# jianfch/stable-ts

Hardware: AMD Instinct MI355X
Metric: real-time factor (audio-sec/wall-sec) large-v3 word_timestamps=True (higher is better)
Workload: dtype f16; 1 GPU; large-v3 (random-init, weight recipe BENCH_WEIGHTS = the parity-pinned recipe of tests/test_gpu_f16_depth.py), 10 min synthetic 16 kHz audio per GPU, word_timestamps=True, beam_size=5, 112 decode steps/window, window-parallel batch 20, default regrouping inside the timed pass; mode=transcribe, windows_per_gpu=20, segments=125, words=1670, parallelism=dp1 (windows sharded, no data-path collective)

## Files before the change

include/swx.h:

```cpp
#ifndef SWX_H
#define SWX_H
#include <stdint.h>
#include <stddef.h>

#ifdef __cplusplus
extern "C" {
#endif

#define SWX_F32 0
#define SWX_F16 1

#define SWX_N_SAMPLES 480000
#define SWX_N_FRAMES 3000
#define SWX_N_FFT 400
#define SWX_HOP 160

typedef struct swx_dims {
    int32_t n_mels, n_audio_ctx, n_audio_state, n_audio_head, n_audio_layer;
    int32_t n_vocab, n_text_ctx, n_text_state, n_text_head, n_text_layer;
} swx_dims;

typedef struct swx_model swx_model;

const char *swx_strerror(int code);
int swx_version(void);

int swx_model_create(const swx_dims *dims, int dtype, swx_model **out);
void swx_model_destroy(swx_model *m);
size_t swx_weights_bytes(const swx_model *m);
int swx_bind_weights(swx_model *m, void *d_arena, size_t bytes);
int swx_share_weights(swx_model *m, const swx_model *owner);
int swx_load_tensor(swx_model *m, const char *name, const float *d_src, int64_t numel, void *stream);
int swx_weights_complete(const swx_model *m);
int swx_missing_tensor(const swx_model *m, int index, char *buf, int buflen);
int swx_weights_mark_loaded(swx_model *m);
int swx_weights_finalize(swx_model *m, void *stream);
int swx_set_alignment_heads(swx_model *m, const int32_t *h_layer_head_pairs, int n_pairs);
int swx_num_alignment_heads(const swx_model *m);

size_t swx_workspace_bytes(const swx_model *m, int max_windows, int max_rows);
int swx_bind_workspace(swx_model *m, void *d_ws, size_t bytes, int max_windows, int max_rows);

int swx_log_mel(swx_model *m, const float *d_pcm, int B, float *d_mel, int per_item_max, void *stream);

int swx_log_mel_ragged(swx_model *m, const float *d_pcm, const int32_t *n_valid, const int32_t *n_total, int B,
                       float *d_mel, int per_item_max, void *stream);
int swx_log_mel_ragged_grouped(swx_model *m, const float *d_pcm, const int32_t *n_valid, const int32_t *n_total, int B,
                               float *d_mel, int group, void *stream);

int swx_encode(swx_model *m, const float *d_mel, int B, void *d_xa, void *stream);

size_t swx_cross_kv_bytes(const swx_model *m, int B);
int swx_cross_kv(swx_model *m, const void *d_xa, int B, void *d_xkv, void *stream);

typedef struct swx_decode_cfg {
    int32_t n_windows;
    int32_t n_group;
    int32_t beam;
    float temperature;
    float patience;
    int32_t sample_len;
    int32_t sample_begin;
    int32_t sot_index;
    int32_t suppress_blank;
    int32_t apply_timestamp_rules;
    int32_t max_initial_timestamp_index;
    int32_t eot, sot, no_timestamps, timestamp_begin, no_speech, blank_token;
    int32_t n_suppress;
    int32_t min_tokens;
    uint64_t seed;
    const int32_t *window_uid;
    const float *noise;
    const int32_t *sample_begins;
    const int32_t *sot_indices;
} swx_decode_cfg;

int swx_decode(swx_model *m, const swx_decode_cfg *cfg, const int32_t *d_init_tokens, const int32_t *d_suppress,
               const uint8_t *d_ts_mask, const void *d_xkv, int32_t *d_tokens_out, int32_t *d_lens_out,
               float *d_sumlp_out, float *d_nospeech, void *stream);
int swx_decode_gout(const swx_decode_cfg *cfg);

int swx_score(swx_model *m, const int32_t *d_tokens, const int32_t *h_n_tok, int W, int max_n, int n_sot, int eot,
              const int32_t *h_n_frames, float qk_scale, int medfilt_width, const void *d_xkv,
              float *d_token_probs, float *d_neg_matrix, void *stream);

int swx_score_qk(swx_model *m, const int32_t *d_tokens, const int32_t *h_n_tok, int W, int max_n, int n_sot, int eot,
                 int row0, int n_rows, const void *d_xkv, float *d_token_probs, float *d_qk, void *stream);

size_t swx_qcap_bytes(const swx_model *m, int max_n);
int swx_score_q(swx_model *m, const int32_t *d_tokens, const int32_t *h_n_tok, int max_n, int n_sot, int eot,
                const void *d_xkv, float *d_token_probs, void *d_q, void *stream);
size_t swx_heads_scratch_bytes(const swx_model *m, int max_n);
int swx_heads_dynamic(swx_model *m, const void *d_q, int max_n, int row0, int n_rows, const void *d_xkv, int n_frames,
                      float qk_scale, int count, const double *d_peaks, float *d_qk_sel, int ld_f, void *d_scratch,
                      size_t scratch_bytes, void *stream);
int swx_heads_new(swx_model *m, const void *d_q, int max_n, int n_tok, int row0, int n_out, const void *d_xkv, int n_frames,
                  float qk_scale, int medfilt_width, int topk, float w_colnorm, float w_rownorm, float w_coverage,
                  float *d_neg_matrix, int ld_f, void *d_scratch, size_t scratch_bytes, void *stream);
int swx_weighted_sum(const float *const *h_xs, const float *h_coef, int n_in, float *d_out, int64_t n, void *stream);

int swx_forward_logits(swx_model *m, const int32_t *d_tokens, const int32_t *h_n_tok, int W, int max_n,
                       const void *d_xkv, float *d_logits, void *stream);

int swx_forward_token_ranks(swx_model *m, const int32_t *d_tokens, const int32_t *h_n_tok, int W, int max_n, int n_vocab_used,
                            const void *d_xkv, float *d_prob, int32_t *d_rank, void *stream);

size_t swx_align_weights_scratch_bytes(int W, int H, int N);
int swx_align_weights(const float *d_qk, int W, int H, int N, int ld_f, const int32_t *h_n_frames, float qk_scale,
                      int medfilt_width, float *d_neg_matrix, void *d_scratch, size_t scratch_bytes, void *stream);

int swx_median_filter(const float *d_x, int64_t rows, int n, int width, float *d_out, void *stream);

int swx_loudness_probe(const float *d_pcm, int64_t pcm_stride, const int32_t *d_nk, const int32_t *d_idx, int n_idx, int W,
                       float *d_out, void *d_scratch, size_t scratch_bytes, void *stream);
size_t swx_loudness_probe_scratch_bytes(int W);

typedef struct swx_flac_info {
    int32_t sample_rate, channels, bits_per_sample, min_block, max_block;
    int64_t total_samples;
    uint8_t md5[16];
} swx_flac_info;
int swx_flac_probe(const uint8_t *h_data, size_t n_bytes, swx_flac_info *info);
int64_t swx_flac_decode(const uint8_t *h_data, size_t n_bytes, int32_t *h_out, int64_t capacity_frames, swx_flac_info *info);

size_t swx_dtw_workspace_bytes(int W, int ld_n, int ld_m);
int swx_dtw(const float *d_x, int W, int ld_n, int ld_m, const int32_t *d_N, const int32_t *d_M,
            int32_t *d_text_idx, int32_t *d_time_idx, int32_t *d_len, void *d_trace_ws, void *stream);

int swx_prof_enable(int on);
int swx_debug_flags(int flags);
int swx_prof_collect(double *out, int n_classes);
int swx_graph_stats(const swx_model *m, int64_t *out);

int swx_test_gemm(int dtype, const void *d_a, int64_t lda, const void *d_w, const float *d_bias, const void *d_res,
                  void *d_c, int64_t ldc, int M, int N, int K, int epilogue, int force_kernel, void *stream);
int swx_test_gemm_plan(int M, int N, int K, int epilogue, int force_kernel, int flags);
int swx_test_dec_gemm(const void *d_a, int64_t lda, const void *d_w, const float *d_gamma, const float *d_beta,
                      const float *d_bias, void *d_c, int64_t ldc, void *d_x, void *d_kcache, void *d_vcache,
                      const int32_t *d_pos0, int n_ctx, int d, int M, int N, int K, int epilogue, void *d_scratch,
                      size_t scratch_bytes, void *stream);
int swx_test_layernorm(int dtype, const void *d_x, const float *d_g, const float *d_b, void *d_y, int rows, int d,
                       void *stream);
int swx_test_attention(int dtype, const void *d_q, int64_t ldq, const void *d_k, const void *d_v, int64_t ldkv,
                       void *d_o, int64_t ldo, int B, int H, int nq, int nk, int force_kernel, int vt_kp, void *stream);

int swx_test_self_attn_step(const void *d_q, void *d_kcache, void *d_vcache, const int32_t *d_anc, const int32_t *d_pos0,
                            int R, int H, int n_ctx, int d, int variant, void *d_o, void *stream);

int swx_test_self_attn_multi(const void *d_q, void *d_kcache, void *d_vcache, int R, int H, int n_new, int n_ctx, int d, int mq,
                             void *d_o, void *stream);

int swx_test_lane_xor(const uint32_t *d_in, uint32_t *d_out, int n_waves, void *stream);

int swx_test_gelu_pair(uint64_t *d_out, void *stream);

#ifdef __cplusplus
}
#endif
#endif
```

stable_ts_amd/_lib.py:

```python
import ctypes
import os
from ctypes import POINTER, Structure, c_char_p, c_float, c_int, c_int32, c_int64, c_size_t, c_uint64, c_void_p

_HERE = os.path.dirname(os.path.abspath(__file__))
LIB_PATH = os.path.join(_HERE, "libswx.so")

SWX_F32 = 0
SWX_F16 = 1


class SwxError(RuntimeError):
    pass


class swx_dims(Structure):
    _fields_ = [(n, c_int32) for n in ("n_mels", "n_audio_ctx", "n_audio_state", "n_audio_head", "n_audio_layer",
                                       "n_vocab", "n_text_ctx", "n_text_state", "n_text_head", "n_text_layer")]


class swx_flac_info(Structure):
    _fields_ = [("sample_rate", c_int32), ("channels", c_int32), ("bits_per_sample", c_int32), ("min_block", c_int32),
                ("max_block", c_int32), ("total_samples", c_int64), ("md5", ctypes.c_uint8 * 16)]


class swx_decode_cfg(Structure):
    _fields_ = [
        ("n_windows", c_int32), ("n_group", c_int32), ("beam", c_int32), ("temperature", c_float),
        ("patience", c_float), ("sample_len", c_int32), ("sample_begin", c_int32), ("sot_index", c_int32),
        ("suppress_blank", c_int32), ("apply_timestamp_rules", c_int32), ("max_initial_timestamp_index", c_int32),
        ("eot", c_int32), ("sot", c_int32), ("no_timestamps", c_int32), ("timestamp_begin", c_int32),
        ("no_speech", c_int32), ("blank_token", c_int32), ("n_suppress", c_int32), ("min_tokens", c_int32),
        ("seed", c_uint64), ("window_uid", POINTER(c_int32)), ("noise", c_void_p),
        ("sample_begins", POINTER(c_int32)), ("sot_indices", POINTER(c_int32)),
    ]


SYMBOLS = {
    "swx_strerror": (c_char_p, [c_int]),
    "swx_version": (c_int, []),
    "swx_model_create": (c_int, [POINTER(swx_dims), c_int, POINTER(c_void_p)]),
    "swx_model_destroy": (None, [c_void_p]),
    "swx_weights_bytes": (c_size_t, [c_void_p]),
    "swx_bind_weights": (c_int, [c_void_p, c_void_p, c_size_t]),
    "swx_share_weights": (c_int, [c_void_p, c_void_p]),
    "swx_load_tensor": (c_int, [c_void_p, c_char_p, c_void_p, c_int64, c_void_p]),
    "swx_weights_complete": (c_int, [c_void_p]),
    "swx_missing_tensor": (c_int, [c_void_p, c_int, c_char_p, c_int]),
    "swx_weights_mark_loaded": (c_int, [c_void_p]),
    "swx_weights_finalize": (c_int, [c_void_p, c_void_p]),
    "swx_set_alignment_heads": (c_int, [c_void_p, POINTER(c_int32), c_int]),
    "swx_num_alignment_heads": (c_int, [c_void_p]),
    "swx_workspace_bytes": (c_size_t, [c_void_p, c_int, c_int]),
    "swx_bind_workspace": (c_int, [c_void_p, c_void_p, c_size_t, c_int, c_int]),
    "swx_log_mel": (c_int, [c_void_p, c_void_p, c_int, c_void_p, c_int, c_void_p]),
    "swx_log_mel_ragged": (c_int, [c_void_p, c_void_p, c_void_p, c_void_p, c_int, c_void_p, c_int, c_void_p]),
    "swx_log_mel_ragged_grouped": (c_int, [c_void_p, c_void_p, c_void_p, c_void_p, c_int, c_void_p, c_int, c_void_p]),
    "swx_encode": (c_int, [c_void_p, c_void_p, c_int, c_void_p, c_void_p]),
    "swx_cross_kv_bytes": (c_size_t, [c_void_p, c_int]),
    "swx_cross_kv": (c_int, [c_void_p, c_void_p, c_int, c_void_p, c_void_p]),
    "swx_decode": (c_int, [c_void_p, POINTER(swx_decode_cfg), c_void_p, c_void_p, c_void_p, c_void_p, c_void_p,
                           c_void_p, c_void_p, c_void_p, c_void_p]),
    "swx_decode_gout": (c_int, [POINTER(swx_decode_cfg)]),
    "swx_score": (c_int, [c_void_p, c_void_p, POINTER(c_int32), c_int, c_int, c_int, c_int, POINTER(c_int32), c_float,
                          c_int, c_void_p, c_void_p, c_void_p, c_void_p]),
    "swx_score_qk": (c_int, [c_void_p, c_void_p, POINTER(c_int32), c_int, c_int, c_int, c_int, c_int, c_int, c_void_p,
                             c_void_p, c_void_p, c_void_p]),
    "swx_qcap_bytes": (c_size_t, [c_void_p, c_int]),
    "swx_score_q": (c_int, [c_void_p, c_void_p, POINTER(c_int32), c_int, c_int, c_int, c_void_p, c_void_p, c_void_p, c_void_p]),
    "swx_heads_scratch_bytes": (c_size_t, [c_void_p, c_int]),
    "swx_heads_dynamic": (c_int, [c_void_p, c_void_p, c_int, c_int, c_int, c_void_p, c_int, c_float, c_int, c_void_p, c_void_p,
                                  c_int, c_void_p, c_size_t, c_void_p]),
    "swx_heads_new": (c_int, [c_void_p, c_void_p, c_int, c_int, c_int, c_int, c_void_p, c_int, c_float, c_int, c_int, c_float,
                              c_float, c_float, c_void_p, c_int, c_void_p, c_size_t, c_void_p]),
    "swx_weighted_sum": (c_int, [c_void_p, c_void_p, c_int, c_void_p, c_int64, c_void_p]),
    "swx_forward_logits": (c_int, [c_void_p, c_void_p, POINTER(c_int32), c_int, c_int, c_void_p, c_void_p, c_void_p]),
    "swx_forward_token_ranks": (c_int, [c_void_p, c_void_p, POINTER(c_int32), c_int, c_int, c_int, c_void_p, c_void_p, c_void_p,
                                        c_void_p]),
    "swx_align_weights_scratch_bytes": (c_size_t, [c_int, c_int, c_int]),
    "swx_align_weights": (c_int, [c_void_p, c_int, c_int, c_int, c_int, POINTER(c_int32), c_float, c_int, c_void_p,
                                  c_void_p, c_size_t, c_void_p]),
    "swx_median_filter": (c_int, [c_void_p, c_int64, c_int, c_int, c_void_p, c_void_p]),
    "swx_loudness_probe": (c_int, [c_void_p, c_int64, c_void_p, c_void_p, c_int, c_int, c_void_p, c_void_p, c_size_t, c_void_p]),
    "swx_loudness_probe_scratch_bytes": (c_size_t, [c_int]),
    "swx_flac_probe": (c_int, [c_void_p, c_size_t, POINTER(swx_flac_info)]),
    "swx_flac_decode": (c_int64, [c_void_p, c_size_t, c_void_p, c_int64, POINTER(swx_flac_info)]),
    "swx_dtw_workspace_bytes": (c_size_t, [c_int, c_int, c_int]),
    "swx_dtw": (c_int, [c_void_p, c_int, c_int, c_int, c_void_p, c_void_p, c_void_p, c_void_p, c_void_p, c_void_p,
                        c_void_p]),
    "swx_prof_enable": (c_int, [c_int]),
    "swx_debug_flags": (c_int, [c_int]),
    "swx_prof_collect": (c_int, [POINTER(ctypes.c_double), c_int]),
    "swx_graph_stats": (c_int, [c_void_p, POINTER(c_int64)]),
    "swx_test_gemm": (c_int, [c_int, c_void_p, c_int64, c_void_p, c_void_p, c_void_p, c_void_p, c_int64, c_int, c_int,
                              c_int, c_int, c_int, c_void_p]),
    "swx_test_gemm_plan": (c_int, [c_int, c_int, c_int, c_int, c_int, c_int]),
    "swx_test_dec_gemm": (c_int, [c_void_p, c_int64, c_void_p, c_void_p, c_void_p, c_void_p, c_void_p, c_int64, c_void_p,
                                  c_void_p, c_void_p, c_void_p, c_int, c_int, c_int, c_int, c_int, c_int, c_void_p, c_size_t,
                                  c_void_p]),
    "swx_test_self_attn_step": (c_int, [c_void_p, c_void_p, c_void_p, c_void_p, c_void_p, c_int, c_int, c_int, c_int, c_int, c_void_p,
                                        c_void_p]),
    "swx_test_self_attn_multi": (c_int, [c_void_p, c_void_p, c_void_p, c_int, c_int, c_int, c_int, c_int, c_int, c_void_p, c_void_p]),
    "swx_test_gelu_pair": (c_int, [c_void_p, c_void_p]),
    "swx_test_lane_xor": (c_int, [c_void_p, c_void_p, c_int, c_void_p]),
    "swx_test_layernorm": (c_int, [c_int, c_void_p, c_void_p, c_void_p, c_void_p, c_int, c_int, c_void_p]),
    "swx_test_attention": (c_int, [c_int, c_void_p, c_int64, c_void_p, c_void_p, c_int64, c_void_p, c_int64, c_int,
                                   c_int, c_int, c_int, c_int, c_int, c_void_p]),
}

_lib = None


def load(build_if_missing: bool = False) -> ctypes.CDLL:
    global _lib
    if _lib is not None:
        return _lib
    if not os.path.exists(LIB_PATH):
        if build_if_missing:
            from .build import build
            build(verbose=False)
        else:
            raise SwxError(f"{LIB_PATH} not found: build it with `python -m stable_ts_amd.build` "
                           f"(hipcc --offload-arch=gfx950). There is no CPU fallback.")
    lib = ctypes.CDLL(LIB_PATH)
    for name, (res, args) in SYMBOLS.items():
        fn = getattr(lib, name)
        fn.restype = res
        fn.argtypes = args
    _lib = lib
    return lib


def check(code: int, what: str = "") -> int:
    if code < 0:
        msg = load().swx_strerror(code).decode()
        raise SwxError(f"{what or 'libswx'} failed: {msg} ({code})")
    return code


def require_gpu():
    import torch
    if not torch.cuda.is_available():
        raise SwxError("stable_ts_amd needs a ROCm GPU (MI355X / gfx950); no CPU path exists in this package")
```

stable_ts_amd/csrc/swx_common.h:

```cpp
#pragma once
#include <hip/hip_runtime.h>
#include <hip/hip_fp16.h>
#include <stdint.h>
#include <math.h>

#define SWX_WAVE 64

typedef _Float16 f16;
typedef _Float16 f16x4 __attribute__((ext_vector_type(4)));
typedef _Float16 f16x8 __attribute__((ext_vector_type(8)));
typedef float f32x4 __attribute__((ext_vector_type(4)));
typedef float f32x16 __attribute__((ext_vector_type(16)));

#define SWX_CHECK_LAUNCH() do { hipError_t _e = hipGetLastError(); if (_e != hipSuccess) return -100 - (int)_e; } while (0)

static inline int cdiv(int64_t a, int64_t b) { return (int)((a + b - 1) / b); }

template <typename T> __device__ __forceinline__ float to_f32(T v);
template <> __device__ __forceinline__ float to_f32<float>(float v) { return v; }
template <> __device__ __forceinline__ float to_f32<f16>(f16 v) { return (float)v; }
template <typename T> __device__ __forceinline__ T from_f32(float v);
template <> __device__ __forceinline__ float from_f32<float>(float v) { return v; }
template <> __device__ __forceinline__ f16 from_f32<f16>(float v) { return (f16)v; }

template <typename T> __device__ __forceinline__ void load8(const T *p, float (&o)[8]);
template <> __device__ __forceinline__ void load8<f16>(const f16 *p, float (&o)[8]) {
    const f16x8 v = *(const f16x8 *)p;
#pragma unroll
    for (int e = 0; e < 8; ++e) o[e] = (float)v[e];
}
template <> __device__ __forceinline__ void load8<float>(const float *p, float (&o)[8]) {
    const f32x4 a = *(const f32x4 *)p, b = *(const f32x4 *)(p + 4);
#pragma unroll
    for (int e = 0; e < 4; ++e) { o[e] = a[e]; o[4 + e] = b[e]; }
}

__device__ __forceinline__ int swx_lane_id() { return (int)__builtin_amdgcn_mbcnt_hi(~0u, __builtin_amdgcn_mbcnt_lo(~0u, 0u)); }

template <int O> __device__ __forceinline__ unsigned lane_xor_u32(unsigned x, int lane)
{
    static_assert(O == 1 || O == 2 || O == 4 || O == 8 || O == 16 || O == 32, "lane_xor: one butterfly step");
#ifdef SWX_LANE_XOR_BPERMUTE
    return (unsigned)__shfl_xor((int)x, O, 64);
#endif
    if constexpr (O == 32) {
        const auto r = __builtin_amdgcn_permlane32_swap(x, x, false, false);
        return (lane & 32) ? r[0] : r[1];
    } else if constexpr (O == 16) {
        const auto r = __builtin_amdgcn_permlane16_swap(x, x, false, false);
        return (lane & 16) ? r[0] : r[1];
    } else if constexpr (O == 8) {
        return (unsigned)__builtin_amdgcn_update_dpp(0, (int)x, 0x128, 0xF, 0xF, false);
    } else if constexpr (O == 4) {
        int t = __builtin_amdgcn_update_dpp(0, (int)x, 0x104, 0xF, 0x5, false);
        t = __builtin_amdgcn_update_dpp(t, (int)x, 0x114, 0xF, 0xA, false);
        return (unsigned)t;
    } else if constexpr (O == 2) {
        return (unsigned)__builtin_amdgcn_update_dpp(0, (int)x, 0x4E, 0xF, 0xF, false);
    } else {
        return (unsigned)__builtin_amdgcn_update_dpp(0, (int)x, 0xB1, 0xF, 0xF, false);
    }
}
template <int O> __device__ __forceinline__ float lane_xor(float x, int lane) { return __uint_as_float(lane_xor_u32<O>(__float_as_uint(x), lane)); }
template <int O> __device__ __forceinline__ int lane_xor(int x, int lane) { return (int)lane_xor_u32<O>((unsigned)x, lane); }
template <int O> __device__ __forceinline__ double lane_xor(double x, int lane)
{
    const unsigned long long u = (unsigned long long)__double_as_longlong(x);
    const unsigned lo = lane_xor_u32<O>((unsigned)u, lane), hi = lane_xor_u32<O>((unsigned)(u >> 32), lane);
    return __longlong_as_double((long long)(((unsigned long long)hi << 32) | lo));
}
__device__ __forceinline__ float lane_xor16_max(float x) {
#ifdef SWX_LANE_XOR_BPERMUTE
    return fmaxf(x, __shfl_xor(x, 16, 64));
#endif
    const unsigned u = __float_as_uint(x);
    const auto r = __builtin_amdgcn_permlane16_swap(u, u, false, false);
    return fmaxf(__uint_as_float(r[0]), __uint_as_float(r[1]));
}
__device__ __forceinline__ float lane_xor32_max(float x) {
#ifdef SWX_LANE_XOR_BPERMUTE
    return fmaxf(x, __shfl_xor(x, 32, 64));
#endif
    const unsigned u = __float_as_uint(x);
    const auto r = __builtin_amdgcn_permlane32_swap(u, u, false, false);
    return fmaxf(__uint_as_float(r[0]), __uint_as_float(r[1]));
}
__device__ __forceinline__ float lane_xor16_add(float x) {
#ifdef SWX_LANE_XOR_BPERMUTE
    return x + __shfl_xor(x, 16, 64);
#endif
    const unsigned u = __float_as_uint(x);
    const auto r = __builtin_amdgcn_permlane16_swap(u, u, false, false);
    return __uint_as_float(r[0]) + __uint_as_float(r[1]);
}
__device__ __forceinline__ float lane_xor32_add(float x) {
#ifdef SWX_LANE_XOR_BPERMUTE
    return x + __shfl_xor(x, 32, 64);
#endif
    const unsigned u = __float_as_uint(x);
    const auto r = __builtin_amdgcn_permlane32_swap(u, u, false, false);
    return __uint_as_float(r[0]) + __uint_as_float(r[1]);
}

__device__ __forceinline__ float lane_xor16_max_lds(float x) {
#ifdef SWX_XATTN_VALU
    return lane_xor16_max(x);
#else
    return fmaxf(x, __shfl_xor(x, 16, 64));
#endif
}
__device__ __forceinline__ float lane_xor32_max_lds(float x) {
#ifdef SWX_XATTN_VALU
    return lane_xor32_max(x);
#else
    return fmaxf(x, __shfl_xor(x, 32, 64));
#endif
}
__device__ __forceinline__ float lane_xor16_add_lds(float x) {
#ifdef SWX_XATTN_VALU
    return lane_xor16_add(x);
#else
    return x + __shfl_xor(x, 16, 64);
#endif
}
__device__ __forceinline__ float lane_xor32_add_lds(float x) {
#ifdef SWX_XATTN_VALU
    return lane_xor32_add(x);
#else
    return x + __shfl_xor(x, 32, 64);
#endif
}

__device__ __forceinline__ float wave_max(float v) {
    const int lane = swx_lane_id();
    v = fmaxf(v, lane_xor<32>(v, lane)); v = fmaxf(v, lane_xor<16>(v, lane)); v = fmaxf(v, lane_xor<8>(v, lane));
    v = fmaxf(v, lane_xor<4>(v, lane)); v = fmaxf(v, lane_xor<2>(v, lane)); v = fmaxf(v, lane_xor<1>(v, lane));
    return v;
}
__device__ __forceinline__ float wave_sum(float v) {
    const int lane = swx_lane_id();
    v += lane_xor<32>(v, lane); v += lane_xor<16>(v, lane); v += lane_xor<8>(v, lane);
    v += lane_xor<4>(v, lane); v += lane_xor<2>(v, lane); v += lane_xor<1>(v, lane);
    return v;
}
__device__ __forceinline__ double wave_sum_d(double v) {
    const int lane = swx_lane_id();
    v += lane_xor<32>(v, lane); v += lane_xor<16>(v, lane); v += lane_xor<8>(v, lane);
    v += lane_xor<4>(v, lane); v += lane_xor<2>(v, lane); v += lane_xor<1>(v, lane);
    return v;
}

__device__ __forceinline__ float gelu_erf(float x) { return 0.5f * x * (1.0f + erff(x * 0.70710678118654752440f)); }

typedef float f32x2 __attribute__((ext_vector_type(2)));
__device__ __forceinline__ f32x2 swx_k2(unsigned u) { const float f = __uint_as_float(u); return (f32x2){f, f}; }
__device__ __forceinline__ f32x2 gelu_erf2(f32x2 x)
{
#ifdef SWX_GELU_SCALAR
    return (f32x2){gelu_erf(x[0]), gelu_erf(x[1])};
#else
    const f32x2 z = x * swx_k2(0x3f3504f3u);
    const f32x2 az = __builtin_elementwise_abs(z);
    f32x2 p = __builtin_elementwise_fma(az, swx_k2(0x378e98abu), swx_k2(0xb9c68948u));
    p = __builtin_elementwise_fma(az, p, swx_k2(0x3b7cd369u));
    p = __builtin_elementwise_fma(az, p, swx_k2(0xbcc618b2u));
    p = __builtin_elementwise_fma(az, p, swx_k2(0x3dda74e4u));
    p = __builtin_elementwise_fma(az, p, swx_k2(0x3f228afdu));
    p = __builtin_elementwise_fma(az, p, swx_k2(0x3e03c728u));
    const f32x2 t = __builtin_elementwise_fma(az, p, az);
    f32x2 a = t * swx_k2(0xbfb8aa3bu);
    f32x2 b = __builtin_elementwise_fma(t, swx_k2(0xbfb8aa3bu), -a);
    f32x2 r;
    r[0] = __builtin_rintf(a[0]); r[1] = __builtin_rintf(a[1]);
    b = __builtin_elementwise_fma(t, swx_k2(0xb2a5705fu), b);
    a = a - r;
    a = a + b;
    f32x2 big;
#pragma unroll
    for (int i = 0; i < 2; ++i) {
        float e = __builtin_amdgcn_exp2f(a[i]);
        e = __builtin_ldexpf(e, (int)r[i]);
        e = !(__uint_as_float(0x42ce8ed0u) < t[i]) ? e : 0.f;
        e = !(__uint_as_float(0xc2b17218u) > t[i]) ? e : __builtin_inff();
        big[i] = e;
    }
    big = swx_k2(0x3f800000u) - big;
    const f32x2 t2 = z * z;
    f32x2 q = __builtin_elementwise_fma(swx_k2(0xba1345e1u), t2, swx_k2(0x3ba10414u));
    q = __builtin_elementwise_fma(t2, q, swx_k2(0xbcdac9b8u));
    q = __builtin_elementwise_fma(t2, q, swx_k2(0x3de703beu));
    q = __builtin_elementwise_fma(t2, q, swx_k2(0xbec09330u));
    q = __builtin_elementwise_fma(t2, q, swx_k2(0x3e0375d0u));
    const f32x2 small = __builtin_elementwise_fma(az, q, az);
    f32x2 erf;
#pragma unroll
    for (int i = 0; i < 2; ++i) {
        const float res = !(az[i] < 1.0f) ? big[i] : small[i];
        erf[i] = __uint_as_float((__float_as_uint(res) & 0x7fffffffu) | (__float_as_uint(z[i]) & 0x80000000u));
    }
    return (x * swx_k2(0x3f000000u)) * (erf + swx_k2(0x3f800000u));
#endif
}
template <int N> __device__ __forceinline__ void gelu_erf_n(float (&v)[N])
{
    static_assert(N % 2 == 0, "pairs");
#pragma unroll
    for (int e = 0; e < N; e += 2) { f32x2 t = {v[e], v[e + 1]}; t = gelu_erf2(t); v[e] = t[0]; v[e + 1] = t[1]; }
}

__device__ __forceinline__ unsigned f32_to_ordered(float f) {
    unsigned u = __float_as_uint(f);
    return (u & 0x80000000u) ? ~u : (u | 0x80000000u);
}
__device__ __forceinline__ float ordered_to_f32(unsigned u) {
    return __uint_as_float((u & 0x80000000u) ? (u & 0x7fffffffu) : ~u);
}
```

stable_ts_amd/csrc/swx_decode.h:

```cpp
#pragma once
#include <hip/hip_runtime.h>
#include <stdint.h>
#include "../../include/swx.h"

struct DecodeBufs {
    swx_decode_cfg cfg;
    int W, G, M, V, TS, n_ctx, n_init;
    int max_cand, fin_cap;
    int32_t *tokens[2];
    int32_t *anc[2];
    int32_t *pos0;
    const int32_t *begin;
    float *sum_lp, *sum_lp_next;
    int32_t *row_done;
    int32_t *win_done, *win_done_prev;
    int32_t *n_done;
    int32_t *step_dev;
    int32_t *fin_tokens;
    float *fin_score;
    int32_t *fin_len;
    int32_t *fin_count;
    float *cand_lp;
    int32_t *cand_tok;
    float *logits;
    const int32_t *suppress;
    const uint8_t *ts_mask;
    const int32_t *win_uid;
};

int swx_decode_init(const DecodeBufs &b, const int32_t *init_tokens, hipStream_t s);
int swx_decode_after_prefill(const DecodeBufs &b, const float *lg2, float *nospeech, hipStream_t s);
int swx_decode_select(const DecodeBufs &b, int cur, hipStream_t s);
int swx_decode_finalize(const DecodeBufs &b, int cur, int n_steps, int32_t *tokens_out, int32_t *lens_out,
                        float *sumlp_out, int G_out, hipStream_t s);
```

stable_ts_amd/csrc/swx_decode.hip:

```cpp
#include "swx_common.h"
#include "swx_kernels.h"
#include "swx_decode.h"

namespace {

constexpr int SEL_T = 1024;
constexpr float NEG_INF = -__builtin_inff();

struct ArgMax { float v; int i; };

__device__ __forceinline__ ArgMax argmax_combine(ArgMax a, ArgMax b)
{
    if (b.v > a.v || (b.v == a.v && b.i < a.i)) return b;
    return a;
}

static_assert(SEL_T == 1024, "block reductions: 16 wave slots");

__device__ ArgMax block_argmax(ArgMax x, ArgMax *sh)
{
    const int wave = threadIdx.x >> 6, lane = threadIdx.x & 63;
#define SWX_ARGMAX_STEP(O) { ArgMax y; y.v = lane_xor<O>(x.v, lane); y.i = lane_xor<O>(x.i, lane); x = argmax_combine(x, y); }
    SWX_ARGMAX_STEP(32) SWX_ARGMAX_STEP(16) SWX_ARGMAX_STEP(8) SWX_ARGMAX_STEP(4) SWX_ARGMAX_STEP(2) SWX_ARGMAX_STEP(1)
    __syncthreads();
    if (lane == 0) sh[wave] = x;
    __syncthreads();
#ifdef SWX_SELECT_R5_REDUCE
    ArgMax r = sh[0];
    for (int w = 1; w < (int)(blockDim.x >> 6); ++w) r = argmax_combine(r, sh[w]);
    return r;
#else
    x = sh[lane & 15];
    SWX_ARGMAX_STEP(8) SWX_ARGMAX_STEP(4) SWX_ARGMAX_STEP(2) SWX_ARGMAX_STEP(1)
    return x;
#endif
#undef SWX_ARGMAX_STEP
}

__device__ float block_max(float x, float *sh)
{
    x = wave_max(x);
    const int wave = threadIdx.x >> 6, lane = threadIdx.x & 63;
    __syncthreads();
    if (lane == 0) sh[wave] = x;
    __syncthreads();
#if defined(SWX_SELECT_R5_REDUCE) || defined(SWX_SELECT_MAX_WALK)
    float r = sh[0];
    for (int w = 1; w < (int)(blockDim.x >> 6); ++w) r = fmaxf(r, sh[w]);
    return r;
#else
    const f32x4 *s4 = (const f32x4 *)sh;
    float r = -__builtin_inff();
#pragma unroll
    for (int q = 0; q < 4; ++q) { const f32x4 v = s4[q]; r = fmaxf(r, fmaxf(fmaxf(v[0], v[1]), fmaxf(v[2], v[3]))); }
    return r;
#endif
}

__device__ float block_sum(float x, float *sh)
{
    x = wave_sum(x);
    const int wave = threadIdx.x >> 6, lane = threadIdx.x & 63;
    __syncthreads();
    if (lane == 0) sh[wave] = x;
    __syncthreads();
    float r = 0.f;
#if defined(SWX_SELECT_R5_REDUCE) || defined(SWX_SELECT_SUM_WALK)
    for (int w = 0; w < (int)(blockDim.x >> 6); ++w) r += sh[w];
#else
    const f32x4 *s4 = (const f32x4 *)sh;
#pragma unroll
    for (int q = 0; q < 4; ++q) { const f32x4 v = s4[q]; r += v[0]; r += v[1]; r += v[2]; r += v[3]; }
#endif
    return r;
}

__device__ __forceinline__ unsigned hash32(unsigned x)
{
    x ^= x >> 16; x *= 0x7feb352du; x ^= x >> 15; x *= 0x846ca68bu; x ^= x >> 16;
    return x;
}

__device__ __forceinline__ float gumbel(uint64_t seed, unsigned row_uid, unsigned step, unsigned idx)
{
    unsigned h = hash32((unsigned)seed ^ hash32(idx + 0x9e3779b9u * (step + 1u)));
    h = hash32(h ^ hash32(row_uid * 0x85ebca6bu + (unsigned)(seed >> 32)));
    const float u = ((float)(h >> 8) + 0.5f) * (1.0f / 16777216.0f);
    return -logf(-logf(u));
}

__device__ __forceinline__ int win_begin(const DecodeBufs &b, int w) { return b.begin ? b.begin[w] : b.n_init; }

__global__ void decode_init_kernel(DecodeBufs b, const int32_t *__restrict__ init_tokens)
{
    const int r = blockIdx.x;
    const int w = r / b.G;
    const int n0 = win_begin(b, w);
    int32_t *row0 = b.tokens[0] + (size_t)r * b.TS;
    int32_t *row1 = b.tokens[1] + (size_t)r * b.TS;
    for (int i = threadIdx.x; i < b.TS; i += blockDim.x) {
        const int32_t t = (i < n0) ? init_tokens[(size_t)w * b.n_init + i] : b.cfg.eot;
        row0[i] = t;
        row1[i] = t;
    }
    if (threadIdx.x == 0) {
        b.pos0[r] = 0;
        b.sum_lp[r] = 0.f;
        b.row_done[r] = 0;
        if (r % b.G == 0) { b.win_done[w] = 0; b.fin_count[w] = 0; }
        if (r == 0) { *b.n_done = 0; *b.step_dev = 0; }
    }
}

__global__ void decode_after_prefill_kernel(DecodeBufs b)
{
    const int r = blockIdx.x;
    const int w = r / b.G;
    const int n0 = win_begin(b, w);
    if (b.anc[0]) {
        for (int p = threadIdx.x; p < b.n_ctx; p += blockDim.x) {
            const int v = (p < n0) ? w * b.G : r;
            b.anc[0][(size_t)r * b.n_ctx + p] = v;
            b.anc[1][(size_t)r * b.n_ctx + p] = v;
        }
    }
    if (threadIdx.x == 0) b.pos0[r] = n0 - 1;
}

__global__ __launch_bounds__(SEL_T) void decode_prefill_logits_kernel(DecodeBufs b, const float *__restrict__ lg2,
                                                                      float *__restrict__ nospeech)
{
    __shared__ __attribute__((aligned(16))) float sh[SEL_T / 64];
    const int r = blockIdx.x, w = r / b.G, V = b.V;
    const float *last = lg2 + ((size_t)w * 2 + 1) * V;
    float *dst = b.logits + (size_t)r * V;
    for (int i = threadIdx.x; i < V; i += SEL_T) dst[i] = last[i];
    if (r % b.G == 0 && nospeech) {
        const float *sot = lg2 + ((size_t)w * 2) * V;
        float mx = NEG_INF;
        for (int i = threadIdx.x; i < V; i += SEL_T) mx = fmaxf(mx, sot[i]);
        mx = block_max(mx, sh);
        float sum = 0.f;
        for (int i = threadIdx.x; i < V; i += SEL_T) sum += expf(sot[i] - mx);
        sum = block_sum(sum, sh);
        if (threadIdx.x == 0) nospeech[w] = (b.cfg.no_speech >= 0) ? expf(sot[b.cfg.no_speech] - mx) / sum : NAN;
    }
}

__global__ __launch_bounds__(SEL_T) void decode_select_kernel(DecodeBufs b, int cur)
{
    const int step = *b.step_dev;
    __shared__ __attribute__((aligned(16))) float shf[SEL_T / 64];
    __shared__ __attribute__((aligned(16))) ArgMax sha[SEL_T / 64];
    __shared__ int sh_last_ts;
    const int r = blockIdx.x, w = r / b.G, V = b.V, tid = threadIdx.x;
    const swx_decode_cfg &c = b.cfg;
    if (b.win_done[w]) return;
    float *lg = b.logits + (size_t)r * V;
    int32_t *tok = b.tokens[cur] + (size_t)r * b.TS;
    const int n0 = win_begin(b, w);
    const int len = n0 + step;
    const int nsamp = step;
    const int tsb = c.timestamp_begin;

    if (c.suppress_blank && nsamp == 0 && tid == 0) { if (c.blank_token >= 0) lg[c.blank_token] = NEG_INF; lg[c.eot] = NEG_INF; }
    for (int i = tid; i < c.n_suppress; i += SEL_T) { const int t = b.suppress[i]; if ((unsigned)t < (unsigned)V) lg[t] = NEG_INF; }
    if (c.min_tokens > 0 && nsamp < c.min_tokens && tid == 0) lg[c.eot] = NEG_INF;
    __syncthreads();

    if (c.apply_timestamp_rules) {
        if (tid == 0) { sh_last_ts = -1; if (c.no_timestamps >= 0) lg[c.no_timestamps] = NEG_INF; }
        __syncthreads();
        int my = -1;
        for (int i = n0 + tid; i < len; i += SEL_T) if (tok[i] >= tsb) my = i;
        if (my >= 0) atomicMax(&sh_last_ts, my);
        __syncthreads();
        const int last_ts_pos = sh_last_ts;
        const bool last_was_ts = nsamp >= 1 && tok[len - 1] >= tsb;
        const bool penult_was_ts = nsamp < 2 || tok[len - 2] >= tsb;
        int lo0 = 0, hi0 = 0;
        if (last_was_ts) { if (penult_was_ts) { lo0 = tsb; hi0 = V; } else { lo0 = 0; hi0 = c.eot; } }
        int hi1 = tsb;
        if (last_ts_pos >= 0) {
            const int tl = tok[last_ts_pos];
            hi1 = (last_was_ts && !penult_was_ts) ? tl : tl + 1;
        }
        int hi2 = 0;
        int lo3 = V;
        if (nsamp == 0) { hi2 = tsb; if (c.max_initial_timestamp_index >= 0) lo3 = tsb + c.max_initial_timestamp_index + 1; }
        float mx_text = NEG_INF, mx_ts = NEG_INF;
        for (int i = tid; i < V; i += SEL_T) {
            float v = lg[i];
            if ((i >= lo0 && i < hi0) || (i >= tsb && i < hi1) || (i < hi2) || (i >= lo3)) { v = NEG_INF; lg[i] = v; }
            if (i < tsb) mx_text = fmaxf(mx_text, v); else mx_ts = fmaxf(mx_ts, v);
        }
        mx_text = block_max(mx_text, shf);
        mx_ts = block_max(mx_ts, shf);
        float s_ts = 0.f;
        if (mx_ts > NEG_INF)
            for (int i = tsb + tid; i < V; i += SEL_T) s_ts += expf(lg[i] - mx_ts);
        s_ts = block_sum(s_ts, shf);
        const float lse_ts = (mx_ts > NEG_INF) ? mx_ts + logf(s_ts) : NEG_INF;
        if (lse_ts > mx_text)
            for (int i = tid; i < tsb; i += SEL_T) lg[i] = NEG_INF;
        __syncthreads();
    }

    const uint8_t *tmask = b.ts_mask ? b.ts_mask + (size_t)w * 1501 : nullptr;
    float mx = NEG_INF;
    for (int i = tid; i < V; i += SEL_T) {
        float v = lg[i];
        if (tmask && i >= tsb && i - tsb < 1501 && tmask[i - tsb]) v = NEG_INF;
        if (v != v) v = NEG_INF;
        else if (v == NEG_INF) v = -3.4028234663852886e38f;
        else if (v == -NEG_INF) v = 3.4028234663852886e38f;
        lg[i] = v;
        mx = fmaxf(mx, v);
    }
    mx = block_max(mx, shf);
    float se = 0.f;
    for (int i = tid; i < V; i += SEL_T) se += expf(lg[i] - mx);
    se = block_sum(se, shf);
    const float lse = logf(se);

    if (!c.beam) {
        ArgMax best; best.v = NEG_INF; best.i = 0x7fffffff;
        if (c.temperature == 0.f) {
            for (int i = tid; i < V; i += SEL_T) { ArgMax x; x.v = lg[i]; x.i = i; best = argmax_combine(best, x); }
        } else {
            const float invT = 1.0f / c.temperature;
            const unsigned row_uid = b.win_uid ? (unsigned)b.win_uid[r / b.G] * 0x9E3779B1u + (unsigned)(r % b.G) : (unsigned)r;
            const float *qn = c.noise ? c.noise + ((size_t)step * b.M + r) * V : nullptr;
            for (int i = tid; i < V; i += SEL_T) {
                ArgMax x; x.v = lg[i] * invT + (qn ? -logf(qn[i]) : gumbel(c.seed, row_uid, (unsigned)step, (unsigned)i)); x.i = i;
                best = argmax_combine(best, x);
            }
        }
        best = block_argmax(best, sha);
        if (tid == 0) {
            int next = best.i;
            const bool prev_eot = tok[len - 1] == c.eot;
            const float lp = (lg[next] - mx) - lse;
            if (!prev_eot) b.sum_lp[r] += lp; else next = c.eot;
            tok[len] = next;
            if (len < b.n_ctx) b.pos0[r] = len;
            b.row_done[r] = (next == c.eot) ? 1 : 0;
        }
    } else {
        const int K = b.G + 1;
        for (int k = 0; k < K; ++k) {
            ArgMax best; best.v = NEG_INF; best.i = 0x7fffffff;
            for (int i = tid; i < V; i += SEL_T) { ArgMax x; x.v = lg[i]; x.i = i; best = argmax_combine(best, x); }
            best = block_argmax(best, sha);
            if (tid == 0) {
                b.cand_lp[(size_t)r * K + k] = (best.v - mx) - lse;
                b.cand_tok[(size_t)r * K + k] = best.i;
                lg[best.i] = NEG_INF;
            }
            __syncthreads();
        }
    }
}

template <int NV>
__global__ __launch_bounds__(SEL_T) void decode_select_reg_kernel(DecodeBufs b, int cur)
{
    const int step = *b.step_dev;
    __shared__ __attribute__((aligned(16))) float shf[SEL_T / 64];
    __shared__ __attribute__((aligned(16))) ArgMax sha[SEL_T / 64];
    __shared__ float sh_rot[SEL_T];
    __shared__ int sh_last_ts;
    __shared__ float sh_raw;
    const int r = blockIdx.x, w = r / b.G, V = b.V, tid = threadIdx.x;
    const swx_decode_cfg &c = b.cfg;
    if (b.win_done[w]) return;
    float *lg = b.logits + (size_t)r * V;
    int32_t *tok = b.tokens[cur] + (size_t)r * b.TS;
    const int n0 = win_begin(b, w);
    const int len = n0 + step;
    const int nsamp = step;
    const int tsb = c.timestamp_begin;

    if (c.suppress_blank && nsamp == 0 && tid == 0) { if (c.blank_token >= 0) lg[c.blank_token] = NEG_INF; lg[c.eot] = NEG_INF; }
    for (int i = tid; i < c.n_suppress; i += SEL_T) { const int t = b.suppress[i]; if ((unsigned)t < (unsigned)V) lg[t] = NEG_INF; }
    if (c.min_tokens > 0 && nsamp < c.min_tokens && tid == 0) lg[c.eot] = NEG_INF;
    if (c.apply_timestamp_rules && tid == 0) { sh_last_ts = -1; if (c.no_timestamps >= 0) lg[c.no_timestamps] = NEG_INF; }
    __syncthreads();

    float v[NV];
#pragma unroll
    for (int k = 0; k < NV; ++k) { const int i = tid + k * SEL_T; v[k] = i < V ? lg[i] : NEG_INF; }

    if (c.apply_timestamp_rules) {
        int my = -1;
        for (int i = n0 + tid; i < len; i += SEL_T) if (tok[i] >= tsb) my = i;
        if (my >= 0) atomicMax(&sh_last_ts, my);
        __syncthreads();
        const int last_ts_pos = sh_last_ts;
        const bool last_was_ts = nsamp >= 1 && tok[len - 1] >= tsb;
        const bool penult_was_ts = nsamp < 2 || tok[len - 2] >= tsb;
        int lo0 = 0, hi0 = 0;
        if (last_was_ts) { if (penult_was_ts) { lo0 = tsb; hi0 = V; } else { lo0 = 0; hi0 = c.eot; } }
        int hi1 = tsb;
        if (last_ts_pos >= 0) {
            const int tl = tok[last_ts_pos];
            hi1 = (last_was_ts && !penult_was_ts) ? tl : tl + 1;
        }
        int hi2 = 0, lo3 = V;
        if (nsamp == 0) { hi2 = tsb; if (c.max_initial_timestamp_index >= 0) lo3 = tsb + c.max_initial_timestamp_index + 1; }
        float mx_text = NEG_INF, mx_ts = NEG_INF;
#pragma unroll
        for (int k = 0; k < NV; ++k) {
            const int i = tid + k * SEL_T;
            if (i < V) {
                if ((i >= lo0 && i < hi0) || (i >= tsb && i < hi1) || (i < hi2) || (i >= lo3)) v[k] = NEG_INF;
                if (i < tsb) mx_text = fmaxf(mx_text, v[k]); else mx_ts = fmaxf(mx_ts, v[k]);
            }
        }
        mx_text = block_max(mx_text, shf);
        mx_ts = block_max(mx_ts, shf);
        float s_own = 0.f;
        if (mx_ts > NEG_INF) {
#pragma unroll
            for (int k = 0; k < NV; ++k) { const int i = tid + k * SEL_T; if (i >= tsb && i < V) s_own += expf(v[k] - mx_ts); }
        }
        sh_rot[(tid - tsb) & (SEL_T - 1)] = s_own;
        __syncthreads();
        float s_ts = block_sum(sh_rot[tid], shf);
        const float lse_ts = (mx_ts > NEG_INF) ? mx_ts + logf(s_ts) : NEG_INF;
        if (lse_ts > mx_text) {
#pragma unroll
            for (int k = 0; k < NV; ++k) if (tid + k * SEL_T < tsb) v[k] = NEG_INF;
        }
    }

    const uint8_t *tmask = b.ts_mask ? b.ts_mask + (size_t)w * 1501 : nullptr;
    float mx = NEG_INF;
#pragma unroll
    for (int k = 0; k < NV; ++k) {
        const int i = tid + k * SEL_T;
        if (i < V) {
            float x = v[k];
            if (tmask && i >= tsb && i - tsb < 1501 && tmask[i - tsb]) x = NEG_INF;
            if (x != x) x = NEG_INF;
            else if (x == NEG_INF) x = -3.4028234663852886e38f;
            else if (x == -NEG_INF) x = 3.4028234663852886e38f;
            v[k] = x;
            mx = fmaxf(mx, x);
        }
    }
    mx = block_max(mx, shf);
    float se = 0.f;
#pragma unroll
    for (int k = 0; k < NV; ++k) if (tid + k * SEL_T < V) se += expf(v[k] - mx);
    se = block_sum(se, shf);
    const float lse = logf(se);

    if (!c.beam) {
        ArgMax best; best.v = NEG_INF; best.i = 0x7fffffff;
        float raw_own = 0.f;
        if (c.temperature == 0.f) {
#pragma unroll
            for (int k = 0; k < NV; ++k) {
                const int i = tid + k * SEL_T;
                if (i < V) { ArgMax x; x.v = v[k]; x.i = i; const ArgMax nb = argmax_combine(best, x); if (nb.i != best.i) raw_own = v[k]; best = nb; }
            }
        } else {
            const float invT = 1.0f / c.temperature;
            const unsigned row_uid = b.win_uid ? (unsigned)b.win_uid[r / b.G] * 0x9E3779B1u + (unsigned)(r % b.G) : (unsigned)r;
            const float *qn = c.noise ? c.noise + ((size_t)step * b.M + r) * V : nullptr;
#pragma unroll
            for (int k = 0; k < NV; ++k) {
                const int i = tid + k * SEL_T;
                if (i < V) {
                    ArgMax x; x.v = v[k] * invT + (qn ? -logf(qn[i]) : gumbel(c.seed, row_uid, (unsigned)step, (unsigned)i)); x.i = i;
                    const ArgMax nb = argmax_combine(best, x);
                    if (nb.i != best.i) raw_own = v[k];
                    best = nb;
                }
            }
        }
        const int own_i = best.i;
        best = block_argmax(best, sha);
        if (own_i == best.i) sh_raw = raw_own;
        __syncthreads();
        if (tid == 0) {
            int next = best.i;
            const bool prev_eot = tok[len - 1] == c.eot;
            const float lp = (sh_raw - mx) - lse;
            if (!prev_eot) b.sum_lp[r] += lp; else next = c.eot;
            tok[len] = next;
            if (len < b.n_ctx) b.pos0[r] = len;
            b.row_done[r] = (next == c.eot) ? 1 : 0;
        }
    } else {
        const int K = b.G + 1;
        auto local_best = [&]() {
            ArgMax best; best.v = NEG_INF; best.i = 0x7fffffff;
#pragma unroll
            for (int k = 0; k < NV; ++k) {
                const int i = tid + k * SEL_T;
                if (i < V) { ArgMax x; x.v = v[k]; x.i = i; best = argmax_combine(best, x); }
            }
            return best;
        };
        ArgMax mine = local_best();
        for (int kk = 0; kk < K; ++kk) {
            const ArgMax best = block_argmax(mine, sha);
            if (tid == 0) {
                b.cand_lp[(size_t)r * K + kk] = (best.v - mx) - lse;
                b.cand_tok[(size_t)r * K + kk] = best.i;
            }
            if ((best.i & (SEL_T - 1)) == tid) {
#pragma unroll
                for (int k = 0; k < NV; ++k) if (tid + k * SEL_T == best.i) v[k] = NEG_INF;
                mine = local_best();
            }
        }
    }
}

__global__ __launch_bounds__(256) void decode_beam_update_kernel(DecodeBufs b, int cur)
{
    const int step = *b.step_dev;
    constexpr int MAXC = 17 * 16;
    __shared__ float sc[MAXC];
    __shared__ short src[MAXC];
    __shared__ int tk[MAXC];
    __shared__ short order[MAXC];
    __shared__ int sel_src[16], sel_tok[16];
    __shared__ float sel_sc[16];
    const int w = blockIdx.x, G = b.G, K = G + 1, tid = threadIdx.x;
    const swx_decode_cfg &c = b.cfg;
    __shared__ int s_frozen;
    if (tid == 0) s_frozen = b.win_done[w];
    __syncthreads();
    const bool frozen = s_frozen != 0;
    const int len = win_begin(b, w) + step;
    const int nb = (step == 0) ? 1 : G;
    const int nc = nb * K;
    if (!frozen) {
        for (int ci = tid; ci < nc; ci += 256) {
            const int j = ci / K, k = ci - j * K, idx = w * G + j;
            sc[ci] = b.sum_lp[idx] + b.cand_lp[(size_t)idx * K + k];
            src[ci] = (short)idx;
            tk[ci] = b.cand_tok[(size_t)idx * K + k];
        }
    }
    __syncthreads();
    if (!frozen) {
        for (int ci = tid; ci < nc; ci += 256) {
            const float raw = sc[ci], mine = (raw != raw) ? -INFINITY : raw;
            int rank = 0;
            for (int q = 0; q < nc; ++q) {
                const float rq = sc[q], oq = (rq != rq) ? -INFINITY : rq;
                rank += (oq > mine || (oq == mine && q < ci)) ? 1 : 0;
            }
            order[rank] = (short)ci;
        }
    }
    __syncthreads();
    if (frozen) {
        if (tid < G) sel_src[tid] = w * G + tid;
    } else if (tid == 0) {
        int saved = 0;
        int fc = b.fin_count[w];
        for (int a = 0; a < nc && saved < G; ++a) {
            const int ci = order[a];
            if (tk[ci] == c.eot) {
                if (fc < b.max_cand) {
                    int32_t *ft = b.fin_tokens + ((size_t)w * b.fin_cap + fc) * b.TS;
                    const int32_t *st = b.tokens[cur] + (size_t)src[ci] * b.TS;
                    for (int i = 0; i < len; ++i) ft[i] = st[i];
                    for (int i = len; i < b.TS; ++i) ft[i] = c.eot;
                    b.fin_score[(size_t)w * b.fin_cap + fc] = sc[ci];
                    b.fin_len[(size_t)w * b.fin_cap + fc] = len + 1;
                    ++fc;
                }
            } else {
                sel_src[saved] = src[ci]; sel_tok[saved] = tk[ci]; sel_sc[saved] = sc[ci];
                ++saved;
            }
        }
        b.fin_count[w] = fc;
        if (fc >= b.max_cand) b.win_done[w] = 1;
    }
    __syncthreads();
    for (int s = 0; s < G; ++s) {
        const int dst = w * G + s, from = sel_src[s];
        const int32_t *st = b.tokens[cur] + (size_t)from * b.TS;
        int32_t *dt = b.tokens[cur ^ 1] + (size_t)dst * b.TS;
        const int32_t *sa = b.anc[cur] + (size_t)from * b.n_ctx;
        int32_t *da = b.anc[cur ^ 1] + (size_t)dst * b.n_ctx;
        if (frozen) {
            for (int i = tid; i < b.TS; i += 256) dt[i] = st[i];
            for (int p = tid; p < b.n_ctx; p += 256) da[p] = sa[p];
        } else {
            for (int i = tid; i < b.TS; i += 256) dt[i] = (i < len) ? st[i] : (i == len ? sel_tok[s] : c.eot);
            for (int p = tid; p < b.n_ctx; p += 256) da[p] = (p < len) ? sa[p] : dst;
            if (tid == 0) { b.sum_lp[dst] = sel_sc[s]; if (len < b.n_ctx) b.pos0[dst] = len; }
        }
    }
}

__global__ __launch_bounds__(64) void decode_step_finish_kernel(DecodeBufs b)
{
    if (blockIdx.x != 0) return;
    const int lane = threadIdx.x;
    const int step = *b.step_dev;
    int nd = 0;
    for (int w = lane; w < b.W; w += 64) {
        int done = b.win_done[w];
        if (!b.cfg.beam && !done) {
            int all = 1;
            for (int g = 0; g < b.G; ++g) all &= b.row_done[w * b.G + g];
            if (all) { b.win_done[w] = 1; done = 1; }
        }
        if (b.begin && !done && b.begin[w] + step + 1 > b.n_ctx) { b.win_done[w] = 1; done = 1; }
        b.win_done_prev[w] = done;
        nd += done ? 1 : 0;
    }
    nd += lane_xor<32>(nd, lane); nd += lane_xor<16>(nd, lane); nd += lane_xor<8>(nd, lane);
    nd += lane_xor<4>(nd, lane); nd += lane_xor<2>(nd, lane); nd += lane_xor<1>(nd, lane);
    if (lane == 0) { *b.n_done = nd; *b.step_dev = step + 1; }
}

__global__ void decode_finalize_kernel(DecodeBufs b, int cur, int n_steps, int32_t *__restrict__ tokens_out,
                                       int32_t *__restrict__ lens_out, float *__restrict__ sumlp_out, int G_out)
{
    const int w = blockIdx.x, tid = threadIdx.x, TS = b.TS;
    const swx_decode_cfg &c = b.cfg;
    __shared__ int n_out;
    __shared__ int pick[16];
    if (!c.beam) {
        for (int g = 0; g < b.G; ++g) {
            const int32_t *st = b.tokens[cur] + (size_t)(w * b.G + g) * TS;
            int32_t *dt = tokens_out + ((size_t)w * G_out + g) * TS;
            for (int i = tid; i < TS; i += blockDim.x) dt[i] = st[i];
            if (tid == 0) sumlp_out[(size_t)w * G_out + g] = b.sum_lp[w * b.G + g];
        }
        if (tid == 0) n_out = b.G;
    } else {
        if (tid == 0) {
            int fc = b.fin_count[w];
            int np = 0;
            if (fc < b.G) {
                bool used[16];
                for (int g = 0; g < b.G; ++g) used[g] = false;
                while (fc + np < b.G) {
                    int bj = -1;
                    for (int g = b.G - 1; g >= 0; --g)
                        if (!used[g] && (bj < 0 || b.sum_lp[w * b.G + g] > b.sum_lp[w * b.G + bj])) bj = g;
                    used[bj] = true;
                    pick[np++] = bj;
                }
            }
            n_out = fc + np;
        }
        __syncthreads();
        const int fc = b.fin_count[w];
        for (int k = 0; k < n_out; ++k) {
            int32_t *dt = tokens_out + ((size_t)w * G_out + k) * TS;
            if (k < fc) {
                const int32_t *st = b.fin_tokens + ((size_t)w * b.fin_cap + k) * TS;
                for (int i = tid; i < TS; i += blockDim.x) dt[i] = st[i];
                if (tid == 0) sumlp_out[(size_t)w * G_out + k] = b.fin_score[(size_t)w * b.fin_cap + k];
            } else {
                const int g = pick[k - fc];
                const int32_t *st = b.tokens[cur] + (size_t)(w * b.G + g) * TS;
                for (int i = tid; i < TS; i += blockDim.x) dt[i] = st[i];
                if (tid == 0) sumlp_out[(size_t)w * G_out + k] = b.sum_lp[w * b.G + g];
            }
        }
    }
    __syncthreads();
    for (int k = tid; k < G_out; k += blockDim.x) {
        if (k >= n_out) { lens_out[(size_t)w * G_out + k] = -1; continue; }
    }
    __syncthreads();
    if (tid == 0) {
        for (int k = 0; k < n_out; ++k) {
            const int32_t *dt = tokens_out + ((size_t)w * G_out + k) * TS;
            const int n0 = win_begin(b, w);
            int e = n0;
            while (e < TS && dt[e] != c.eot) ++e;
            lens_out[(size_t)w * G_out + k] = e - n0;
        }
    }
}

}

int swx_decode_init(const DecodeBufs &b, const int32_t *init_tokens, hipStream_t s)
{
    hipLaunchKernelGGL(decode_init_kernel, dim3(b.M), dim3(256), 0, s, b, init_tokens);
    SWX_CHECK_LAUNCH();
    return 0;
}
int swx_decode_after_prefill(const DecodeBufs &b, const float *lg2, float *nospeech, hipStream_t s)
{
    hipLaunchKernelGGL(decode_after_prefill_kernel, dim3(b.M), dim3(256), 0, s, b);
    hipLaunchKernelGGL(decode_prefill_logits_kernel, dim3(b.M), dim3(SEL_T), 0, s, b, lg2, nospeech);
    SWX_CHECK_LAUNCH();
    return 0;
}
int swx_decode_select(const DecodeBufs &b, int cur, hipStream_t s)
{
    SwxProfScope prof(PC_SELECT, (double)b.M * b.V * 4.0, s);
    const bool mem_kernel = swx_flags() & SWX_FLAG_SELECT_MEM;
    if (!mem_kernel && b.V <= 51 * SEL_T)
        hipLaunchKernelGGL(decode_select_reg_kernel<51>, dim3(b.M), dim3(SEL_T), 0, s, b, cur);
    else
        hipLaunchKernelGGL(decode_select_kernel, dim3(b.M), dim3(SEL_T), 0, s, b, cur);
    if (b.cfg.beam) {
        hipLaunchKernelGGL(decode_beam_update_kernel, dim3(b.W), dim3(256), 0, s, b, cur);
    }
    hipLaunchKernelGGL(decode_step_finish_kernel, dim3(1), dim3(64), 0, s, b);
    SWX_CHECK_LAUNCH();
    return 0;
}
int swx_decode_finalize(const DecodeBufs &b, int cur, int n_steps, int32_t *tokens_out, int32_t *lens_out,
                        float *sumlp_out, int G_out, hipStream_t s)
{
    hipLaunchKernelGGL(decode_finalize_kernel, dim3(b.W), dim3(256), 0, s, b, cur, n_steps, tokens_out, lens_out, sumlp_out, G_out);
    SWX_CHECK_LAUNCH();
    return 0;
}
```

stable_ts_amd/csrc/swx_kernels.h:

```cpp
#pragma once
#include <hip/hip_runtime.h>
#include <stdint.h>
#include "../../include/swx.h"

#define EPI_BIAS 1
#define EPI_GELU 2
#define EPI_RES 4
#define EPI_OUT_F32 8
#define EPI_RESF32MOD 16
#define EPI_CBATCH 64
#define EPI_STORE_VT 32
#define EPI_KV 128

#define EPI_QKV_VT 256

struct GemmArgs {
    const void *A; int64_t lda;
    const void *W; int64_t ldw;
    const float *bias;
    const void *R; int64_t ldr;
    const float *Rf; int res_mod;
    void *C; int64_t ldc;
    void *C2;
    void *P; int64_t p_bs;
    int p_nkpad, p_vcol0;
    int M, N, K;
    int epi;
    int vt_s, vt_kp; int64_t vt_bs;
    int vt_zero_pad;
    int tile_order;
};
int swx_gemm(int dtype, const GemmArgs &g, int force_kernel, hipStream_t s);
enum { SWX_GEMM_TILED_REG = 0, SWX_GEMM_SKINNY = 1, SWX_GEMM_GLDS128 = 2, SWX_GEMM_GLDS64 = 3, SWX_GEMM_RING64 = 4, SWX_GEMM_RING128 = 5,
       SWX_GEMM_BIG = 6 };
int swx_gemm_plan_f16(int M, int N, int K, int epi, int64_t ldc, int64_t ldr, bool ptr16, int force_kernel, int flags);

#define SWX_FLAG_NO_FAST_STEP 1
#define SWX_FLAG_NO_PACKED_XKV 2048
#define SWX_FLAG_SELECT_MEM 8192
#define SWX_FLAG_NO_GRAPH 16384
#define SWX_FLAG_NO_PREFETCH 32768
#define SWX_FLAG_NO_RING 65536
#define SWX_FLAG_SCORE_TILED 262144
#define SWX_FLAG_NO_TALL 524288
#define SWX_FLAG_NO_FUSED_XQ 1048576
#define SWX_FLAG_TICKET 2097152
#define SWX_FLAG_BIG8_GROUPED 4194304
#define SWX_FLAG_XKV_TWO_LAUNCHES 8388608
#define SWX_FLAG_LOUDNESS_ONE_WG 16777216
#define SWX_FLAG_XATTN_R5 33554432
#define SWX_FLAG_FLASH_PIPELINED 67108864
#define SWX_FLAG_SELFATTN_WG5 134217728
#define SWX_FLAG_QKV_SEPARATE_VT 268435456
#define SWX_FLAG_SELFATTN_NO_DEEP 4
#define SWX_FLAG_DEC_NO_W1 16
#define SWX_FLAG_TALL_NO_W8 32
#define SWX_FLAG_SELFATTN_NO_MQ 256
#define SWX_FLAG_FLASH_NO_QB1 64
#define SWX_FLAG_XKV_PACK_SEPARATE 128
#define SWX_FLAG_DEC_W1_FULL_TILE 256
#define SWX_FLAG_XQ_FULL_TILE 512
#define SWX_FLAG_NO_BIG_TILE 131072
#define SWX_DEFAULT_FLAGS 0
int swx_flags();

#define DEC_LN 1
#define DEC_GELU 2
#define DEC_RES 4
#define DEC_QKV 8
#define DEC_SLAB 16
#define DEC_TICKET 32
struct DecPrefetch {
    const void *base;
    int lines;
};
DecPrefetch swx_dec_prefetch_of(const void *packed_w, int M, int N, int K, int epi);

struct DecGemmArgs {
    const _Float16 *A; int64_t lda;
    const _Float16 *W; int64_t ldw;
    int M, N, K;
    int epi;
    const float *c2;
    const float *c1;
    _Float16 *C; int64_t ldc;
    _Float16 *X; int64_t ldx;
    float *slabs;
    int *ticket;
    _Float16 *kcache, *vcache; const int32_t *pos0; int n_ctx, d;
    int rps;
    int row_mul;
    int ks2, kslice, n_rg; int64_t slab_stride;
    int tall;
    int tps;
    DecPrefetch pf;
    int w1_full_tile;
};
#define SWX_DEC_TICKETS 4096
int swx_dec_plan(int M, int N, int K, int epi, int *mt, int *ks2);
size_t swx_dec_slab_floats(int M, int N, int K);
int swx_gemm_dec(DecGemmArgs g, hipStream_t s);
int swx_fold_ln(const void *W, const float *gamma, const float *beta, const float *bias, void *Wf, float *c1, float *c2,
                int N, int K, hipStream_t s);

enum SwxProfClass { PC_GEMM_TILED = 0, PC_GEMM_SKINNY = 1, PC_ATTN_FLASH = 2, PC_ATTN_ROWWISE = 3, PC_SELF_ATTN = 4,
                    PC_SELECT = 5, PC_MEL = 6, PC_ALIGN = 7, PC_DTW = 8, PC_NORM = 9, PC_COUNT = 10 };
bool swx_prof_on();
void swx_prof_begin(int cls, double work, hipStream_t s);
void swx_prof_end(hipStream_t s);
struct SwxProfScope {
    hipStream_t s; bool on;
    SwxProfScope(int cls, double work, hipStream_t st) : s(st), on(swx_prof_on()) { if (on) swx_prof_begin(cls, work, st); }
    ~SwxProfScope() { if (on) swx_prof_end(s); }
};

int swx_layernorm(int dtype, const void *x, int64_t ldx, const float *gamma, const float *beta, void *y, int64_t ldy,
                  int rows, int d, hipStream_t s);
int swx_mel_transpose(int dtype, const float *mel, int B, int n_mels, int Cp, void *melT, hipStream_t s);
int swx_fill_zero(void *p, size_t bytes, hipStream_t s);
int swx_embed(int dtype, const int32_t *tokens, int64_t ld_tok, const int32_t *tok_off, const int32_t *pos0, int R, int n_new,
              const void *tok_emb, const float *pos_emb, int d, void *x, hipStream_t s);
int swx_convert_f32(int dtype, const float *src, void *dst, int64_t n, hipStream_t s);
int swx_copy_rows(int dtype, const float *src, int64_t src_ld, void *dst, int64_t dst_ld, int64_t rows, int64_t cols,
                  hipStream_t s);
int swx_copy_conv_w(int dtype, const float *src, int out_c, int in_c, int in_cp, void *dst, hipStream_t s);

struct AttnArgs {
    const void *q; int64_t ldq;
    const void *k; const void *v; int64_t ldkv;
    int64_t k_bs, v_bs;
    int vt_kp;
    void *o; int64_t ldo;
    int B, H, nq, nk;
    int q_rows_per_batch;
    const void *kv_packed;
    const _Float16 *fq_x; int64_t fq_ldx; int fq_rows;
    const _Float16 *fq_w; const float *fq_c1, *fq_c2; int fq_k;
    const void *fq_pf; int fq_pf_lines;
    int fq_full_tile;
};
__host__ __device__ inline int64_t swx_xkv_packed_elems_per_head(int nk) { return (int64_t)((nk + 31) / 32) * 4 * 512 * 2; }
int swx_xkv_pack(const void *k, const void *vt, void *packed, int B, int H, int nk, int ldk, int vt_kp, int64_t batch_stride,
                 hipStream_t s);
#define SWX_VT_KP 1536
int swx_attention(int dtype, const AttnArgs &a, int force_kernel, hipStream_t s);
int swx_transpose_v(const void *v, int64_t ldv, int64_t v_bs, int n, void *vt, int kp, int64_t vt_bs, int B, int H, hipStream_t s);
int swx_pad_zero(void *base, int64_t row_bytes, int64_t batch_bytes, int off_bytes, int pad_bytes, int rows, int nb, hipStream_t s);
struct SelfAttnArgs {
    const void *qkv; int64_t ldqkv;
    void *kcache; void *vcache;
    int32_t *anc;
    const int32_t *pos0;
    void *o; int64_t ldo;
    int R, n_new, H, n_ctx, d;
    int skip_append;
    int step_cached;
    int step_pos;
    int pos_bound;
    int pos0_all_zero;
};
int swx_self_attention(int dtype, const SelfAttnArgs &a, int row_mul, hipStream_t s);
int swx_qk_capture(int dtype, const void *q, int64_t ldq, int q_rows_per_w, int row0, int n_rows, const void *k,
                   int64_t ldk, int64_t k_bs, int nk, const int32_t *heads, int n_heads, int head_slot0, int slots_total, int W,
                   float *out, int out_ld_n, int out_ld_f, hipStream_t s);

int swx_align_weights_launch(const float *d_qk, float *d_p, float *d_mean, float *d_sd, int W, int H, int N, int ld_f,
                             const int *d_n_rows, const int *d_n_frames, float qk_scale, int medfilt_width,
                             float *d_neg_matrix, int out_ld_n, int out_ld_f, hipStream_t s);
int swx_mel_launch(const float *d_pcm, int B, const float *d_hann, const double2 *d_twiddle, const float *d_filters,
                   int n_mels, float *d_mel, unsigned *d_gmax, int per_item_max, hipStream_t s);
int swx_mel_ragged_launch(const float *d_pcm, const int *d_lens, int B, const float *d_hann, const double2 *d_twiddle,
                          const float *d_filters, int n_mels, float *d_mel, unsigned *d_gmax, int group,
                          hipStream_t s);

constexpr int SWX_HS_MAXF = 1536;
int swx_headsel_dynamic_launch(int dtype, const void *qcap, int max_n, int d, int row0, int n_rows, const void *xkv,
                               int64_t layer_stride, int L, int H, int F, int nk, float qk_scale, int count, const double *d_peaks,
                               double *d_score, int32_t *d_sel, float *d_out, int out_ld_f, hipStream_t s);
int swx_headsel_new_launch(int dtype, const void *qcap, int max_n, int d, int n, int row0, int n_out, const void *xkv,
                           int64_t layer_stride, int L, int H, int F, float qk_scale, int medfilt_width, int topk, float w_col,
                           float w_row, float w_cov, float *d_colnorm, float *d_score, int32_t *d_top, float *d_out, int out_ld_f,
                           hipStream_t s);
int swx_weighted_sum_launch(const float *const *h_xs, const float *h_coef, int n_in, float *d_out, int64_t n, hipStream_t s);

struct DecodeState;
```

stable_ts_amd/csrc/swx_norm.hip:

```cpp
#include "swx_common.h"
#include "swx_kernels.h"

namespace {

constexpr int LN_MAXC = 3;
template <typename T>
__global__ __launch_bounds__(256) void layernorm_kernel(const T *__restrict__ x, int64_t ldx, const float *__restrict__ gamma,
                                                        const float *__restrict__ beta, T *__restrict__ y, int64_t ldy,
                                                        int rows, int d)
{
    const int wave = threadIdx.x >> 6, lane = threadIdx.x & 63;
    const int row = blockIdx.x * 4 + wave;
    if (row >= rows) return;
    const T *xr = x + (size_t)row * ldx;
    const int nchunk = d >> 3;
    float v[LN_MAXC][8];
    float s = 0.f;
#pragma unroll
    for (int c = 0; c < LN_MAXC; ++c) {
        const int ch = lane + 64 * c;
        if (ch < nchunk) {
            load8<T>(xr + ch * 8, v[c]);
#pragma unroll
            for (int e = 0; e < 8; ++e) s += v[c][e];
        }
    }
    const float mean = wave_sum(s) / (float)d;
    float q = 0.f;
#pragma unroll
    for (int c = 0; c < LN_MAXC; ++c) {
        const int ch = lane + 64 * c;
        if (ch < nchunk) {
#pragma unroll
            for (int e = 0; e < 8; ++e) { const float t = v[c][e] - mean; q += t * t; }
        }
    }
    const float rstd = 1.0f / sqrtf(wave_sum(q) / (float)d + 1e-5f);
    T *yr = y + (size_t)row * ldy;
#pragma unroll
    for (int c = 0; c < LN_MAXC; ++c) {
        const int ch = lane + 64 * c;
        if (ch < nchunk) {
            float gm[8], bt[8];
            load8<float>(gamma + ch * 8, gm);
            load8<float>(beta + ch * 8, bt);
#pragma unroll
            for (int e = 0; e < 8; ++e) yr[ch * 8 + e] = from_f32<T>((v[c][e] - mean) * rstd * gm[e] + bt[e]);
        }
    }
}

template <typename T>
__global__ __launch_bounds__(256) void mel_transpose_kernel(const float *__restrict__ mel, int n_mels, int Cp, T *__restrict__ melT)
{
    const int b = blockIdx.y;
    const size_t total = (size_t)3002 * Cp;
    for (size_t i = (size_t)blockIdx.x * 256 + threadIdx.x; i < total; i += (size_t)gridDim.x * 256) {
        const int t = (int)(i / Cp), c = (int)(i % Cp);
        float v = 0.f;
        if (t >= 1 && t <= 3000 && c < n_mels) v = mel[((size_t)b * n_mels + c) * 3000 + (t - 1)];
        melT[(size_t)b * total + i] = from_f32<T>(v);
    }
}

template <typename T>
__global__ __launch_bounds__(256) void embed_kernel(const int32_t *__restrict__ tokens, int64_t ld_tok,
                                                    const int32_t *__restrict__ pos0, int n_new, const T *__restrict__ tok_emb,
                                                    const float *__restrict__ pos_emb, int d, T *__restrict__ x)
{
    const int r = blockIdx.y, i = blockIdx.x;
    const int p = pos0[r] + i;
    const int tok = tokens[(size_t)r * ld_tok + p];
    const T *e = tok_emb + (size_t)tok * d;
    const float *pe = pos_emb + (size_t)p * d;
    T *o = x + ((size_t)r * n_new + i) * d;
    for (int c = threadIdx.x; c < d; c += 256) o[c] = from_f32<T>(to_f32<T>(e[c]) + pe[c]);
}

template <typename T>
__global__ __launch_bounds__(256) void copy_rows_kernel(const float *__restrict__ src, int64_t src_ld, T *__restrict__ dst,
                                                        int64_t dst_ld, int64_t rows, int64_t cols)
{
    const int64_t total = rows * cols;
    for (int64_t i = (int64_t)blockIdx.x * 256 + threadIdx.x; i < total; i += (int64_t)gridDim.x * 256) {
        const int64_t r = i / cols, c = i % cols;
        dst[r * dst_ld + c] = from_f32<T>(src[r * src_ld + c]);
    }
}

template <typename T>
__global__ __launch_bounds__(256) void copy_conv_w_kernel(const float *__restrict__ src, int out_c, int in_c, int in_cp,
                                                          T *__restrict__ dst)
{
    const int64_t total = (int64_t)out_c * 3 * in_cp;
    for (int64_t i = (int64_t)blockIdx.x * 256 + threadIdx.x; i < total; i += (int64_t)gridDim.x * 256) {
        const int c = (int)(i % in_cp);
        const int tap = (int)((i / in_cp) % 3);
        const int o = (int)(i / ((int64_t)3 * in_cp));
        dst[i] = from_f32<T>(c < in_c ? src[((int64_t)o * in_c + c) * 3 + tap] : 0.f);
    }
}

}

int swx_layernorm(int dtype, const void *x, int64_t ldx, const float *gamma, const float *beta, void *y, int64_t ldy,
                  int rows, int d, hipStream_t s)
{
    if (rows <= 0) return 0;
    if (d % 8 != 0 || d > 8 * 64 * LN_MAXC) return -2;
    SwxProfScope prof(PC_NORM, 2.0 * rows * (double)d * (dtype == SWX_F16 ? 2 : 4), s);
    if (dtype == SWX_F16)
        hipLaunchKernelGGL(layernorm_kernel<f16>, dim3(cdiv(rows, 4)), dim3(256), 0, s, (const f16 *)x, ldx, gamma, beta, (f16 *)y, ldy, rows, d);
    else
        hipLaunchKernelGGL(layernorm_kernel<float>, dim3(cdiv(rows, 4)), dim3(256), 0, s, (const float *)x, ldx, gamma, beta, (float *)y, ldy, rows, d);
    SWX_CHECK_LAUNCH();
    return 0;
}

int swx_mel_transpose(int dtype, const float *mel, int B, int n_mels, int Cp, void *melT, hipStream_t s)
{
    if (B <= 0) return 0;
    dim3 g(256, B);
    if (dtype == SWX_F16) hipLaunchKernelGGL(mel_transpose_kernel<f16>, g, dim3(256), 0, s, mel, n_mels, Cp, (f16 *)melT);
    else hipLaunchKernelGGL(mel_transpose_kernel<float>, g, dim3(256), 0, s, mel, n_mels, Cp, (float *)melT);
    SWX_CHECK_LAUNCH();
    return 0;
}

int swx_fill_zero(void *p, size_t bytes, hipStream_t s)
{
    hipError_t e = hipMemsetAsync(p, 0, bytes, s);
    return e == hipSuccess ? 0 : -100 - (int)e;
}

int swx_embed(int dtype, const int32_t *tokens, int64_t ld_tok, const int32_t *, const int32_t *pos0, int R, int n_new,
              const void *tok_emb, const float *pos_emb, int d, void *x, hipStream_t s)
{
    if (R <= 0 || n_new <= 0) return 0;
    dim3 g(n_new, R);
    if (dtype == SWX_F16) hipLaunchKernelGGL(embed_kernel<f16>, g, dim3(256), 0, s, tokens, ld_tok, pos0, n_new, (const f16 *)tok_emb, pos_emb, d, (f16 *)x);
    else hipLaunchKernelGGL(embed_kernel<float>, g, dim3(256), 0, s, tokens, ld_tok, pos0, n_new, (const float *)tok_emb, pos_emb, d, (float *)x);
    SWX_CHECK_LAUNCH();
    return 0;
}

int swx_convert_f32(int dtype, const float *src, void *dst, int64_t n, hipStream_t s)
{
    return swx_copy_rows(dtype, src, n, dst, n, 1, n, s);
}

int swx_copy_rows(int dtype, const float *src, int64_t src_ld, void *dst, int64_t dst_ld, int64_t rows, int64_t cols, hipStream_t s)
{
    if (rows <= 0 || cols <= 0) return 0;
    const int64_t total = rows * cols;
    const int blocks = (int)((total + 255) / 256 > 4096 ? 4096 : (total + 255) / 256);
    if (dtype == SWX_F16) hipLaunchKernelGGL(copy_rows_kernel<f16>, dim3(blocks), dim3(256), 0, s, src, src_ld, (f16 *)dst, dst_ld, rows, cols);
    else hipLaunchKernelGGL(copy_rows_kernel<float>, dim3(blocks), dim3(256), 0, s, src, src_ld, (float *)dst, dst_ld, rows, cols);
    SWX_CHECK_LAUNCH();
    return 0;
}

int swx_copy_conv_w(int dtype, const float *src, int out_c, int in_c, int in_cp, void *dst, hipStream_t s)
{
    const int64_t total = (int64_t)out_c * 3 * in_cp;
    const int blocks = (int)((total + 255) / 256 > 4096 ? 4096 : (total + 255) / 256);
    if (dtype == SWX_F16) hipLaunchKernelGGL(copy_conv_w_kernel<f16>, dim3(blocks), dim3(256), 0, s, src, out_c, in_c, in_cp, (f16 *)dst);
    else hipLaunchKernelGGL(copy_conv_w_kernel<float>, dim3(blocks), dim3(256), 0, s, src, out_c, in_c, in_cp, (float *)dst);
    SWX_CHECK_LAUNCH();
    return 0;
}
```

stable_ts_amd/csrc/swx_runtime.hip:

```cpp
#include <algorithm>
#include <map>
#include <memory>
#include <string>
#include <vector>
#include <cmath>
#include <cstring>
#include <cstdio>
#include <cstdlib>
#include "swx_common.h"
#include "swx_kernels.h"
#include "swx_decode.h"

namespace {

enum SlotKind { SK_MAT = 0, SK_VEC = 1, SK_CONV = 2 };

struct Slot {
    size_t off = 0;
    int kind = SK_VEC;
    int64_t rows = 0, cols = 0;
    int64_t dst_ld = 0;
    bool loaded = false;
};

struct LayerW {
    size_t ln1_g, ln1_b, wqkv, bqkv, wo, bo;
    size_t lnx_g, lnx_b, wcq, bcq, wckv, bckv, wco, bco;
    size_t ln2_g, ln2_b, w1, b1, w2, b2;
    size_t wqkv_f, qkv_c1, qkv_c2, wcq_f, cq_c1, cq_c2, w1_f, w1_c1, w1_c2;
    size_t wo_p, wco_p, w2_p;
};

size_t align_up(size_t v, size_t a = 256) { return (v + a - 1) / a * a; }

}

struct swx_model {
    swx_dims dims;
    int dtype;
    size_t esz;
    int Cp;
    std::map<std::string, Slot> slots;
    std::vector<LayerW> enc, dec;
    size_t o_conv1_w, o_conv1_b, o_conv2_w, o_conv2_b, o_enc_pos, o_lnpost_g, o_lnpost_b;
    size_t o_tok_emb, o_dec_pos, o_ln_g, o_ln_b;
    size_t o_hann, o_twiddle, o_filters, o_heads, o_zeros;
    size_t arena_bytes = 0;
    unsigned char *arena = nullptr;
    bool has_fold = false;
    std::shared_ptr<bool> fold_state = std::make_shared<bool>(false);
    bool is_folded() const { return has_fold && *fold_state; }
    std::vector<std::vector<int>> heads_by_layer;
    std::vector<int> head_slot0;
    int n_align = 0;
    std::vector<int32_t> heads_flat;
    unsigned char *ws = nullptr;
    size_t ws_bytes = 0;
    int max_windows = 0, max_rows = 0, ws_n_align = 0;
    struct WsLayout {
        size_t melT, h1, x, h, qkv, att, u, gmax, small_i32, zeros_i32, ticket;
        size_t tokens0, tokens1, anc0, anc1, pos0, win_begin, sum_lp, sum_lp_next, row_done, win_done, win_done_prev, n_done;
        size_t fin_tokens, fin_score, fin_len, fin_count, cand_lp, cand_tok, logits, hid2;
        size_t kcache, vcache, sk, sv, cap, mean, sd, suppress, slabs, heads, win_uid;
        size_t total;
        int64_t rows_big, logits_rows;
        size_t slab_bytes;
    } L;

    template <typename P> P *A(size_t off) const { return (P *)(arena + off); }
    template <typename P> P *Wp(size_t off) const { return (P *)(ws + off); }

    struct StepGraph { std::vector<uint64_t> key; hipGraph_t graph = nullptr; hipGraphExec_t exec = nullptr; uint64_t used = 0; };
    std::vector<StepGraph> graphs;
    uint64_t graph_clock = 0;
    std::vector<int32_t> ragged_hv;
    hipStream_t cap_stream = nullptr;
    bool graphs_off = false;
    int graph_failures = 0;
    int64_t n_captures = 0, n_replays = 0, n_eager_units = 0;
    void drop_graphs() {
        for (auto &g : graphs) { if (g.exec) (void)hipGraphExecDestroy(g.exec); if (g.graph) (void)hipGraphDestroy(g.graph); }
        graphs.clear();
    }
    ~swx_model() { drop_graphs(); if (cap_stream) (void)hipStreamDestroy(cap_stream); }
};

namespace {

constexpr int FIN_CAP = 32;
constexpr int MAX_GROUP = 16;
constexpr int MAX_SUPPRESS = 4096;
constexpr int SMALL_I32 = 8192;

size_t add_slot(swx_model *m, size_t &cur, const std::string &name, int kind, int64_t rows, int64_t cols, int64_t dst_ld,
                size_t bytes, size_t base_off = (size_t)-1, size_t sub_off = 0)
{
    Slot s;
    s.kind = kind; s.rows = rows; s.cols = cols; s.dst_ld = dst_ld;
    if (base_off == (size_t)-1) { s.off = cur; cur = align_up(cur + bytes); }
    else s.off = base_off + sub_off;
    m->slots[name] = s;
    return s.off;
}

void build_layout(swx_model *m)
{
    const swx_dims &D = m->dims;
    const size_t e = m->esz;
    size_t cur = 0;
    auto mat = [&](const std::string &n, int64_t r, int64_t c) { return add_slot(m, cur, n, SK_MAT, r, c, c, (size_t)r * c * e); };
    auto vec = [&](const std::string &n, int64_t c) { return add_slot(m, cur, n, SK_VEC, 1, c, c, (size_t)c * 4); };
    auto reserve = [&](size_t bytes) { size_t o = cur; cur = align_up(cur + bytes); return o; };

    const int da = D.n_audio_state, dt = D.n_text_state;
    m->Cp = (D.n_mels + 31) / 32 * 32;
    m->o_conv1_w = add_slot(m, cur, "encoder.conv1.weight", SK_CONV, da, D.n_mels, m->Cp, (size_t)da * 3 * m->Cp * e);
    m->o_conv1_b = vec("encoder.conv1.bias", da);
    m->o_conv2_w = add_slot(m, cur, "encoder.conv2.weight", SK_CONV, da, da, da, (size_t)da * 3 * da * e);
    m->o_conv2_b = vec("encoder.conv2.bias", da);
    m->o_enc_pos = add_slot(m, cur, "encoder.positional_embedding", SK_VEC, 1, (int64_t)D.n_audio_ctx * da, 0, (size_t)D.n_audio_ctx * da * 4);

    auto block = [&](const std::string &p, int d, bool cross) {
        LayerW w{};
        w.ln1_g = vec(p + "attn_ln.weight", d);
        w.ln1_b = vec(p + "attn_ln.bias", d);
        w.wqkv = reserve((size_t)3 * d * d * e);
        add_slot(m, cur, p + "attn.query.weight", SK_MAT, d, d, d, 0, w.wqkv, 0);
        add_slot(m, cur, p + "attn.key.weight", SK_MAT, d, d, d, 0, w.wqkv, (size_t)d * d * e);
        add_slot(m, cur, p + "attn.value.weight", SK_MAT, d, d, d, 0, w.wqkv, (size_t)2 * d * d * e);
        w.bqkv = reserve((size_t)3 * d * 4);
        add_slot(m, cur, p + "attn.query.bias", SK_VEC, 1, d, d, 0, w.bqkv, 0);
        add_slot(m, cur, p + "attn.value.bias", SK_VEC, 1, d, d, 0, w.bqkv, (size_t)2 * d * 4);
        w.wo = mat(p + "attn.out.weight", d, d);
        w.bo = vec(p + "attn.out.bias", d);
        if (cross) {
            w.lnx_g = vec(p + "cross_attn_ln.weight", d);
            w.lnx_b = vec(p + "cross_attn_ln.bias", d);
            w.wcq = mat(p + "cross_attn.query.weight", d, d);
            w.bcq = vec(p + "cross_attn.query.bias", d);
            w.wckv = reserve((size_t)2 * d * d * e);
            add_slot(m, cur, p + "cross_attn.key.weight", SK_MAT, d, d, d, 0, w.wckv, 0);
            add_slot(m, cur, p + "cross_attn.value.weight", SK_MAT, d, d, d, 0, w.wckv, (size_t)d * d * e);
            w.bckv = reserve((size_t)2 * d * 4);
            add_slot(m, cur, p + "cross_attn.value.bias", SK_VEC, 1, d, d, 0, w.bckv, (size_t)d * 4);
            w.wco = mat(p + "cross_attn.out.weight", d, d);
            w.bco = vec(p + "cross_attn.out.bias", d);
        }
        w.ln2_g = vec(p + "mlp_ln.weight", d);
        w.ln2_b = vec(p + "mlp_ln.bias", d);
        w.w1 = mat(p + "mlp.0.weight", 4 * d, d);
        w.b1 = vec(p + "mlp.0.bias", 4 * d);
        w.w2 = mat(p + "mlp.2.weight", d, 4 * d);
        w.b2 = vec(p + "mlp.2.bias", d);
        return w;
    };
    for (int l = 0; l < D.n_audio_layer; ++l) m->enc.push_back(block("encoder.blocks." + std::to_string(l) + ".", da, false));
    m->o_lnpost_g = vec("encoder.ln_post.weight", da);
    m->o_lnpost_b = vec("encoder.ln_post.bias", da);
    m->o_tok_emb = mat("decoder.token_embedding.weight", D.n_vocab, dt);
    m->o_dec_pos = add_slot(m, cur, "decoder.positional_embedding", SK_VEC, 1, (int64_t)D.n_text_ctx * dt, 0, (size_t)D.n_text_ctx * dt * 4);
    for (int l = 0; l < D.n_text_layer; ++l) m->dec.push_back(block("decoder.blocks." + std::to_string(l) + ".", dt, true));
    {
        int mt = 0, ks = 0;
        m->has_fold = m->dtype == SWX_F16 && swx_dec_plan(64, 3 * dt, dt, DEC_LN, &mt, &ks) == 0 &&
                      swx_dec_plan(64, dt, 4 * dt, DEC_RES | DEC_SLAB, &mt, &ks) == 0;
        if (m->has_fold)
            for (auto &w : m->dec) {
                w.wqkv_f = reserve((size_t)3 * dt * dt * e); w.qkv_c1 = reserve((size_t)3 * dt * 4); w.qkv_c2 = reserve((size_t)3 * dt * 4);
                w.wcq_f = reserve((size_t)dt * dt * e); w.cq_c1 = reserve((size_t)dt * 4); w.cq_c2 = reserve((size_t)dt * 4);
                w.w1_f = reserve((size_t)4 * dt * dt * e); w.w1_c1 = reserve((size_t)4 * dt * 4); w.w1_c2 = reserve((size_t)4 * dt * 4);
                w.wo_p = reserve((size_t)dt * dt * e); w.wco_p = reserve((size_t)dt * dt * e); w.w2_p = reserve((size_t)4 * dt * dt * e);
            }
    }
    m->o_ln_g = vec("decoder.ln.weight", dt);
    m->o_ln_b = vec("decoder.ln.bias", dt);
    m->o_hann = vec("const.hann", SWX_N_FFT);
    m->o_filters = add_slot(m, cur, "const.mel_filters", SK_VEC, 1, (int64_t)D.n_mels * 201, 0, (size_t)D.n_mels * 201 * 4);
    m->o_twiddle = reserve(sizeof(double2) * SWX_N_FFT);
    m->o_heads = reserve(sizeof(int32_t) * (size_t)D.n_text_layer * D.n_text_head);
    m->o_zeros = reserve(256);
    m->arena_bytes = cur;
}

void default_alignment_heads(swx_model *m)
{
    const swx_dims &D = m->dims;
    m->heads_by_layer.assign(D.n_text_layer, {});
    for (int l = D.n_text_layer / 2; l < D.n_text_layer; ++l)
        for (int h = 0; h < D.n_text_head; ++h) m->heads_by_layer[l].push_back(h);
}

int upload_heads(swx_model *m)
{
    const swx_dims &D = m->dims;
    std::vector<int32_t> flat;
    m->head_slot0.assign(D.n_text_layer, 0);
    for (int l = 0; l < D.n_text_layer; ++l) {
        m->head_slot0[l] = (int)flat.size();
        for (int h : m->heads_by_layer[l]) flat.push_back(h);
    }
    m->n_align = (int)flat.size();
    m->heads_flat = flat;
    if (m->ws && m->n_align == m->ws_n_align && !flat.empty()) {
        hipError_t e = hipMemcpy(m->ws + m->L.heads, flat.data(), flat.size() * 4, hipMemcpyHostToDevice);
        if (e != hipSuccess) return -100 - (int)e;
    }
    return 0;
}

void ws_layout(const swx_model *m, int Bmax, int Mmax, int n_align, swx_model::WsLayout &L)
{
    const swx_dims &D = m->dims;
    const size_t e = m->esz;
    const int da = D.n_audio_state, dt = D.n_text_state;
    const int dmax = da > dt ? da : dt;
    const int TS = D.n_text_ctx + 1;
    size_t cur = 0;
    auto take = [&](size_t bytes) { size_t o = cur; cur = align_up(cur + bytes); return o; };
    int64_t rows_big = (int64_t)Bmax * D.n_audio_ctx;
    if ((int64_t)Bmax * D.n_text_ctx > rows_big) rows_big = (int64_t)Bmax * D.n_text_ctx;
    if (Mmax > rows_big) rows_big = Mmax;
    L.rows_big = rows_big;
    L.melT = take((size_t)Bmax * 3002 * m->Cp * e);
    L.h1 = take((size_t)Bmax * 3002 * da * e);
    L.x = take((size_t)rows_big * dmax * e);
    L.h = take((size_t)rows_big * dmax * e);
    L.qkv = take((size_t)rows_big * 3 * dmax * e);
    L.att = take((size_t)rows_big * dmax * e);
    L.u = take((size_t)rows_big * 4 * dmax * e);
    L.gmax = take((size_t)Bmax * 4);
    L.small_i32 = take((size_t)SMALL_I32 * 4);
    L.zeros_i32 = take((size_t)(Mmax > Bmax ? Mmax : Bmax) * 4 + 256);
    L.ticket = take((size_t)SWX_DEC_TICKETS * 4);
    L.tokens0 = take((size_t)Mmax * TS * 4);
    L.tokens1 = take((size_t)Mmax * TS * 4);
    L.anc0 = take((size_t)Mmax * D.n_text_ctx * 4);
    L.anc1 = take((size_t)Mmax * D.n_text_ctx * 4);
    L.pos0 = take((size_t)Mmax * 4);
    L.win_begin = take((size_t)Bmax * 4 * 3);
    L.sum_lp = take((size_t)Mmax * 4);
    L.sum_lp_next = take((size_t)Mmax * 4);
    L.row_done = take((size_t)Mmax * 4);
    L.win_done = take((size_t)Bmax * 4);
    L.win_done_prev = take((size_t)Bmax * 4);
    L.n_done = take(256);
    L.fin_tokens = take((size_t)Bmax * FIN_CAP * TS * 4);
    L.fin_score = take((size_t)Bmax * FIN_CAP * 4);
    L.fin_len = take((size_t)Bmax * FIN_CAP * 4);
    L.fin_count = take((size_t)Bmax * 4);
    L.cand_lp = take((size_t)Mmax * (MAX_GROUP + 1) * 4);
    L.cand_tok = take((size_t)Mmax * (MAX_GROUP + 1) * 4);
    int64_t lrows = (int64_t)Mmax + 2 * Bmax;
    if (lrows < 64) lrows = 64;
    L.logits_rows = lrows;
    L.logits = take((size_t)lrows * D.n_vocab * 4);
    L.hid2 = take((size_t)2 * Bmax * dt * e);
    L.kcache = take((size_t)D.n_text_layer * Mmax * D.n_text_ctx * dt * e);
    L.vcache = take((size_t)D.n_text_layer * Mmax * D.n_text_ctx * dt * e);
    L.sk = take((size_t)Bmax * D.n_text_ctx * dt * e);
    L.sv = take((size_t)Bmax * D.n_text_ctx * dt * e);
    L.cap = take((size_t)Bmax * (n_align > 0 ? n_align : 1) * D.n_text_ctx * D.n_audio_ctx * 4);
    L.mean = take((size_t)Bmax * (n_align > 0 ? n_align : 1) * D.n_audio_ctx * 4);
    L.sd = take((size_t)Bmax * (n_align > 0 ? n_align : 1) * D.n_audio_ctx * 4);
    L.suppress = take((size_t)MAX_SUPPRESS * 4);
    {
        int64_t srows = Mmax > 160 ? Mmax : 160;
        if ((int64_t)Bmax * D.n_text_ctx > srows) srows = (int64_t)Bmax * D.n_text_ctx;
        const size_t mx = swx_dec_slab_floats((int)srows, dt, 4 * dt);
        L.slabs = take(mx * 4 + 256);
        L.slab_bytes = mx * 4;
    }
    L.heads = take(sizeof(int32_t) * (size_t)D.n_text_layer * D.n_text_head);
    L.win_uid = take((size_t)Bmax * 4 + 256);
    L.total = cur;
}

inline hipStream_t S(void *s) { return (hipStream_t)s; }

struct ProfRec { int cls; double work; hipEvent_t a, b; };
bool g_prof_enabled = false;
int g_debug_flags = SWX_DEFAULT_FLAGS;
std::vector<ProfRec> g_prof;
std::vector<hipEvent_t> g_pool;
size_t g_pool_next = 0;

hipEvent_t prof_event()
{
    if (g_pool_next == g_pool.size()) {
        hipEvent_t e;
        if (hipEventCreate(&e) != hipSuccess) return nullptr;
        g_pool.push_back(e);
    }
    return g_pool[g_pool_next++];
}

#define SWX_TRY(expr) do { int _r = (expr); if (_r < 0) return _r; } while (0)

GemmArgs gemm_args(const void *A, int64_t lda, const void *W, int64_t ldw, const float *bias, void *C, int64_t ldc,
                   int M, int N, int K, int epi)
{
    GemmArgs g{};
    g.A = A; g.lda = lda; g.W = W; g.ldw = ldw; g.bias = bias; g.C = C; g.ldc = ldc; g.M = M; g.N = N; g.K = K; g.epi = epi;
    g.R = nullptr; g.ldr = 0; g.Rf = nullptr; g.res_mod = 1;
    return g;
}

int gemm_residual(swx_model *m, const void *A, int64_t lda, size_t w_off, size_t b_off, void *X, int64_t ldx, int M, int N,
                  int K, hipStream_t s)
{
    GemmArgs g = gemm_args(A, lda, m->arena + w_off, K, m->A<float>(b_off), X, ldx, M, N, K, EPI_BIAS | EPI_RES);
    g.R = X; g.ldr = ldx;
    return swx_gemm(m->dtype, g, 0, s);
}

inline int64_t xkv_plain_elems(const swx_dims &D)
{
    return (int64_t)D.n_audio_ctx * D.n_text_state + (int64_t)D.n_text_state * SWX_VT_KP;
}
inline int64_t xkv_packed_elems(const swx_dims &D)
{
    return (int64_t)D.n_text_head * swx_xkv_packed_elems_per_head(D.n_audio_ctx);
}
inline int64_t xkv_chunk_elems(const swx_model *m)
{
    return xkv_plain_elems(m->dims) + (m->dtype == SWX_F16 ? xkv_packed_elems(m->dims) : 0);
}

struct FwdCfg {
    int W;
    int rpw;
    int row_mul;
    int n_new;
    const int32_t *tokens; int64_t ld_tok;
    int xkv_W;
    const int32_t *pos0;
    unsigned char *kcache, *vcache;
    size_t layer_stride;
    int cache_rows;
    int32_t *anc;
    const unsigned char *xkv;
    bool capture; int cap_row0, cap_rows, cap_ld_n;
    int step_pos;
    int pos_bound;
    unsigned char *qcap;
};

int decoder_step_dec(swx_model *m, const FwdCfg &f, hipStream_t s)
{
    const swx_dims &D = m->dims;
    const int d = D.n_text_state, H = D.n_text_head;
    const size_t e = m->esz;
    const int rows = f.W * f.rpw;
    f16 *x = m->Wp<f16>(m->L.x), *q = m->Wp<f16>(m->L.qkv), *att = m->Wp<f16>(m->L.att), *u = m->Wp<f16>(m->L.u);
    float *slabs = m->Wp<float>(m->L.slabs);
    SWX_TRY(swx_embed(m->dtype, f.tokens, f.ld_tok, nullptr, f.pos0, rows, 1, m->arena + m->o_tok_emb,
                      m->A<float>(m->o_dec_pos), d, x, s));
    const int64_t chunk = xkv_chunk_elems(m);
    const bool pf_on = !(g_debug_flags & SWX_FLAG_NO_PREFETCH) && rows >= 32;
    auto pf_of = [&](size_t w_off, int N, int K, int epi) {
        return pf_on ? swx_dec_prefetch_of(m->A<f16>(w_off), rows, N, K, epi) : DecPrefetch{};
    };
    for (int l = 0; l < D.n_text_layer; ++l) {
        const LayerW &w = m->dec[l];
        f16 *kc = (f16 *)(f.kcache + (size_t)l * f.layer_stride), *vc = (f16 *)(f.vcache + (size_t)l * f.layer_stride);
        DecGemmArgs g{};
        g.M = rows;
        g.A = x; g.lda = d; g.W = m->A<f16>(w.wqkv_f); g.ldw = d; g.N = 3 * d; g.K = d; g.epi = DEC_LN | DEC_QKV;
        g.c1 = m->A<float>(w.qkv_c1); g.c2 = m->A<float>(w.qkv_c2); g.C = q; g.ldc = d;
        g.kcache = kc; g.vcache = vc; g.pos0 = f.pos0; g.n_ctx = D.n_text_ctx; g.d = d;
        g.pf = pf_of(w.wo_p, d, d, DEC_RES);
        SWX_TRY(swx_gemm_dec(g, s));
        SelfAttnArgs sa{};
        sa.qkv = q; sa.ldqkv = d; sa.kcache = kc; sa.vcache = vc; sa.anc = f.anc; sa.pos0 = f.pos0; sa.o = att; sa.ldo = d;
        sa.R = rows; sa.n_new = 1; sa.H = H; sa.n_ctx = D.n_text_ctx; sa.d = d; sa.skip_append = 1; sa.step_cached = 1;
        sa.step_pos = f.step_pos; sa.pos_bound = f.pos_bound;
        SWX_TRY(swx_self_attention(m->dtype, sa, 1, s));
        g = DecGemmArgs{};
        g.M = rows; g.A = att; g.lda = d; g.W = m->A<f16>(w.wo_p); g.ldw = d; g.N = d; g.K = d; g.epi = DEC_RES;
        g.c2 = m->A<float>(w.bo); g.X = x; g.ldx = d;
        g.pf = pf_of(w.wcq_f, d, d, DEC_LN);
        SWX_TRY(swx_gemm_dec(g, s));
        const bool fuse_xq = !(g_debug_flags & (SWX_FLAG_NO_FUSED_XQ | SWX_FLAG_NO_PACKED_XKV)) && f.rpw <= 16 && d % 128 == 0 &&
                             (d == 384 || d == 512 || d == 640 || d == 768 || d == 1024 || d == 1280);
        if (!fuse_xq) {
            g = DecGemmArgs{};
            g.M = rows; g.A = x; g.lda = d; g.W = m->A<f16>(w.wcq_f); g.ldw = d; g.N = d; g.K = d; g.epi = DEC_LN;
            g.c1 = m->A<float>(w.cq_c1); g.c2 = m->A<float>(w.cq_c2); g.C = q; g.ldc = d;
            g.pf = pf_of(w.wco_p, d, d, DEC_RES);
            SWX_TRY(swx_gemm_dec(g, s));
        }
        const unsigned char *kl = f.xkv + (size_t)l * (f.xkv_W ? f.xkv_W : f.W) * chunk * e;
        AttnArgs ca{};
        ca.q = q; ca.ldq = d; ca.k = kl; ca.v = kl + (size_t)D.n_audio_ctx * d * e; ca.ldkv = d;
        ca.k_bs = chunk; ca.v_bs = chunk; ca.vt_kp = SWX_VT_KP; ca.o = att; ca.ldo = d;
        ca.B = f.W; ca.H = H; ca.nq = f.rpw; ca.nk = D.n_audio_ctx; ca.q_rows_per_batch = f.rpw;
        ca.kv_packed = kl + (size_t)xkv_plain_elems(D) * e;
        if (fuse_xq) {
            ca.fq_x = x; ca.fq_ldx = d; ca.fq_rows = rows; ca.fq_w = m->A<f16>(w.wcq_f); ca.fq_c1 = m->A<float>(w.cq_c1);
            ca.fq_c2 = m->A<float>(w.cq_c2); ca.fq_k = d;
            if (pf_on) { ca.fq_pf = m->A<f16>(w.wco_p); ca.fq_pf_lines = (int)(((int64_t)d * d * 2) >> 7); }
        }
        SWX_TRY(swx_attention(m->dtype, ca, 0, s));
        g = DecGemmArgs{};
        g.M = rows; g.A = att; g.lda = d; g.W = m->A<f16>(w.wco_p); g.ldw = d; g.N = d; g.K = d; g.epi = DEC_RES;
        g.c2 = m->A<float>(w.bco); g.X = x; g.ldx = d;
        g.pf = pf_of(w.w1_f, 4 * d, d, DEC_LN | DEC_GELU);
        SWX_TRY(swx_gemm_dec(g, s));
        g = DecGemmArgs{};
        g.M = rows; g.A = x; g.lda = d; g.W = m->A<f16>(w.w1_f); g.ldw = d; g.N = 4 * d; g.K = d; g.epi = DEC_LN | DEC_GELU;
        g.c1 = m->A<float>(w.w1_c1); g.c2 = m->A<float>(w.w1_c2); g.C = u; g.ldc = 4 * d;
        g.pf = pf_of(w.w2_p, d, 4 * d, DEC_RES | DEC_SLAB);
        SWX_TRY(swx_gemm_dec(g, s));
        g = DecGemmArgs{};
        g.M = rows; g.A = u; g.lda = 4 * d; g.W = m->A<f16>(w.w2_p); g.ldw = 4 * d; g.N = d; g.K = 4 * d; g.epi = DEC_RES | DEC_SLAB;
        g.c2 = m->A<float>(w.b2); g.X = x; g.ldx = d; g.slabs = slabs; g.ticket = m->Wp<int>(m->L.ticket);
        if (l + 1 < D.n_text_layer) g.pf = pf_of(m->dec[l + 1].wqkv_f, 3 * d, d, DEC_LN | DEC_QKV);
        SWX_TRY(swx_gemm_dec(g, s));
    }
    return 0;
}

int decoder_forward_dec(swx_model *m, const FwdCfg &f, hipStream_t s)
{
    const swx_dims &D = m->dims;
    const int d = D.n_text_state, H = D.n_text_head;
    const size_t e = m->esz;
    const int R = f.W * f.rpw, rows = R * f.n_new;
    f16 *x = m->Wp<f16>(m->L.x), *q = m->Wp<f16>(m->L.qkv), *att = m->Wp<f16>(m->L.att), *u = m->Wp<f16>(m->L.u);
    float *slabs = m->Wp<float>(m->L.slabs);
    SWX_TRY(swx_embed(m->dtype, f.tokens, f.ld_tok, nullptr, f.pos0, R, f.n_new, m->arena + m->o_tok_emb,
                      m->A<float>(m->o_dec_pos), d, x, s));
    const int64_t chunk = xkv_chunk_elems(m);
    const bool pf_on = !(g_debug_flags & SWX_FLAG_NO_PREFETCH) && rows >= 32;
    auto pf_of = [&](size_t w_off, int N, int K, int epi) {
        return pf_on ? swx_dec_prefetch_of(m->A<f16>(w_off), rows, N, K, epi) : DecPrefetch{};
    };
    for (int l = 0; l < D.n_text_layer; ++l) {
        const LayerW &w = m->dec[l];
        f16 *kc = (f16 *)(f.kcache + (size_t)l * f.layer_stride), *vc = (f16 *)(f.vcache + (size_t)l * f.layer_stride);
        DecGemmArgs g{};
        g.M = rows; g.tall = 1; g.A = x; g.lda = d; g.W = m->A<f16>(w.wqkv_f); g.ldw = d; g.N = 3 * d; g.K = d; g.epi = DEC_LN | DEC_QKV;
        g.c1 = m->A<float>(w.qkv_c1); g.c2 = m->A<float>(w.qkv_c2); g.C = q; g.ldc = d;
        g.kcache = kc; g.vcache = vc; g.pos0 = f.pos0; g.n_ctx = D.n_text_ctx; g.d = d; g.rps = f.n_new; g.row_mul = f.row_mul;
        g.pf = pf_of(w.wo_p, d, d, DEC_RES);
        SWX_TRY(swx_gemm_dec(g, s));
        SelfAttnArgs sa{};
        sa.qkv = q; sa.ldqkv = d; sa.kcache = kc; sa.vcache = vc; sa.anc = f.anc; sa.pos0 = f.pos0; sa.o = att; sa.ldo = d;
        sa.R = R; sa.n_new = f.n_new; sa.H = H; sa.n_ctx = D.n_text_ctx; sa.d = d; sa.skip_append = 1;
        sa.pos0_all_zero = f.pos0 == m->Wp<int32_t>(m->L.zeros_i32) ? 1 : 0;
        SWX_TRY(swx_self_attention(m->dtype, sa, f.row_mul, s));
        g = DecGemmArgs{};
        g.M = rows; g.tall = 1; g.A = att; g.lda = d; g.W = m->A<f16>(w.wo_p); g.ldw = d; g.N = d; g.K = d; g.epi = DEC_RES;
        g.c2 = m->A<float>(w.bo); g.X = x; g.ldx = d;
        g.pf = pf_of(w.wcq_f, d, d, DEC_LN);
        SWX_TRY(swx_gemm_dec(g, s));
        g = DecGemmArgs{};
        g.M = rows; g.tall = 1; g.A = x; g.lda = d; g.W = m->A<f16>(w.wcq_f); g.ldw = d; g.N = d; g.K = d; g.epi = DEC_LN;
        g.c1 = m->A<float>(w.cq_c1); g.c2 = m->A<float>(w.cq_c2); g.C = q; g.ldc = d;
        g.pf = pf_of(w.wco_p, d, d, DEC_RES);
        SWX_TRY(swx_gemm_dec(g, s));
        if (f.qcap) {
            hipError_t qe = hipMemcpyAsync(f.qcap + (size_t)l * rows * d * e, q, (size_t)rows * d * e, hipMemcpyDeviceToDevice, s);
            if (qe != hipSuccess) return -100 - (int)qe;
        }
        const unsigned char *kl = f.xkv + (size_t)l * (f.xkv_W ? f.xkv_W : f.W) * chunk * e;
        AttnArgs ca{};
        ca.q = q; ca.ldq = d; ca.k = kl; ca.v = kl + (size_t)D.n_audio_ctx * d * e; ca.ldkv = d;
        ca.k_bs = chunk; ca.v_bs = chunk; ca.vt_kp = SWX_VT_KP; ca.o = att; ca.ldo = d;
        ca.B = f.W; ca.H = H; ca.nq = f.rpw * f.n_new; ca.nk = D.n_audio_ctx; ca.q_rows_per_batch = f.rpw * f.n_new;
        ca.kv_packed = kl + (size_t)xkv_plain_elems(D) * e;
        SWX_TRY(swx_attention(m->dtype, ca, 0, s));
        if (f.capture && !m->heads_by_layer[l].empty()) {
            SWX_TRY(swx_qk_capture(m->dtype, q, d, f.rpw * f.n_new, f.cap_row0, f.cap_rows, kl, d, chunk, D.n_audio_ctx,
                                   m->Wp<int32_t>(m->L.heads) + m->head_slot0[l], (int)m->heads_by_layer[l].size(),
                                   m->head_slot0[l], m->n_align, f.W, m->Wp<float>(m->L.cap), f.cap_ld_n, D.n_audio_ctx, s));
        }
        g = DecGemmArgs{};
        g.M = rows; g.tall = 1; g.A = att; g.lda = d; g.W = m->A<f16>(w.wco_p); g.ldw = d; g.N = d; g.K = d; g.epi = DEC_RES;
        g.c2 = m->A<float>(w.bco); g.X = x; g.ldx = d;
        g.pf = pf_of(w.w1_f, 4 * d, d, DEC_LN | DEC_GELU);
        SWX_TRY(swx_gemm_dec(g, s));
        g = DecGemmArgs{};
        g.M = rows; g.tall = 1; g.A = x; g.lda = d; g.W = m->A<f16>(w.w1_f); g.ldw = d; g.N = 4 * d; g.K = d; g.epi = DEC_LN | DEC_GELU;
        g.c1 = m->A<float>(w.w1_c1); g.c2 = m->A<float>(w.w1_c2); g.C = u; g.ldc = 4 * d;
        g.pf = pf_of(w.w2_p, d, 4 * d, DEC_RES | DEC_SLAB);
        SWX_TRY(swx_gemm_dec(g, s));
        g = DecGemmArgs{};
        g.M = rows; g.tall = 1; g.A = u; g.lda = 4 * d; g.W = m->A<f16>(w.w2_p); g.ldw = 4 * d; g.N = d; g.K = 4 * d; g.epi = DEC_RES | DEC_SLAB;
        g.c2 = m->A<float>(w.b2); g.X = x; g.ldx = d; g.slabs = slabs; g.ticket = m->Wp<int>(m->L.ticket);
        if (l + 1 < D.n_text_layer) g.pf = pf_of(m->dec[l + 1].wqkv_f, 3 * d, d, DEC_LN | DEC_QKV);
        SWX_TRY(swx_gemm_dec(g, s));
    }
    return 0;
}

int decoder_forward(swx_model *m, const FwdCfg &f, hipStream_t s)
{
    const bool dec_ok = m->dtype == SWX_F16 && m->is_folded() && !(g_debug_flags & SWX_FLAG_NO_FAST_STEP);
    const int64_t rows_all = (int64_t)f.W * f.rpw * f.n_new;
    if (dec_ok && f.n_new > 1 && (rows_all <= 160 || !(g_debug_flags & SWX_FLAG_SCORE_TILED)) && rows_all <= m->L.rows_big &&
        swx_dec_slab_floats((int)rows_all, m->dims.n_text_state, 4 * m->dims.n_text_state) * 4 <= m->L.slab_bytes)
        return decoder_forward_dec(m, f, s);
    if (dec_ok && f.n_new == 1 && f.row_mul == 1 && !f.capture && f.rpw <= 16 && m->dims.n_audio_ctx >= 128 &&
        (size_t)f.W * f.rpw <= (size_t)m->L.rows_big)
        return decoder_step_dec(m, f, s);
    const swx_dims &D = m->dims;
    const int d = D.n_text_state, H = D.n_text_head;
    const size_t e = m->esz;
    const int R = f.W * f.rpw;
    const int rows = R * f.n_new;
    if (rows > m->L.rows_big) return -8;
    unsigned char *x = m->ws + m->L.x, *h = m->ws + m->L.h, *qkv = m->ws + m->L.qkv, *att = m->ws + m->L.att, *u = m->ws + m->L.u;
    SWX_TRY(swx_embed(m->dtype, f.tokens, f.ld_tok, nullptr, f.pos0, R, f.n_new, m->arena + m->o_tok_emb,
                      m->A<float>(m->o_dec_pos), d, x, s));
    for (int l = 0; l < D.n_text_layer; ++l) {
        const LayerW &w = m->dec[l];
        SWX_TRY(swx_layernorm(m->dtype, x, d, m->A<float>(w.ln1_g), m->A<float>(w.ln1_b), h, d, rows, d, s));
        SWX_TRY(swx_gemm(m->dtype, gemm_args(h, d, m->arena + w.wqkv, d, m->A<float>(w.bqkv), qkv, 3 * d, rows, 3 * d, d, EPI_BIAS), 0, s));
        SelfAttnArgs sa{};
        sa.qkv = qkv; sa.ldqkv = 3 * d;
        sa.kcache = f.kcache + (size_t)l * f.layer_stride;
        sa.vcache = f.vcache + (size_t)l * f.layer_stride;
        sa.anc = f.anc; sa.pos0 = f.pos0; sa.o = att; sa.ldo = d;
        sa.R = R; sa.n_new = f.n_new; sa.H = H; sa.n_ctx = D.n_text_ctx; sa.d = d;
        sa.pos0_all_zero = f.pos0 == m->Wp<int32_t>(m->L.zeros_i32) ? 1 : 0;
        SWX_TRY(swx_self_attention(m->dtype, sa, f.row_mul, s));
        SWX_TRY(gemm_residual(m, att, d, w.wo, w.bo, x, d, rows, d, d, s));
        SWX_TRY(swx_layernorm(m->dtype, x, d, m->A<float>(w.lnx_g), m->A<float>(w.lnx_b), h, d, rows, d, s));
        SWX_TRY(swx_gemm(m->dtype, gemm_args(h, d, m->arena + w.wcq, d, m->A<float>(w.bcq), qkv, d, rows, d, d, EPI_BIAS), 0, s));
        if (f.qcap) {
            hipError_t qe = hipMemcpyAsync(f.qcap + (size_t)l * rows * d * e, qkv, (size_t)rows * d * e, hipMemcpyDeviceToDevice, s);
            if (qe != hipSuccess) return -100 - (int)qe;
        }
        const int64_t chunk = xkv_chunk_elems(m);
        const unsigned char *kl = f.xkv + (size_t)l * (f.xkv_W ? f.xkv_W : f.W) * chunk * e;
        AttnArgs ca{};
        ca.q = qkv; ca.ldq = d; ca.k = kl; ca.v = kl + (size_t)D.n_audio_ctx * d * e; ca.ldkv = d;
        ca.k_bs = chunk; ca.v_bs = chunk; ca.vt_kp = SWX_VT_KP; ca.o = att; ca.ldo = d;
        ca.B = f.W; ca.H = H; ca.nq = f.rpw * f.n_new; ca.nk = D.n_audio_ctx; ca.q_rows_per_batch = f.rpw * f.n_new;
        SWX_TRY(swx_attention(m->dtype, ca, 0, s));
        if (f.capture && !m->heads_by_layer[l].empty()) {
            SWX_TRY(swx_qk_capture(m->dtype, qkv, d, f.rpw * f.n_new, f.cap_row0, f.cap_rows, kl, d, chunk, D.n_audio_ctx,
                                   m->Wp<int32_t>(m->L.heads) + m->head_slot0[l], (int)m->heads_by_layer[l].size(),
                                   m->head_slot0[l], m->n_align, f.W, m->Wp<float>(m->L.cap), f.cap_ld_n, D.n_audio_ctx, s));
        }
        SWX_TRY(gemm_residual(m, att, d, w.wco, w.bco, x, d, rows, d, d, s));
        SWX_TRY(swx_layernorm(m->dtype, x, d, m->A<float>(w.ln2_g), m->A<float>(w.ln2_b), h, d, rows, d, s));
        SWX_TRY(swx_gemm(m->dtype, gemm_args(h, d, m->arena + w.w1, d, m->A<float>(w.b1), u, 4 * d, rows, 4 * d, d, EPI_BIAS | EPI_GELU), 0, s));
        SWX_TRY(gemm_residual(m, u, 4 * d, w.w2, w.b2, x, d, rows, d, 4 * d, s));
    }
    return 0;
}

int logits_gemm(swx_model *m, const void *hid, int64_t ld, int rows, float *out, hipStream_t s)
{
    const swx_dims &D = m->dims;
    return swx_gemm(m->dtype, gemm_args(hid, ld, m->arena + m->o_tok_emb, D.n_text_state, nullptr, out, D.n_vocab, rows,
                                        D.n_vocab, D.n_text_state, EPI_OUT_F32), 0, s);
}


template <typename F>
swx_model::StepGraph *step_graph(swx_model *m, const DecodeBufs &b, const void *d_xkv, int cur, F record)
{
    const swx_decode_cfg &c = b.cfg;
    uint32_t tbits, pbits;
    memcpy(&tbits, &c.temperature, 4); memcpy(&pbits, &c.patience, 4);
    std::vector<uint64_t> key = {
        (uint64_t)c.n_windows, (uint64_t)c.n_group, (uint64_t)c.beam, tbits, pbits, (uint64_t)c.sample_len, (uint64_t)c.sample_begin,
        (uint64_t)c.sot_index, (uint64_t)c.suppress_blank, (uint64_t)c.apply_timestamp_rules, (uint64_t)(int64_t)c.max_initial_timestamp_index,
        (uint64_t)c.eot, (uint64_t)c.sot, (uint64_t)(int64_t)c.no_timestamps, (uint64_t)c.timestamp_begin, (uint64_t)(int64_t)c.no_speech,
        (uint64_t)(int64_t)c.blank_token, (uint64_t)c.n_suppress, (uint64_t)c.min_tokens, (uint64_t)c.seed,
        (uint64_t)(uintptr_t)b.ts_mask, (uint64_t)(uintptr_t)b.win_uid, (uint64_t)(uintptr_t)d_xkv, (uint64_t)(uintptr_t)m->arena,
        (uint64_t)(uintptr_t)m->ws, (uint64_t)m->ws_bytes, (uint64_t)g_debug_flags, (uint64_t)cur, (uint64_t)m->is_folded(),
        (uint64_t)(uintptr_t)c.noise, (uint64_t)(uintptr_t)b.begin};
    ++m->graph_clock;
    for (auto &g : m->graphs) if (g.key == key) { g.used = m->graph_clock; return &g; }
    if (!m->cap_stream && hipStreamCreateWithFlags(&m->cap_stream, hipStreamNonBlocking) != hipSuccess) { m->cap_stream = nullptr; return nullptr; }
    swx_model::StepGraph ng;
    if (hipStreamBeginCapture(m->cap_stream, hipStreamCaptureModeThreadLocal) != hipSuccess) return nullptr;
    const int rc = record(m->cap_stream);
    hipError_t er = hipStreamEndCapture(m->cap_stream, &ng.graph);
    if (rc < 0 || er != hipSuccess || !ng.graph) { if (ng.graph) (void)hipGraphDestroy(ng.graph); return nullptr; }
    if (hipGraphInstantiate(&ng.exec, ng.graph, nullptr, nullptr, 0) != hipSuccess) { (void)hipGraphDestroy(ng.graph); return nullptr; }
    ng.key = std::move(key); ng.used = m->graph_clock;
    ++m->n_captures;
    constexpr size_t MAX_GRAPHS = 8;
    if (m->graphs.size() >= MAX_GRAPHS) {
        size_t lru = 0;
        for (size_t i = 1; i < m->graphs.size(); ++i) if (m->graphs[i].used < m->graphs[lru].used) lru = i;
        (void)hipGraphExecDestroy(m->graphs[lru].exec); (void)hipGraphDestroy(m->graphs[lru].graph);
        m->graphs[lru] = std::move(ng);
        return &m->graphs[lru];
    }
    m->graphs.push_back(std::move(ng));
    return &m->graphs.back();
}

template <bool RANK>
__global__ __launch_bounds__(256) void token_prob_kernel(const float *__restrict__ logits, int V, int n_used,
                                                         const int32_t *__restrict__ target_tok, float *__restrict__ out,
                                                         int32_t *__restrict__ rank)
{
    __shared__ float sh[4];
    __shared__ int shc[4];
    const int row = blockIdx.x, tid = threadIdx.x;
    const float *lg = logits + (size_t)row * V;
    int t = 0, below = 0;
    bool ok = false;
    float xt = 0.f;
    if constexpr (RANK) {
        t = target_tok[row];
        ok = t >= 0 && t < n_used;
        xt = ok ? lg[t] : 0.f;
    }
    float mx = -__builtin_inff();
    for (int i = tid; i < n_used; i += 256) {
        const float v = lg[i];
        mx = fmaxf(mx, v);
        if constexpr (RANK) below += (v < xt || (v == xt && i < t)) ? 1 : 0;
    }
    mx = wave_max(mx);
    if constexpr (RANK) {
        const int lane = tid & 63;
        below += lane_xor<32>(below, lane); below += lane_xor<16>(below, lane); below += lane_xor<8>(below, lane);
        below += lane_xor<4>(below, lane); below += lane_xor<2>(below, lane); below += lane_xor<1>(below, lane);
        if (lane == 0) shc[tid >> 6] = below;
    }
    if ((tid & 63) == 0) sh[tid >> 6] = mx;
    __syncthreads();
    mx = fmaxf(fmaxf(sh[0], sh[1]), fmaxf(sh[2], sh[3]));
    if constexpr (RANK) below = shc[0] + shc[1] + shc[2] + shc[3];
    __syncthreads();
    float sum = 0.f;
    for (int i = tid; i < n_used; i += 256) sum += expf(lg[i] - mx);
    sum = wave_sum(sum);
    if ((tid & 63) == 0) sh[tid >> 6] = sum;
    __syncthreads();
    sum = sh[0] + sh[1] + sh[2] + sh[3];
    if (tid == 0) {
        if constexpr (!RANK) t = target_tok[row];
        const bool in = t >= 0 && t < n_used;
        out[row] = in ? expf(lg[t] - mx) / sum : 0.f;
        if constexpr (RANK) rank[row] = in ? below : -1;
    }
}

__global__ void score_targets_kernel(const int32_t *__restrict__ tokens, int max_n, int n_sot, int rows_per_w,
                                     int32_t *__restrict__ targets, int total)
{
    const int idx = blockIdx.x * blockDim.x + threadIdx.x;
    if (idx >= total) return;
    const int w = idx / rows_per_w, i = idx % rows_per_w;
    const int p = n_sot + 1 + i;
    targets[idx] = (p < max_n) ? tokens[(size_t)w * max_n + p] : -1;
}

}

bool swx_prof_on() { return g_prof_enabled; }
int swx_flags() { return g_debug_flags; }
void swx_prof_begin(int cls, double work, hipStream_t s)
{
    ProfRec r{cls, work, prof_event(), prof_event()};
    if (!r.a || !r.b) return;
    (void)hipEventRecord(r.a, s);
    g_prof.push_back(r);
}
void swx_prof_end(hipStream_t s)
{
    if (!g_prof.empty()) (void)hipEventRecord(g_prof.back().b, s);
}

__global__ __launch_bounds__(64) void lane_xor_check_kernel(const uint32_t *__restrict__ in, uint32_t *__restrict__ out)
{
    const int lane = threadIdx.x;
    const uint32_t x = in[blockIdx.x * 64 + lane];
    uint32_t *o = out + (size_t)blockIdx.x * 13 * 64 + lane;
    o[0 * 64] = lane_xor_u32<32>(x, lane); o[1 * 64] = lane_xor_u32<16>(x, lane); o[2 * 64] = lane_xor_u32<8>(x, lane);
    o[3 * 64] = lane_xor_u32<4>(x, lane);  o[4 * 64] = lane_xor_u32<2>(x, lane);  o[5 * 64] = lane_xor_u32<1>(x, lane);
    o[6 * 64] = (uint32_t)__shfl_xor((int)x, 32, 64); o[7 * 64] = (uint32_t)__shfl_xor((int)x, 16, 64);
    o[8 * 64] = (uint32_t)__shfl_xor((int)x, 8, 64);  o[9 * 64] = (uint32_t)__shfl_xor((int)x, 4, 64);
    o[10 * 64] = (uint32_t)__shfl_xor((int)x, 2, 64); o[11 * 64] = (uint32_t)__shfl_xor((int)x, 1, 64);
    double v = (double)__uint_as_float(x);
    double ref = v;
#pragma unroll
    for (int off = 32; off > 0; off >>= 1) ref += __shfl_xor(ref, off, 64);
    const double got = wave_sum_d(v);
    unsigned ok = (__double_as_longlong(got) == __double_as_longlong(ref)) ? 1u : 0u;
    const float f = (float)(int)(x >> 9) * 1.1920929e-7f - 0.37f;
    ok |= (__float_as_uint(lane_xor16_max(f)) == __float_as_uint(fmaxf(f, __shfl_xor(f, 16, 64)))) ? 2u : 0u;
    ok |= (__float_as_uint(lane_xor32_max(f)) == __float_as_uint(fmaxf(f, __shfl_xor(f, 32, 64)))) ? 4u : 0u;
    ok |= (__float_as_uint(lane_xor16_add(f)) == __float_as_uint(f + __shfl_xor(f, 16, 64))) ? 8u : 0u;
    ok |= (__float_as_uint(lane_xor32_add(f)) == __float_as_uint(f + __shfl_xor(f, 32, 64))) ? 16u : 0u;
    float wm = f, ws = f;
#pragma unroll
    for (int off = 32; off > 0; off >>= 1) { wm = fmaxf(wm, __shfl_xor(wm, off, 64)); ws += __shfl_xor(ws, off, 64); }
    ok |= (__float_as_uint(wave_max(f)) == __float_as_uint(wm)) ? 32u : 0u;
    ok |= (__float_as_uint(wave_sum(f)) == __float_as_uint(ws)) ? 64u : 0u;
    o[12 * 64] = ok;
}

__global__ __launch_bounds__(256) void gelu_pair_check_kernel(unsigned long long *__restrict__ out)
{
    const unsigned base = (blockIdx.x * 256u + threadIdx.x) * 32u;
    unsigned bad = 0, nan_bits = 0, first = 0xffffffffu;
#pragma unroll 4
    for (unsigned j = 0; j < 32; j += 2) {
        const unsigned u0 = base + j, u1 = base + j + 1;
        const f32x2 x = {__uint_as_float(u0), __uint_as_float(u1)};
        const f32x2 got = gelu_erf2(x);
        const float r0 = gelu_erf(x[0]), r1 = gelu_erf(x[1]);
        const unsigned g0 = __float_as_uint(got[0]), g1 = __float_as_uint(got[1]), e0 = __float_as_uint(r0), e1 = __float_as_uint(r1);
        if (g0 != e0) { if (r0 != r0 && got[0] != got[0]) ++nan_bits; else { ++bad; first = first < u0 ? first : u0; } }
        if (g1 != e1) { if (r1 != r1 && got[1] != got[1]) ++nan_bits; else { ++bad; first = first < u1 ? first : u1; } }
    }
    if (bad) { atomicAdd(out, (unsigned long long)bad); atomicMin(out + 1, (unsigned long long)first); }
    if (nan_bits) atomicAdd(out + 2, (unsigned long long)nan_bits);
}

extern "C" {

int swx_debug_flags(int flags)
{
    const int old = g_debug_flags;
    if (flags >= 0) g_debug_flags = flags;
    return old;
}

int swx_prof_enable(int on)
{
    g_prof_enabled = on != 0;
    if (on) { g_prof.clear(); g_pool_next = 0; }
    return 0;
}

int swx_prof_collect(double *out, int n_classes)
{
    hipError_t e = hipDeviceSynchronize();
    if (e != hipSuccess) return -100 - (int)e;
    for (int i = 0; i < n_classes * 3; ++i) out[i] = 0.0;
    for (auto &r : g_prof) {
        if (r.cls < 0 || r.cls >= n_classes) continue;
        float ms = 0.f;
        if (hipEventElapsedTime(&ms, r.a, r.b) != hipSuccess) continue;
        out[r.cls * 3 + 0] += 1.0;
        out[r.cls * 3 + 1] += (double)ms;
        out[r.cls * 3 + 2] += r.work;
    }
    g_prof.clear();
    g_pool_next = 0;
    (void)hipGetLastError();
    return PC_COUNT;
}

const char *swx_strerror(int code)
{
    switch (code) {
        case 0: return "ok";
        case -1: return "invalid argument";
        case -2: return "size out of range";
        case -3: return "unsupported filter width";
        case -4: return "gemm shape/alignment not supported";
        case -5: return "attention shape not supported";
        case -7: return "not implemented";
        case -8: return "workspace too small for this call";
        case -9: return "weights / workspace not bound";
        case -10: return "unknown tensor name";
        case -11: return "tensor size mismatch";
        case -20: return "not a FLAC stream";
        case -21: return "corrupt FLAC stream (bad header, reserved code or CRC mismatch)";
        case -22: return "unsupported FLAC stream";
        case -23: return "truncated FLAC stream";
        default: return code <= -100 ? "HIP runtime error (code = -100 - hipError_t)" : "unknown error";
    }
}

int swx_version(void) { return 1; }

int swx_model_create(const swx_dims *dims, int dtype, swx_model **out)
{
    if (!dims || !out || (dtype != SWX_F32 && dtype != SWX_F16)) return -1;
    if (dims->n_audio_state % 64 || dims->n_text_state % 64) return -1;
    if (dims->n_audio_state / dims->n_audio_head != 64 || dims->n_text_state / dims->n_text_head != 64) return -1;
    if (dims->n_text_ctx > 448 || dims->n_audio_ctx > 1500) return -2;
    swx_model *m = new swx_model();
    m->dims = *dims;
    m->dtype = dtype;
    m->esz = dtype == SWX_F16 ? 2 : 4;
    build_layout(m);
    default_alignment_heads(m);
    upload_heads(m);
    *out = m;
    return 0;
}

void swx_model_destroy(swx_model *m) { delete m; }

size_t swx_weights_bytes(const swx_model *m) { return m ? m->arena_bytes : 0; }

int swx_bind_weights(swx_model *m, void *d_arena, size_t bytes)
{
    if (m) m->drop_graphs();
    if (!m || !d_arena || bytes < m->arena_bytes) return -1;
    m->arena = (unsigned char *)d_arena;
    hipError_t e = hipMemset(d_arena, 0, m->arena_bytes);
    if (e != hipSuccess) return -100 - (int)e;
    std::vector<double2> tw(SWX_N_FFT);
    for (int i = 0; i < SWX_N_FFT; ++i) {
        const double a = 2.0 * M_PI * (double)i / (double)SWX_N_FFT;
        tw[i].x = cos(a); tw[i].y = sin(a);
    }
    e = hipMemcpy(m->arena + m->o_twiddle, tw.data(), sizeof(double2) * SWX_N_FFT, hipMemcpyHostToDevice);
    if (e != hipSuccess) return -100 - (int)e;
    for (auto &kv : m->slots) kv.second.loaded = false;
    m->fold_state = std::make_shared<bool>(false);
    return upload_heads(m);
}

int swx_share_weights(swx_model *m, const swx_model *owner)
{
    if (!m || !owner || !owner->arena || m == owner) return -1;
    if (m->dtype != owner->dtype || m->arena_bytes != owner->arena_bytes || memcmp(&m->dims, &owner->dims, sizeof(swx_dims)) != 0)
        return -1;
    m->arena = owner->arena;
    m->fold_state = owner->fold_state;
    for (auto &kv : m->slots) {
        auto it = owner->slots.find(kv.first);
        kv.second.loaded = it != owner->slots.end() && it->second.loaded;
    }
    return upload_heads(m);
}

int swx_load_tensor(swx_model *m, const char *name, const float *d_src, int64_t numel, void *stream)
{
    if (!m || !m->arena) return -9;
    auto it = m->slots.find(name);
    if (it == m->slots.end()) return -10;
    Slot &sl = it->second;
    hipStream_t s = S(stream);
    if (sl.kind == SK_MAT) {
        if (numel != sl.rows * sl.cols) return -11;
        SWX_TRY(swx_copy_rows(m->dtype, d_src, sl.cols, m->arena + sl.off, sl.dst_ld, sl.rows, sl.cols, s));
    } else if (sl.kind == SK_CONV) {
        if (numel != sl.rows * sl.cols * 3) return -11;
        SWX_TRY(swx_copy_conv_w(m->dtype, d_src, (int)sl.rows, (int)sl.cols, (int)sl.dst_ld, m->arena + sl.off, s));
    } else {
        if (numel != sl.cols) return -11;
        hipError_t e = hipMemcpyAsync(m->arena + sl.off, d_src, (size_t)numel * 4, hipMemcpyDeviceToDevice, s);
        if (e != hipSuccess) return -100 - (int)e;
    }
    sl.loaded = true;
    *m->fold_state = false;
    return 0;
}

int swx_weights_complete(const swx_model *m)
{
    if (!m) return 0;
    for (auto &kv : m->slots) if (!kv.second.loaded) return 0;
    return 1;
}

int swx_weights_mark_loaded(swx_model *m)
{
    if (!m || !m->arena) return -9;
    for (auto &kv : m->slots) kv.second.loaded = true;
    return 0;
}

int swx_weights_finalize(swx_model *m, void *stream)
{
    if (!m || !m->arena) return -9;
    if (!m->has_fold) return 0;
    for (auto &kv : m->slots) if (!kv.second.loaded) return -9;
    hipStream_t s = S(stream);
    const int d = m->dims.n_text_state;
    for (auto &w : m->dec) {
        SWX_TRY(swx_fold_ln(m->arena + w.wqkv, m->A<float>(w.ln1_g), m->A<float>(w.ln1_b), m->A<float>(w.bqkv), m->arena + w.wqkv_f,
                            m->A<float>(w.qkv_c1), m->A<float>(w.qkv_c2), 3 * d, d, s));
        SWX_TRY(swx_fold_ln(m->arena + w.wcq, m->A<float>(w.lnx_g), m->A<float>(w.lnx_b), m->A<float>(w.bcq), m->arena + w.wcq_f,
                            m->A<float>(w.cq_c1), m->A<float>(w.cq_c2), d, d, s));
        SWX_TRY(swx_fold_ln(m->arena + w.w1, m->A<float>(w.ln2_g), m->A<float>(w.ln2_b), m->A<float>(w.b1), m->arena + w.w1_f,
                            m->A<float>(w.w1_c1), m->A<float>(w.w1_c2), 4 * d, d, s));
        SWX_TRY(swx_fold_ln(m->arena + w.wo, nullptr, nullptr, nullptr, m->arena + w.wo_p, nullptr, nullptr, d, d, s));
        SWX_TRY(swx_fold_ln(m->arena + w.wco, nullptr, nullptr, nullptr, m->arena + w.wco_p, nullptr, nullptr, d, d, s));
        SWX_TRY(swx_fold_ln(m->arena + w.w2, nullptr, nullptr, nullptr, m->arena + w.w2_p, nullptr, nullptr, d, 4 * d, s));
    }
    *m->fold_state = true;
    return 0;
}

int swx_missing_tensor(const swx_model *m, int index, char *buf, int buflen)
{
    int k = 0;
    for (auto &kv : m->slots)
        if (!kv.second.loaded) {
            if (k == index) { snprintf(buf, buflen, "%s", kv.first.c_str()); return 1; }
            ++k;
        }
    return 0;
}

int swx_set_alignment_heads(swx_model *m, const int32_t *pairs, int n_pairs)
{
    if (!m || (n_pairs > 0 && !pairs)) return -1;
    const swx_dims &D = m->dims;
    std::vector<std::vector<int>> by(D.n_text_layer);
    for (int i = 0; i < n_pairs; ++i) {
        const int l = pairs[2 * i], h = pairs[2 * i + 1];
        if (l < 0 || l >= D.n_text_layer || h < 0 || h >= D.n_text_head) return -1;
        by[l].push_back(h);
    }
    m->heads_by_layer = by;
    return upload_heads(m);
}

int swx_num_alignment_heads(const swx_model *m) { return m ? m->n_align : 0; }

size_t swx_workspace_bytes(const swx_model *m, int max_windows, int max_rows)
{
    if (!m || max_windows <= 0 || max_rows <= 0) return 0;
    swx_model::WsLayout L;
    ws_layout(m, max_windows, max_rows, m->n_align, L);
    return L.total;
}

int swx_bind_workspace(swx_model *m, void *d_ws, size_t bytes, int max_windows, int max_rows)
{
    if (m) m->drop_graphs();
    if (!m || !d_ws || max_windows <= 0 || max_rows <= 0) return -1;
    swx_model::WsLayout L;
    ws_layout(m, max_windows, max_rows, m->n_align, L);
    if (bytes < L.total) return -8;
    m->ws = (unsigned char *)d_ws;
    m->ws_bytes = bytes;
    m->max_windows = max_windows;
    m->max_rows = max_rows;
    m->ws_n_align = m->n_align;
    m->L = L;
    hipError_t e = hipMemset(m->ws + L.zeros_i32, 0, (size_t)(max_rows > max_windows ? max_rows : max_windows) * 4 + 256);
    if (e == hipSuccess) e = hipMemset(m->ws + L.ticket, 0, (size_t)SWX_DEC_TICKETS * 4);
    if (e != hipSuccess) return -100 - (int)e;
    if (!m->heads_flat.empty()) {
        e = hipMemcpy(m->ws + L.heads, m->heads_flat.data(), m->heads_flat.size() * 4, hipMemcpyHostToDevice);
        if (e != hipSuccess) return -100 - (int)e;
    }
    return 0;
}

int swx_log_mel(swx_model *m, const float *d_pcm, int B, float *d_mel, int per_item_max, void *stream)
{
    if (!m || !m->arena || !m->ws) return -9;
    if (B > m->max_windows) return -8;
    return swx_mel_launch(d_pcm, B, m->A<float>(m->o_hann), m->A<double2>(m->o_twiddle), m->A<float>(m->o_filters),
                          m->dims.n_mels, d_mel, m->Wp<unsigned>(m->L.gmax), per_item_max, S(stream));
}

int swx_log_mel_ragged_grouped(swx_model *m, const float *d_pcm, const int32_t *n_valid, const int32_t *n_total, int B,
                               float *d_mel, int group, void *stream)
{
    if (!m || !m->arena || !m->ws) return -9;
    if (B <= 0) return 0;
    if (B > m->max_windows) return -8;
    if (group <= 0 || B % group) return -1;
    if (!n_valid || !n_total) return -2;
    std::vector<int32_t> lens((size_t)B * 2);
    for (int b = 0; b < B; ++b) {
        if (n_total[b] <= 200 || n_total[b] / 160 > 3008 || n_valid[b] < 0 || n_valid[b] > n_total[b] ||
            n_valid[b] > 480000)
            return -2;
        lens[2 * b] = n_valid[b];
        lens[2 * b + 1] = n_total[b];
    }
    hipStream_t s = S(stream);
    int32_t *d_lens = m->Wp<int32_t>(m->L.h1);
    hipError_t e = hipMemcpyAsync(d_lens, lens.data(), lens.size() * 4, hipMemcpyHostToDevice, s);
    if (e == hipSuccess) e = hipStreamSynchronize(s);
    if (e != hipSuccess) return -100 - (int)e;
    return swx_mel_ragged_launch(d_pcm, d_lens, B, m->A<float>(m->o_hann), m->A<double2>(m->o_twiddle),
                                 m->A<float>(m->o_filters), m->dims.n_mels, d_mel, m->Wp<unsigned>(m->L.gmax), group, s);
}

int swx_log_mel_ragged(swx_model *m, const float *d_pcm, const int32_t *n_valid, const int32_t *n_total, int B,
                       float *d_mel, int per_item_max, void *stream)
{
    return swx_log_mel_ragged_grouped(m, d_pcm, n_valid, n_total, B, d_mel, per_item_max ? 1 : B, stream);
}

int swx_encode(swx_model *m, const float *d_mel, int B, void *d_xa, void *stream)
{
    if (!m || !m->arena || !m->ws) return -9;
    if (B <= 0) return 0;
    if (B > m->max_windows) return -8;
    const swx_dims &D = m->dims;
    const int d = D.n_audio_state, H = D.n_audio_head, S_ = D.n_audio_ctx;
    const size_t e = m->esz;
    hipStream_t s = S(stream);
    unsigned char *melT = m->ws + m->L.melT, *h1 = m->ws + m->L.h1;
    unsigned char *x = m->ws + m->L.x, *h = m->ws + m->L.h, *qkv = m->ws + m->L.qkv, *att = m->ws + m->L.att, *u = m->ws + m->L.u;
    const int rows = B * S_;
    if (D.n_audio_ctx != 1500) return -2;

    SWX_TRY(swx_mel_transpose(m->dtype, d_mel, B, D.n_mels, m->Cp, melT, s));
    SWX_TRY(swx_fill_zero(h1, (size_t)B * 3002 * d * e, s));
    for (int b = 0; b < B; ++b) {
        const unsigned char *a = melT + (size_t)b * 3002 * m->Cp * e;
        unsigned char *c = h1 + ((size_t)b * 3002 + 1) * d * e;
        SWX_TRY(swx_gemm(m->dtype, gemm_args(a, m->Cp, m->arena + m->o_conv1_w, 3 * m->Cp, m->A<float>(m->o_conv1_b), c, d,
                                             3000, d, 3 * m->Cp, EPI_BIAS | EPI_GELU), 0, s));
    }
    for (int b = 0; b < B; ++b) {
        const unsigned char *a = h1 + (size_t)b * 3002 * d * e;
        GemmArgs g = gemm_args(a, 2 * d, m->arena + m->o_conv2_w, 3 * d, m->A<float>(m->o_conv2_b), x + (size_t)b * S_ * d * e, d,
                               S_, d, 3 * d, EPI_BIAS | EPI_GELU | EPI_RESF32MOD);
        g.Rf = m->A<float>(m->o_enc_pos); g.res_mod = S_;
        SWX_TRY(swx_gemm(m->dtype, g, 0, s));
    }
    for (int l = 0; l < D.n_audio_layer; ++l) {
        const LayerW &w = m->enc[l];
        SWX_TRY(swx_layernorm(m->dtype, x, d, m->A<float>(w.ln1_g), m->A<float>(w.ln1_b), h, d, rows, d, s));
        const bool fuse_vt = m->dtype == SWX_F16 && d % 128 == 0 && S_ % 4 == 0 && !(g_debug_flags & SWX_FLAG_QKV_SEPARATE_VT) &&
                             swx_gemm_plan_f16(rows, 3 * d, d, EPI_BIAS, 3 * d, 1, true, 0, g_debug_flags) != SWX_GEMM_BIG;
        {
            GemmArgs gq = gemm_args(h, d, m->arena + w.wqkv, d, m->A<float>(w.bqkv), qkv, 3 * d, rows, 3 * d, d, EPI_BIAS | (fuse_vt ? EPI_QKV_VT : 0));
            if (fuse_vt) { gq.C2 = u; gq.vt_s = S_; gq.vt_kp = SWX_VT_KP; gq.vt_bs = (int64_t)H * 64 * SWX_VT_KP; gq.vt_zero_pad = 1; }
            SWX_TRY(swx_gemm(m->dtype, gq, 0, s));
        }
        AttnArgs a{};
        a.q = qkv; a.ldq = 3 * d; a.k = qkv + (size_t)d * e; a.v = qkv + (size_t)2 * d * e; a.ldkv = 3 * d; a.o = att; a.ldo = d;
        a.k_bs = (int64_t)S_ * 3 * d; a.v_bs = a.k_bs; a.vt_kp = 0;
        a.B = B; a.H = H; a.nq = S_; a.nk = S_; a.q_rows_per_batch = S_;
        if (m->dtype == SWX_F16) {
            if (!fuse_vt) SWX_TRY(swx_transpose_v(a.v, 3 * d, a.v_bs, S_, u, SWX_VT_KP, (int64_t)H * 64 * SWX_VT_KP, B, H, s));
            a.v = u; a.vt_kp = SWX_VT_KP; a.v_bs = (int64_t)H * 64 * SWX_VT_KP;
        }
        SWX_TRY(swx_attention(m->dtype, a, 0, s));
        SWX_TRY(gemm_residual(m, att, d, w.wo, w.bo, x, d, rows, d, d, s));
        SWX_TRY(swx_layernorm(m->dtype, x, d, m->A<float>(w.ln2_g), m->A<float>(w.ln2_b), h, d, rows, d, s));
        SWX_TRY(swx_gemm(m->dtype, gemm_args(h, d, m->arena + w.w1, d, m->A<float>(w.b1), u, 4 * d, rows, 4 * d, d, EPI_BIAS | EPI_GELU), 0, s));
        SWX_TRY(gemm_residual(m, u, 4 * d, w.w2, w.b2, x, d, rows, d, 4 * d, s));
    }
    SWX_TRY(swx_layernorm(m->dtype, x, d, m->A<float>(m->o_lnpost_g), m->A<float>(m->o_lnpost_b), d_xa, d, rows, d, s));
    return 0;
}

size_t swx_cross_kv_bytes(const swx_model *m, int B)
{
    if (!m) return 0;
    return (size_t)m->dims.n_text_layer * B * (size_t)xkv_chunk_elems(m) * m->esz;
}

int swx_cross_kv(swx_model *m, const void *d_xa, int B, void *d_xkv, void *stream)
{
    if (!m || !m->arena) return -9;
    const swx_dims &D = m->dims;
    const int d = D.n_text_state, S_ = D.n_audio_ctx;
    const size_t e = m->esz;
    if (D.n_audio_state != d) return -1;
    const int64_t chunk = xkv_chunk_elems(m);
    hipStream_t s = S(stream);
    SWX_TRY(swx_pad_zero((unsigned char *)d_xkv + (size_t)S_ * d * e, (int64_t)SWX_VT_KP * e, chunk * (int64_t)e, (int)(S_ * e),
                         (int)((SWX_VT_KP - S_) * e), d, D.n_text_layer * B, s));
    for (int l = 0; l < D.n_text_layer; ++l) {
        const LayerW &w = m->dec[l];
        unsigned char *base = (unsigned char *)d_xkv + (size_t)l * B * chunk * e;
        const bool one_launch = m->dtype == SWX_F16 && d % 128 == 0 && (int64_t)B * S_ > 128 && !(g_debug_flags & SWX_FLAG_XKV_TWO_LAUNCHES);
        bool packed_by_epilogue = false;
        if (one_launch) {
            GemmArgs gkv = gemm_args(d_xa, d, m->arena + w.wckv, d, m->A<float>(w.bckv), base, d, B * S_, 2 * d, d, EPI_BIAS | EPI_KV);
            gkv.vt_s = S_; gkv.vt_kp = SWX_VT_KP; gkv.vt_bs = chunk; gkv.C2 = base + (size_t)S_ * d * e;
            if (!(g_debug_flags & SWX_FLAG_XKV_PACK_SEPARATE)) {
                gkv.P = base + (size_t)xkv_plain_elems(D) * e; gkv.p_bs = chunk; gkv.p_nkpad = ((S_ + 31) / 32) * 32; gkv.p_vcol0 = d;
                packed_by_epilogue = true;
            }
            SWX_TRY(swx_gemm(m->dtype, gkv, 0, s));
        } else {
        GemmArgs gk = gemm_args(d_xa, d, m->arena + w.wckv, d, m->A<float>(w.bckv), base, d, B * S_, d, d, EPI_BIAS | EPI_CBATCH);
        gk.vt_s = S_; gk.vt_kp = 0; gk.vt_bs = chunk;
        SWX_TRY(swx_gemm(m->dtype, gk, 0, s));
        GemmArgs gv = gemm_args(d_xa, d, m->arena + w.wckv + (size_t)d * d * e, d, m->A<float>(w.bckv) + d,
                                base + (size_t)S_ * d * e, d, B * S_, d, d, EPI_BIAS | EPI_STORE_VT);
        gv.vt_s = S_; gv.vt_kp = SWX_VT_KP; gv.vt_bs = chunk;
        SWX_TRY(swx_gemm(m->dtype, gv, 0, s));
        }
        if (m->dtype == SWX_F16 && !packed_by_epilogue)
            SWX_TRY(swx_xkv_pack(base, base + (size_t)S_ * d * e, base + (size_t)xkv_plain_elems(D) * e, B, D.n_text_head, S_, d,
                                 SWX_VT_KP, chunk, s));
    }
    return 0;
}

namespace {
__global__ __launch_bounds__(64) void gather_rows_kernel(const unsigned char *__restrict__ src, const int32_t *__restrict__ idx,
                                                         unsigned char *__restrict__ dst, int row_bytes)
{
    const int j = blockIdx.x;
    const uint4 *sp = (const uint4 *)(src + (size_t)idx[j] * row_bytes);
    uint4 *dp = (uint4 *)(dst + (size_t)j * row_bytes);
    for (int i = threadIdx.x; i < row_bytes / 16; i += 64) dp[i] = sp[i];
}
}

int swx_decode_gout(const swx_decode_cfg *cfg)
{
    if (!cfg) return 0;
    if (!cfg->beam) return cfg->n_group;
    const float pat = cfg->patience > 0.f ? cfg->patience : 1.0f;
    const int mc = (int)lrintf((float)cfg->n_group * pat);
    return mc > cfg->n_group ? mc : cfg->n_group;
}

int swx_decode(swx_model *m, const swx_decode_cfg *cfg, const int32_t *d_init_tokens, const int32_t *d_suppress,
               const uint8_t *d_ts_mask, const void *d_xkv, int32_t *d_tokens_out, int32_t *d_lens_out,
               float *d_sumlp_out, float *d_nospeech, void *stream)
{
    if (!m || !m->arena || !m->ws) return -9;
    if (!cfg || !d_init_tokens || !d_xkv) return -1;
    const swx_dims &D = m->dims;
    const int W = cfg->n_windows, G = cfg->n_group, M = W * G;
    if (W <= 0 || G <= 0 || G > MAX_GROUP) return -1;
    if (W > m->max_windows || M > m->max_rows) return -8;
    if (cfg->n_suppress > MAX_SUPPRESS || cfg->n_suppress < 0) return -2;
    int n_init = cfg->sample_begin, sot_index = cfg->sot_index;
    std::vector<int32_t> nb, si;
    if (cfg->sample_begins || cfg->sot_indices) {
        nb.resize(W); si.resize(W);
        for (int w = 0; w < W; ++w) {
            nb[w] = cfg->sample_begins ? cfg->sample_begins[w] : cfg->sample_begin;
            si[w] = cfg->sot_indices ? cfg->sot_indices[w] : cfg->sot_index;
            if (nb[w] <= 0 || nb[w] > D.n_text_ctx || si[w] < 0 || si[w] >= nb[w]) return -1;
        }
        n_init = *std::max_element(nb.begin(), nb.end());
        sot_index = si[0];
    }
    const int n_min = nb.empty() ? n_init : *std::min_element(nb.begin(), nb.end());
    const bool ragged = !nb.empty() && (n_min != n_init || *std::min_element(si.begin(), si.end()) != *std::max_element(si.begin(), si.end()));
    if (n_init <= 0 || n_init > D.n_text_ctx || sot_index < 0 || sot_index >= n_init) return -1;
    hipStream_t s = S(stream);
    const int d = D.n_text_state;
    const size_t e = m->esz;

    DecodeBufs b{};
    b.cfg = *cfg;
    b.cfg.sample_begin = n_init; b.cfg.sot_index = sot_index;
    b.cfg.sample_begins = nullptr; b.cfg.sot_indices = nullptr;
    if (cfg->beam || cfg->temperature == 0.f) b.cfg.noise = nullptr;
    b.W = W; b.G = G; b.M = M; b.V = D.n_vocab; b.TS = D.n_text_ctx + 1; b.n_ctx = D.n_text_ctx; b.n_init = n_init;
    const float pat = cfg->patience > 0.f ? cfg->patience : 1.0f;
    b.max_cand = cfg->beam ? (int)lrintf((float)G * pat) : 0;
    if (cfg->beam && (b.max_cand <= 0 || b.max_cand > FIN_CAP)) return -2;
    b.fin_cap = FIN_CAP;
    b.tokens[0] = m->Wp<int32_t>(m->L.tokens0); b.tokens[1] = m->Wp<int32_t>(m->L.tokens1);
    const bool use_anc = G > 1;
    b.anc[0] = use_anc ? m->Wp<int32_t>(m->L.anc0) : nullptr;
    b.anc[1] = use_anc ? m->Wp<int32_t>(m->L.anc1) : nullptr;
    b.pos0 = m->Wp<int32_t>(m->L.pos0);
    b.sum_lp = m->Wp<float>(m->L.sum_lp); b.sum_lp_next = m->Wp<float>(m->L.sum_lp_next);
    b.row_done = m->Wp<int32_t>(m->L.row_done);
    b.win_done = m->Wp<int32_t>(m->L.win_done); b.win_done_prev = m->Wp<int32_t>(m->L.win_done_prev);
    b.n_done = m->Wp<int32_t>(m->L.n_done);
    b.step_dev = b.n_done + 1;
    b.fin_tokens = m->Wp<int32_t>(m->L.fin_tokens); b.fin_score = m->Wp<float>(m->L.fin_score);
    b.fin_len = m->Wp<int32_t>(m->L.fin_len); b.fin_count = m->Wp<int32_t>(m->L.fin_count);
    b.cand_lp = m->Wp<float>(m->L.cand_lp); b.cand_tok = m->Wp<int32_t>(m->L.cand_tok);
    b.logits = m->Wp<float>(m->L.logits);
    b.ts_mask = d_ts_mask;
    int32_t *sup = m->Wp<int32_t>(m->L.suppress);
    if (cfg->n_suppress > 0) {
        hipError_t er = hipMemcpyAsync(sup, d_suppress, (size_t)cfg->n_suppress * 4, hipMemcpyDeviceToDevice, s);
        if (er != hipSuccess) return -100 - (int)er;
    }
    b.suppress = sup;
    for (int t : {cfg->eot, cfg->sot, cfg->timestamp_begin}) if (t < 0 || t >= D.n_vocab) return -2;
    for (int t : {cfg->no_timestamps, cfg->no_speech, cfg->blank_token}) if (t < -1 || t >= D.n_vocab) return -2;
    b.win_uid = nullptr;
    if (cfg->window_uid) {
        int32_t *d_uid = m->Wp<int32_t>(m->L.win_uid);
        hipError_t eu = hipMemcpyAsync(d_uid, cfg->window_uid, (size_t)W * 4, hipMemcpyHostToDevice, s);
        if (eu == hipSuccess) eu = hipStreamSynchronize(s);
        if (eu != hipSuccess) return -100 - (int)eu;
        b.win_uid = d_uid;
    }
    b.cfg.window_uid = nullptr;
    auto kind = [](int n) { return n == 1 ? 0 : n <= 16 ? 1 : 2; };
    struct Run { int w0, w1, n_new; };
    std::vector<Run> runs;
    int32_t *d_pre_rows = nullptr;
    if (ragged) {
        std::vector<int32_t> &hv = m->ragged_hv;
        hv.assign(3 * (size_t)W, 0);
        for (int w0 = 0; w0 < W; ) {
            int w1 = w0 + 1, n_new = nb[w0];
            while (w1 < W && kind(nb[w1]) == kind(nb[w0])) { n_new = std::max(n_new, (int)nb[w1]); ++w1; }
            runs.push_back({w0, w1, n_new});
            for (int w = w0; w < w1; ++w) {
                hv[w] = nb[w];
                hv[W + 2 * w] = (w - w0) * n_new + si[w];
                hv[W + 2 * w + 1] = (w - w0) * n_new + nb[w] - 1;
            }
            w0 = w1;
        }
        int32_t *d_begin = m->Wp<int32_t>(m->L.win_begin);
        hipError_t eb = hipMemcpyAsync(d_begin, hv.data(), hv.size() * 4, hipMemcpyHostToDevice, s);
        if (eb != hipSuccess) return -100 - (int)eb;
        b.begin = d_begin;
        d_pre_rows = d_begin + W;
    }
    hipError_t er = hipMemsetAsync(b.win_done_prev, 0, (size_t)W * 4, s);
    if (er != hipSuccess) return -100 - (int)er;

    SWX_TRY(swx_decode_init(b, d_init_tokens, s));

    const size_t layer_stride = (size_t)m->max_rows * D.n_text_ctx * d * e;
    if (g_debug_flags & SWX_FLAG_TICKET) {
        hipError_t e_ = hipMemsetAsync(m->ws + m->L.ticket, 0, (size_t)SWX_DEC_TICKETS * 4, s);
        if (e_ != hipSuccess) return -100 - (int)e_;
    }
    FwdCfg f{};
    f.W = W; f.rpw = 1; f.row_mul = G; f.n_new = n_init;
    f.tokens = b.tokens[0]; f.ld_tok = (int64_t)G * b.TS;
    f.pos0 = m->Wp<int32_t>(m->L.zeros_i32);
    f.kcache = m->ws + m->L.kcache; f.vcache = m->ws + m->L.vcache; f.layer_stride = layer_stride; f.cache_rows = m->max_rows;
    f.anc = nullptr; f.xkv = (const unsigned char *)d_xkv; f.capture = false;
    unsigned char *x = m->ws + m->L.x, *hid2 = m->ws + m->L.hid2;
    float *lg2 = b.logits + (size_t)(m->L.logits_rows - 2 * W) * D.n_vocab;
    if (!ragged) {
        SWX_TRY(decoder_forward(m, f, s));
        SWX_TRY(swx_layernorm(m->dtype, x + (size_t)sot_index * d * e, (int64_t)n_init * d, m->A<float>(m->o_ln_g),
                              m->A<float>(m->o_ln_b), hid2, 2 * d, W, d, s));
        SWX_TRY(swx_layernorm(m->dtype, x + (size_t)(n_init - 1) * d * e, (int64_t)n_init * d, m->A<float>(m->o_ln_g),
                              m->A<float>(m->o_ln_b), hid2 + (size_t)d * e, 2 * d, W, d, s));
    } else {
        unsigned char *park = (unsigned char *)(((uintptr_t)lg2 + 255) & ~(uintptr_t)255);
        const size_t win_xkv = (size_t)xkv_chunk_elems(m) * e, win_cache = (size_t)G * D.n_text_ctx * d * e;
        for (const Run &r : runs) {
            FwdCfg fr = f;
            fr.W = r.w1 - r.w0; fr.n_new = r.n_new; fr.xkv_W = W;
            fr.tokens = f.tokens + (size_t)r.w0 * f.ld_tok;
            fr.kcache = f.kcache + r.w0 * win_cache; fr.vcache = f.vcache + r.w0 * win_cache;
            fr.xkv = f.xkv + r.w0 * win_xkv;
            SWX_TRY(decoder_forward(m, fr, s));
            hipLaunchKernelGGL(gather_rows_kernel, dim3(2 * fr.W), dim3(64), 0, s, x, d_pre_rows + 2 * r.w0,
                               park + (size_t)2 * r.w0 * d * e, (int)(d * e));
            SWX_CHECK_LAUNCH();
        }
        SWX_TRY(swx_layernorm(m->dtype, park, d, m->A<float>(m->o_ln_g), m->A<float>(m->o_ln_b), hid2, d, 2 * W, d, s));
    }
    SWX_TRY(logits_gemm(m, hid2, d, 2 * W, lg2, s));
    SWX_TRY(swx_decode_after_prefill(b, lg2, d_nospeech, s));

    int cur = 0, steps = 0;
    int32_t h_done = 0;
    const int CHECK = 8;
    auto unit = [&](int cur_in, hipStream_t st, bool capturing = false) -> int {
        FwdCfg g{};
        g.W = W; g.rpw = G; g.row_mul = 1; g.n_new = 1;
        g.tokens = b.tokens[cur_in]; g.ld_tok = b.TS; g.pos0 = b.pos0;
        g.kcache = f.kcache; g.vcache = f.vcache; g.layer_stride = layer_stride; g.cache_rows = m->max_rows;
        g.anc = use_anc ? b.anc[cur_in] : nullptr; g.xkv = (const unsigned char *)d_xkv; g.capture = false;
        g.step_pos = capturing ? 0 : n_init + steps;
        g.pos_bound = n_init + cfg->sample_len;
        const int fr = decoder_forward(m, g, st);
        if (fr < 0) return fr;
        unsigned char *hh = m->ws + m->L.h;
        if (fr == 0)
            SWX_TRY(swx_layernorm(m->dtype, x, d, m->A<float>(m->o_ln_g), m->A<float>(m->o_ln_b), hh, d, M, d, st));
        SWX_TRY(logits_gemm(m, hh, d, M, b.logits, st));
        return swx_decode_select(b, cur_in, st);
    };
    auto after_select = [&](int i) -> int {
        steps = i + 1;
        if (n_min + i + 1 > D.n_text_ctx) return 1;
        if ((steps % CHECK == 0 && steps >= cfg->min_tokens) || steps == cfg->sample_len) {
            er = hipMemcpyAsync(&h_done, b.n_done, 4, hipMemcpyDeviceToHost, s);
            if (er != hipSuccess) return -100 - (int)er;
            er = hipStreamSynchronize(s);
            if (er != hipSuccess) return -100 - (int)er;
            if (h_done >= W) return 1;
        }
        return i + 1 >= cfg->sample_len ? 1 : 0;
    };
    SWX_TRY(swx_decode_select(b, cur, s));
    if (cfg->beam) cur ^= 1;
    int stop = after_select(0);
    if (stop < 0) return stop;
    const bool graph_ok = !g_prof_enabled && !(g_debug_flags & SWX_FLAG_NO_GRAPH) && !m->graphs_off;
    swx_model::StepGraph *sg = nullptr;
    bool graph_failed_now = false;
    for (int i = 1; !stop; ) {
        const bool pair = graph_ok && !m->graphs_off && !graph_failed_now && i >= 2 && (i & 1) == 0 && i + 1 < cfg->sample_len && n_min + i + 1 <= D.n_text_ctx;
        if (pair) {
            if (!sg) sg = step_graph(m, b, d_xkv, cur, [&](hipStream_t cs) -> int {
                SWX_TRY(unit(cur, cs, true));
                return unit(cfg->beam ? cur ^ 1 : cur, cs, true);
            });
            if (sg && hipGraphLaunch(sg->exec, s) == hipSuccess) {
                ++m->n_replays;
                stop = after_select(i + 1);
                if (stop < 0) return stop;
                i += 2;
                continue;
            }
            (void)hipGetLastError();
            graph_failed_now = true;
            if (++m->graph_failures >= 3) m->graphs_off = true;
            if (m->graph_failures == 1)
                fprintf(stderr, "libswx: decode-step graph capture / replay failed; launching the steps eagerly (results are identical)\n");
        }
        SWX_TRY(unit(cur, s));
        ++m->n_eager_units;
        if (cfg->beam) cur ^= 1;
        stop = after_select(i);
        if (stop < 0) return stop;
        ++i;
    }
    const int G_out = swx_decode_gout(cfg);
    SWX_TRY(swx_decode_finalize(b, cur, steps, d_tokens_out, d_lens_out, d_sumlp_out, G_out, s));
    er = hipStreamSynchronize(s);
    if (er != hipSuccess) return -100 - (int)er;
    return steps;
}

static int score_forward(swx_model *m, const int32_t *d_tokens, const int32_t *h_n_tok, int W, int max_n, int cap_row0,
                         int cap_rows, int cap_ld, const void *d_xkv, bool capture, hipStream_t s, void *qcap = nullptr)
{
    const swx_dims &D = m->dims;
    if (W > m->max_windows) return -8;
    if (max_n <= 0 || max_n > D.n_text_ctx) return -2;
    for (int w = 0; w < W; ++w) if (h_n_tok[w] > max_n || h_n_tok[w] <= 0) return -1;
    FwdCfg f{};
    f.W = W; f.rpw = 1; f.row_mul = 1; f.n_new = max_n;
    f.tokens = d_tokens; f.ld_tok = max_n;
    f.pos0 = m->Wp<int32_t>(m->L.zeros_i32);
    f.kcache = m->ws + m->L.sk; f.vcache = m->ws + m->L.sv; f.layer_stride = 0; f.cache_rows = m->max_windows;
    f.anc = nullptr; f.xkv = (const unsigned char *)d_xkv;
    f.capture = capture;
    f.qcap = (unsigned char *)qcap;
    f.cap_row0 = cap_row0; f.cap_rows = cap_rows; f.cap_ld_n = cap_ld;
    if (capture && (cap_rows <= 0 || cap_row0 < 0 || cap_row0 + cap_rows > max_n || cap_ld < cap_rows)) return -1;
    return decoder_forward(m, f, s);
}

static int score_token_probs(swx_model *m, const int32_t *d_tokens, int W, int max_n, int n_sot, int eot, float *d_token_probs,
                             hipStream_t s)
{
    const swx_dims &D = m->dims;
    const int d = D.n_text_state;
    const size_t e = m->esz;
    unsigned char *x = m->ws + m->L.x, *hh = m->ws + m->L.h;
    const int rows = W * max_n;
    SWX_TRY(swx_layernorm(m->dtype, x, d, m->A<float>(m->o_ln_g), m->A<float>(m->o_ln_b), hh, d, rows, d, s));
    const int rpw = max_n - n_sot - 2;
    if (rpw > 0) {
        float *lg = m->Wp<float>(m->L.logits);
        int32_t *targets = (int32_t *)(m->ws + m->L.att);
        const int total = W * rpw;
        hipLaunchKernelGGL(score_targets_kernel, dim3(cdiv(total, 256)), dim3(256), 0, s, d_tokens, max_n, n_sot, rpw, targets, total);
        const int chunk = (int)m->L.logits_rows;
        for (int w = 0; w < W; ++w) {
            for (int r0 = 0; r0 < rpw; r0 += chunk) {
                const int nr = (rpw - r0) < chunk ? (rpw - r0) : chunk;
                const unsigned char *hid = hh + ((size_t)w * max_n + n_sot + r0) * d * e;
                SWX_TRY(logits_gemm(m, hid, d, nr, lg, s));
                hipLaunchKernelGGL(token_prob_kernel<false>, dim3(nr), dim3(256), 0, s, lg, D.n_vocab, eot, targets + (size_t)w * rpw + r0,
                                   d_token_probs + (size_t)w * max_n + r0, (int32_t *)nullptr);
            }
        }
        SWX_CHECK_LAUNCH();
    }
    return 0;
}

int swx_score(swx_model *m, const int32_t *d_tokens, const int32_t *h_n_tok, int W, int max_n, int n_sot, int eot,
              const int32_t *h_n_frames, float qk_scale, int medfilt_width, const void *d_xkv, float *d_token_probs,
              float *d_neg_matrix, void *stream)
{
    if (!m || !m->arena || !m->ws) return -9;
    if (W <= 0) return 0;
    if (m->n_align != m->ws_n_align || m->n_align <= 0) return -8;
    if (2 * W + 16 > SMALL_I32) return -8;
    const swx_dims &D = m->dims;
    hipStream_t s = S(stream);
    SWX_TRY(score_forward(m, d_tokens, h_n_tok, W, max_n, n_sot, max_n - n_sot - 1, max_n, d_xkv, true, s));

    std::vector<int32_t> hv(2 * W);
    for (int w = 0; w < W; ++w) {
        const int T = h_n_tok[w] - n_sot - 2;
        if (T < 0) return -1;
        hv[w] = T + 1;
        int F = h_n_frames[w];
        if (F < 1) F = 1;
        if (F > D.n_audio_ctx) F = D.n_audio_ctx;
        hv[W + w] = F;
    }
    int32_t *d_small = m->Wp<int32_t>(m->L.small_i32);
    hipError_t er = hipMemcpyAsync(d_small, hv.data(), hv.size() * 4, hipMemcpyHostToDevice, s);
    if (er != hipSuccess) return -100 - (int)er;
    er = hipStreamSynchronize(s);
    if (er != hipSuccess) return -100 - (int)er;

    SWX_TRY(score_token_probs(m, d_tokens, W, max_n, n_sot, eot, d_token_probs, s));
    SWX_TRY(swx_align_weights_launch(m->Wp<float>(m->L.cap), m->Wp<float>(m->L.mean), m->Wp<float>(m->L.mean), m->Wp<float>(m->L.sd),
                                     W, m->n_align, max_n, D.n_audio_ctx, d_small, d_small + W, qk_scale, medfilt_width,
                                     d_neg_matrix, max_n, D.n_audio_ctx, s));
    return 0;
}

int swx_score_qk(swx_model *m, const int32_t *d_tokens, const int32_t *h_n_tok, int W, int max_n, int n_sot, int eot,
                 int row0, int n_rows, const void *d_xkv, float *d_token_probs, float *d_qk, void *stream)
{
    if (!m || !m->arena || !m->ws) return -9;
    if (W <= 0) return 0;
    if (m->n_align != m->ws_n_align || m->n_align <= 0) return -8;
    if (!d_qk) return -1;
    for (int w = 0; w < W; ++w) if (h_n_tok[w] - n_sot - 2 < 0) return -1;
    hipStream_t s = S(stream);
    SWX_TRY(score_forward(m, d_tokens, h_n_tok, W, max_n, row0, n_rows, n_rows, d_xkv, true, s));
    if (d_token_probs) SWX_TRY(score_token_probs(m, d_tokens, W, max_n, n_sot, eot, d_token_probs, s));
    const size_t bytes = (size_t)W * m->n_align * n_rows * m->dims.n_audio_ctx * sizeof(float);
    hipError_t er = hipMemcpyAsync(d_qk, m->Wp<float>(m->L.cap), bytes, hipMemcpyDeviceToDevice, s);
    return er == hipSuccess ? 0 : -100 - (int)er;
}

int swx_forward_logits(swx_model *m, const int32_t *d_tokens, const int32_t *h_n_tok, int W, int max_n, const void *d_xkv,
                       float *d_logits, void *stream)
{
    if (!m || !m->arena || !m->ws) return -9;
    if (W <= 0) return 0;
    const swx_dims &D = m->dims;
    hipStream_t s = S(stream);
    const int d = D.n_text_state;
    SWX_TRY(score_forward(m, d_tokens, h_n_tok, W, max_n, 0, 0, max_n, d_xkv, false, s));
    unsigned char *x = m->ws + m->L.x, *hh = m->ws + m->L.h;
    const int rows = W * max_n;
    SWX_TRY(swx_layernorm(m->dtype, x, d, m->A<float>(m->o_ln_g), m->A<float>(m->o_ln_b), hh, d, rows, d, s));
    return logits_gemm(m, hh, d, rows, d_logits, s);
}

int swx_forward_token_ranks(swx_model *m, const int32_t *d_tokens, const int32_t *h_n_tok, int W, int max_n, int n_vocab_used,
                            const void *d_xkv, float *d_prob, int32_t *d_rank, void *stream)
{
    if (!m || !m->arena || !m->ws) return -9;
    if (W <= 0) return 0;
    if (!d_tokens || !h_n_tok || !d_prob || !d_rank) return -1;
    const swx_dims &D = m->dims;
    if (n_vocab_used <= 0 || n_vocab_used > D.n_vocab) return -1;
    hipStream_t s = S(stream);
    const int d = D.n_text_state;
    const size_t e = m->esz;
    SWX_TRY(score_forward(m, d_tokens, h_n_tok, W, max_n, 0, 0, max_n, d_xkv, false, s));
    unsigned char *x = m->ws + m->L.x, *hh = m->ws + m->L.h;
    SWX_TRY(swx_layernorm(m->dtype, x, d, m->A<float>(m->o_ln_g), m->A<float>(m->o_ln_b), hh, d, W * max_n, d, s));
    float *lg = m->Wp<float>(m->L.logits);
    const int chunk = 64;
    for (int w = 0; w < W; ++w) {
        const int rows = h_n_tok[w] - 1;
        for (int r0 = 0; r0 < rows; r0 += chunk) {
            const int nr = (rows - r0) < chunk ? (rows - r0) : chunk;
            const size_t at = (size_t)w * max_n + r0;
            SWX_TRY(logits_gemm(m, hh + at * d * e, d, nr, lg, s));
            hipLaunchKernelGGL(token_prob_kernel<true>, dim3(nr), dim3(256), 0, s, lg, D.n_vocab, n_vocab_used, d_tokens + at + 1,
                               d_prob + at, d_rank + at);
            SWX_CHECK_LAUNCH();
        }
    }
    return 0;
}

size_t swx_qcap_bytes(const swx_model *m, int max_n)
{
    if (!m || max_n <= 0) return 0;
    return (size_t)m->dims.n_text_layer * max_n * m->dims.n_text_state * m->esz;
}

int swx_score_q(swx_model *m, const int32_t *d_tokens, const int32_t *h_n_tok, int max_n, int n_sot, int eot, const void *d_xkv,
                float *d_token_probs, void *d_q, void *stream)
{
    if (!m || !m->arena || !m->ws) return -9;
    if (!d_q || !d_tokens || !h_n_tok) return -1;
    if (h_n_tok[0] - n_sot - 2 < 0) return -1;
    hipStream_t s = S(stream);
    SWX_TRY(score_forward(m, d_tokens, h_n_tok, 1, max_n, 0, 0, max_n, d_xkv, false, s, d_q));
    if (d_token_probs) SWX_TRY(score_token_probs(m, d_tokens, 1, max_n, n_sot, eot, d_token_probs, s));
    return 0;
}

size_t swx_heads_scratch_bytes(const swx_model *m, int max_n)
{
    if (!m || max_n <= 0) return 0;
    const size_t LH = (size_t)m->dims.n_text_layer * m->dims.n_text_head;
    return align_up(LH * max_n * sizeof(double)) + align_up(LH * max_n * sizeof(int32_t)) + align_up(LH * SWX_HS_MAXF * sizeof(float)) +
           align_up(LH * sizeof(float)) + align_up(LH * sizeof(int32_t));
}

int swx_heads_dynamic(swx_model *m, const void *d_q, int max_n, int row0, int n_rows, const void *d_xkv, int n_frames, float qk_scale,
                      int count, const double *d_peaks, float *d_qk_sel, int ld_f, void *d_scratch, size_t scratch_bytes, void *stream)
{
    if (!m || !m->arena) return -9;
    if (!d_q || !d_xkv || !d_qk_sel || !d_scratch) return -1;
    if (row0 < 0 || n_rows <= 0 || row0 + n_rows > max_n || ld_f < m->dims.n_audio_ctx) return -1;
    if (scratch_bytes < swx_heads_scratch_bytes(m, max_n)) return -8;
    const swx_dims &D = m->dims;
    const size_t LH = (size_t)D.n_text_layer * D.n_text_head;
    unsigned char *p = (unsigned char *)d_scratch;
    double *score = (double *)p; p += align_up(LH * max_n * sizeof(double));
    int32_t *sel = (int32_t *)p;
    int F = n_frames < 1 ? 1 : (n_frames > D.n_audio_ctx ? D.n_audio_ctx : n_frames);
    return swx_headsel_dynamic_launch(m->dtype, d_q, max_n, D.n_text_state, row0, n_rows, d_xkv, xkv_chunk_elems(m), D.n_text_layer,
                                      D.n_text_head, F, D.n_audio_ctx, qk_scale, count, d_peaks, score, sel, d_qk_sel, ld_f, S(stream));
}

int swx_heads_new(swx_model *m, const void *d_q, int max_n, int n_tok, int row0, int n_out, const void *d_xkv, int n_frames,
                  float qk_scale, int medfilt_width, int topk, float w_colnorm, float w_rownorm, float w_coverage,
                  float *d_neg_matrix, int ld_f, void *d_scratch, size_t scratch_bytes, void *stream)
{
    if (!m || !m->arena) return -9;
    if (!d_q || !d_xkv || !d_neg_matrix || !d_scratch) return -1;
    if (n_tok <= 0 || n_tok > max_n) return -1;
    if (scratch_bytes < swx_heads_scratch_bytes(m, max_n)) return -8;
    const swx_dims &D = m->dims;
    const size_t LH = (size_t)D.n_text_layer * D.n_text_head;
    unsigned char *p = (unsigned char *)d_scratch;
    p += align_up(LH * max_n * sizeof(double)) + align_up(LH * max_n * sizeof(int32_t));
    float *colnorm = (float *)p; p += align_up(LH * SWX_HS_MAXF * sizeof(float));
    float *score = (float *)p; p += align_up(LH * sizeof(float));
    int32_t *top = (int32_t *)p;
    int F = n_frames < 1 ? 1 : (n_frames > D.n_audio_ctx ? D.n_audio_ctx : n_frames);
    return swx_headsel_new_launch(m->dtype, d_q, max_n, D.n_text_state, n_tok, row0, n_out, d_xkv, xkv_chunk_elems(m), D.n_text_layer,
                                  D.n_text_head, F, qk_scale, medfilt_width, topk, w_colnorm, w_rownorm, w_coverage, colnorm, score, top,
                                  d_neg_matrix, ld_f, S(stream));
}

int swx_weighted_sum(const float *const *h_xs, const float *h_coef, int n_in, float *d_out, int64_t n, void *stream)
{
    if (!h_xs || !h_coef || !d_out) return -1;
    return swx_weighted_sum_launch(h_xs, h_coef, n_in, d_out, n, S(stream));
}

int swx_graph_stats(const swx_model *m, int64_t *out)
{
    if (!m || !out) return -1;
    out[0] = m->n_captures; out[1] = m->n_replays; out[2] = m->n_eager_units; out[3] = (m->graphs_off || m->graph_failures > 0) ? 1 : 0;
    return 0;
}

size_t swx_align_weights_scratch_bytes(int W, int H, int N)
{
    if (W <= 0 || H <= 0 || N <= 0) return 0;
    return align_up((size_t)W * H * N * sizeof(float2)) + align_up((size_t)2 * W * sizeof(int32_t));
}

int swx_align_weights(const float *d_qk, int W, int H, int N, int ld_f, const int32_t *h_n_frames, float qk_scale,
                      int medfilt_width, float *d_neg_matrix, void *d_scratch, size_t scratch_bytes, void *stream)
{
    if (W <= 0) return 0;
    if (!d_scratch || scratch_bytes < swx_align_weights_scratch_bytes(W, H, N)) return -8;
    hipStream_t s = S(stream);
    float *rstat = (float *)d_scratch;
    int32_t *cnt = (int32_t *)((unsigned char *)d_scratch + align_up((size_t)W * H * N * sizeof(float2)));
    std::vector<int32_t> hv(2 * W);
    for (int w = 0; w < W; ++w) { hv[w] = N; hv[W + w] = h_n_frames[w]; }
    hipError_t er = hipMemcpyAsync(cnt, hv.data(), hv.size() * 4, hipMemcpyHostToDevice, s);
    if (er == hipSuccess) er = hipStreamSynchronize(s);
    if (er != hipSuccess) return -100 - (int)er;
    return swx_align_weights_launch(d_qk, rstat, nullptr, nullptr, W, H, N, ld_f, cnt, cnt + W, qk_scale, medfilt_width, d_neg_matrix,
                                    N, ld_f, s);
}

int swx_test_gemm(int dtype, const void *d_a, int64_t lda, const void *d_w, const float *d_bias, const void *d_res,
                  void *d_c, int64_t ldc, int M, int N, int K, int epilogue, int force_kernel, void *stream)
{
    GemmArgs g = gemm_args(d_a, lda, d_w, K, d_bias, d_c, ldc, M, N, K, epilogue);
    g.R = d_res; g.ldr = ldc;
    return swx_gemm(dtype, g, force_kernel, S(stream));
}

int swx_test_gemm_plan(int M, int N, int K, int epilogue, int force_kernel, int flags)
{
    return swx_gemm_plan_f16(M, N, K, epilogue, N, N, true, force_kernel, flags);
}

int swx_test_dec_gemm(const void *d_a, int64_t lda, const void *d_w, const float *d_gamma, const float *d_beta, const float *d_bias,
                      void *d_c, int64_t ldc, void *d_x, void *d_kcache, void *d_vcache, const int32_t *d_pos0, int n_ctx, int d,
                      int M, int N, int K, int epilogue, void *d_scratch, size_t scratch_bytes, void *stream)
{
    hipStream_t s = S(stream);
    unsigned char *p = (unsigned char *)d_scratch;
    const size_t slab_b = align_up(swx_dec_slab_floats(M, N, K) * 4 + 256);
    const size_t need = align_up((size_t)N * K * 2) + 2 * align_up((size_t)N * 4) + slab_b + (size_t)SWX_DEC_TICKETS * 4;
    if (scratch_bytes < need) return -8;
    f16 *wf = (f16 *)p; p += align_up((size_t)N * K * 2);
    float *c1 = (float *)p; p += align_up((size_t)N * 4);
    float *c2 = (float *)p; p += align_up((size_t)N * 4);
    float *slabs = (float *)p; p += slab_b;
    int *ticket = (int *)p;
    if (!(epilogue & 128)) { hipError_t e = hipMemsetAsync(ticket, 0, (size_t)SWX_DEC_TICKETS * 4, s); if (e != hipSuccess) return -100 - (int)e; }
    DecGemmArgs g{};
    g.A = (const f16 *)d_a; g.lda = lda; g.M = M; g.N = N; g.K = K; g.epi = epilogue; g.ldw = K;
    g.C = (f16 *)d_c; g.ldc = ldc; g.X = (f16 *)d_x; g.ldx = ldc; g.slabs = slabs; g.ticket = ticket;
    g.kcache = (f16 *)d_kcache; g.vcache = (f16 *)d_vcache; g.pos0 = d_pos0; g.n_ctx = n_ctx; g.d = d;
    g.epi = epilogue & 31;
    g.tall = (epilogue & 64) ? 1 : 0;
    g.rps = (epilogue & 64) && (epilogue & DEC_QKV) ? 7 : 0;
    if ((epilogue & DEC_LN) && (epilogue & 32)) {
        g.W = (const f16 *)d_w; g.c1 = d_gamma; g.c2 = d_beta;
    } else if (epilogue & DEC_LN) {
        SWX_TRY(swx_fold_ln(d_w, d_gamma, d_beta, d_bias, wf, c1, c2, N, K, s));
        g.W = wf; g.c1 = c1; g.c2 = c2;
    } else if (epilogue & 32) {
        g.W = (const f16 *)d_w; g.c2 = d_bias;
    } else {
        SWX_TRY(swx_fold_ln(d_w, nullptr, nullptr, nullptr, wf, nullptr, nullptr, N, K, s));
        g.W = wf; g.c2 = d_bias;
    }
    return swx_gemm_dec(g, s);
}

int swx_test_self_attn_step(const void *d_q, void *d_kcache, void *d_vcache, const int32_t *d_anc, const int32_t *d_pos0,
                            int R, int H, int n_ctx, int d, int variant, void *d_o, void *stream)
{
    SelfAttnArgs sa{};
    sa.qkv = d_q; sa.ldqkv = d; sa.kcache = d_kcache; sa.vcache = d_vcache; sa.anc = (int32_t *)d_anc; sa.pos0 = d_pos0;
    sa.o = d_o; sa.ldo = d; sa.R = R; sa.n_new = 1; sa.H = H; sa.n_ctx = n_ctx; sa.d = d; sa.skip_append = 1;
    sa.step_cached = variant < 2 ? 1 : 0;
    sa.pos_bound = variant == 0 ? 128 : 0;
    return swx_self_attention(SWX_F16, sa, 1, S(stream));
}

int swx_test_self_attn_multi(const void *d_q, void *d_kcache, void *d_vcache, int R, int H, int n_new, int n_ctx, int d, int mq,
                             void *d_o, void *stream)
{
    static int32_t *d_zeros = nullptr;
    static int zeros_n = 0;
    if (R <= 0 || n_new <= 0 || n_new > n_ctx) return -2;
    if (zeros_n < R) {
        if (d_zeros) (void)hipFree(d_zeros);
        zeros_n = 0; d_zeros = nullptr;
        if (hipMalloc((void **)&d_zeros, (size_t)R * 4) != hipSuccess) return -3;
        zeros_n = R;
    }
    hipError_t e = hipMemsetAsync(d_zeros, 0, (size_t)R * 4, S(stream));
    if (e != hipSuccess) return -100 - (int)e;
    SelfAttnArgs sa{};
    sa.qkv = d_q; sa.ldqkv = d; sa.kcache = d_kcache; sa.vcache = d_vcache; sa.anc = nullptr; sa.pos0 = d_zeros;
    sa.o = d_o; sa.ldo = d; sa.R = R; sa.n_new = n_new; sa.H = H; sa.n_ctx = n_ctx; sa.d = d; sa.skip_append = 1;
    sa.pos0_all_zero = mq ? 1 : 0;
    return swx_self_attention(SWX_F16, sa, 1, S(stream));
}

int swx_test_layernorm(int dtype, const void *d_x, const float *d_g, const float *d_b, void *d_y, int rows, int d, void *stream)
{
    return swx_layernorm(dtype, d_x, d, d_g, d_b, d_y, d, rows, d, S(stream));
}

int swx_test_attention(int dtype, const void *d_q, int64_t ldq, const void *d_k, const void *d_v, int64_t ldkv, void *d_o,
                       int64_t ldo, int B, int H, int nq, int nk, int force_kernel, int vt_kp, void *stream)
{
    AttnArgs a{};
    a.q = d_q; a.ldq = ldq; a.k = d_k; a.v = d_v; a.ldkv = ldkv; a.o = d_o; a.ldo = ldo;
    a.k_bs = (int64_t)nk * ldkv; a.vt_kp = vt_kp;
    a.v_bs = vt_kp ? (int64_t)H * 64 * vt_kp : (int64_t)nk * ldkv;
    a.B = B; a.H = H; a.nq = nq; a.nk = nk; a.q_rows_per_batch = nq;
    return swx_attention(dtype, a, force_kernel, S(stream));
}

int swx_test_lane_xor(const uint32_t *d_in, uint32_t *d_out, int n_waves, void *stream)
{
    if (!d_in || !d_out || n_waves <= 0) return -1;
    hipLaunchKernelGGL(lane_xor_check_kernel, dim3(n_waves), dim3(64), 0, S(stream), d_in, d_out);
    SWX_CHECK_LAUNCH();
    return 0;
}

int swx_test_gelu_pair(uint64_t *d_out, void *stream)
{
    if (!d_out) return -1;
    hipStream_t s = S(stream);
    const unsigned long long init[3] = {0ull, 0xffffffffull, 0ull};
    hipError_t e = hipMemcpyAsync(d_out, init, sizeof(init), hipMemcpyHostToDevice, s);
    if (e == hipSuccess) e = hipStreamSynchronize(s);
    if (e != hipSuccess) return -100 - (int)e;
    hipLaunchKernelGGL(gelu_pair_check_kernel, dim3(1u << 19), dim3(256), 0, s, (unsigned long long *)d_out);
    SWX_CHECK_LAUNCH();
    return 0;
}

}
```

Measured before the change: 1409 x real time.

## Fuse decode step tail into one advance kernel and precompute suppress bitmask

Merges beam update, the window-finish/step-counter kernel and the next-step token embedding into one per-window advance kernel. A last-arriver atomic ticket replaces the separate single-block finish reduction. Suppressed tokens are precomputed once into a per-thread register-slot bitmask, so the select kernel no longer writes -inf into logits rows each step. This removes kernel launches and global stores per decode step, at the cost of atomic-ticket coordination. It also adds a test entry point and a flag bit-uniqueness check, and moves DEC_W1_FULL_TILE to a new bit value.

```diff
diff --git a/include/swx.h b/include/swx.h
--- a/include/swx.h
+++ b/include/swx.h
@@ -139,6 +139,11 @@
                       const float *d_bias, void *d_c, int64_t ldc, void *d_x, void *d_kcache, void *d_vcache,
                       const int32_t *d_pos0, int n_ctx, int d, int M, int N, int K, int epilogue, void *d_scratch,
                       size_t scratch_bytes, void *stream);
+#define SWX_TAIL_N_FIELDS 17
+int64_t swx_test_decode_tail_layout(const swx_decode_cfg *cfg, int n_vocab, int n_ctx, int d, int dtype, int64_t *h_offsets);
+int swx_test_decode_tail(const swx_decode_cfg *cfg, const int32_t *d_init_tokens, const int32_t *d_suppress,
+                         const uint8_t *d_ts_mask, int n_vocab, int n_ctx, int d, int dtype, const float *d_logits, int n_steps,
+                         const void *d_tok_emb, const float *d_pos_emb, void *d_work, void *d_state_out, void *stream);
 int swx_test_layernorm(int dtype, const void *d_x, const float *d_g, const float *d_b, void *d_y, int rows, int d,
                        void *stream);
 int swx_test_attention(int dtype, const void *d_q, int64_t ldq, const void *d_k, const void *d_v, int64_t ldkv,
diff --git a/stable_ts_amd/_lib.py b/stable_ts_amd/_lib.py
--- a/stable_ts_amd/_lib.py
+++ b/stable_ts_amd/_lib.py
@@ -101,6 +101,9 @@
                                         c_void_p]),
     "swx_test_self_attn_multi": (c_int, [c_void_p, c_void_p, c_void_p, c_int, c_int, c_int, c_int, c_int, c_int, c_void_p, c_void_p]),
     "swx_test_gelu_pair": (c_int, [c_void_p, c_void_p]),
+    "swx_test_decode_tail_layout": (c_int64, [POINTER(swx_decode_cfg), c_int, c_int, c_int, c_int, POINTER(c_int64)]),
+    "swx_test_decode_tail": (c_int, [POINTER(swx_decode_cfg), c_void_p, c_void_p, c_void_p, c_int, c_int, c_int, c_int, c_void_p,
+                                     c_int, c_void_p, c_void_p, c_void_p, c_void_p, c_void_p]),
     "swx_test_lane_xor": (c_int, [c_void_p, c_void_p, c_int, c_void_p]),
     "swx_test_layernorm": (c_int, [c_int, c_void_p, c_void_p, c_void_p, c_void_p, c_int, c_int, c_void_p]),
     "swx_test_attention": (c_int, [c_int, c_void_p, c_int64, c_void_p, c_void_p, c_int64, c_void_p, c_int64, c_int,
diff --git a/stable_ts_amd/csrc/swx_common.h b/stable_ts_amd/csrc/swx_common.h
--- a/stable_ts_amd/csrc/swx_common.h
+++ b/stable_ts_amd/csrc/swx_common.h
@@ -22,6 +22,15 @@
 template <typename T> __device__ __forceinline__ T from_f32(float v);
 template <> __device__ __forceinline__ float from_f32<float>(float v) { return v; }
 template <> __device__ __forceinline__ f16 from_f32<f16>(float v) { return (f16)v; }
+
+template <typename T>
+__device__ __forceinline__ void embed_row(const T *__restrict__ tok_emb, const float *__restrict__ pos_emb, int tok, int pos, int d,
+                                          T *__restrict__ o, int tid, int nthreads)
+{
+    const T *e = tok_emb + (size_t)tok * d;
+    const float *pe = pos_emb + (size_t)pos * d;
+    for (int c = tid; c < d; c += nthreads) o[c] = from_f32<T>(to_f32<T>(e[c]) + pe[c]);
+}
 
 template <typename T> __device__ __forceinline__ void load8(const T *p, float (&o)[8]);
 template <> __device__ __forceinline__ void load8<f16>(const f16 *p, float (&o)[8]) {
diff --git a/stable_ts_amd/csrc/swx_decode.h b/stable_ts_amd/csrc/swx_decode.h
--- a/stable_ts_amd/csrc/swx_decode.h
+++ b/stable_ts_amd/csrc/swx_decode.h
@@ -24,8 +24,14 @@
     int32_t *cand_tok;
     float *logits;
     const int32_t *suppress;
+    unsigned long long *sup_mask;
     const uint8_t *ts_mask;
     const int32_t *win_uid;
+    const void *emb_tok;
+    const float *emb_pos;
+    void *emb_x;
+    int emb_d, emb_f16;
+    int32_t *adv_ticket;
 };
 
 int swx_decode_init(const DecodeBufs &b, const int32_t *init_tokens, hipStream_t s);
diff --git a/stable_ts_amd/csrc/swx_decode.hip b/stable_ts_amd/csrc/swx_decode.hip
--- a/stable_ts_amd/csrc/swx_decode.hip
+++ b/stable_ts_amd/csrc/swx_decode.hip
@@ -108,7 +108,7 @@
         b.sum_lp[r] = 0.f;
         b.row_done[r] = 0;
         if (r % b.G == 0) { b.win_done[w] = 0; b.fin_count[w] = 0; }
-        if (r == 0) { *b.n_done = 0; *b.step_dev = 0; }
+        if (r == 0) { *b.n_done = 0; *b.step_dev = 0; if (b.adv_ticket) *b.adv_ticket = 0; }
     }
 }
 
@@ -262,9 +262,22 @@
     }
 }
 
-template <int NV>
+__global__ __launch_bounds__(SEL_T) void decode_suppress_mask_kernel(DecodeBufs b, unsigned long long *__restrict__ mask)
+{
+    static_assert(SEL_T == 1 << 10, "slot = token >> 10");
+    const int tid = threadIdx.x;
+    unsigned long long m = 0;
+    for (int i = 0; i < b.cfg.n_suppress; ++i) {
+        const int t = b.suppress[i];
+        if ((unsigned)t < (unsigned)b.V && (t & (SEL_T - 1)) == tid && (t >> 10) < 64) m |= 1ull << (t >> 10);
+    }
+    mask[tid] = m;
+}
+
+template <int NV, bool ROW_STORES>
 __global__ __launch_bounds__(SEL_T) void decode_select_reg_kernel(DecodeBufs b, int cur)
 {
+    static_assert(NV <= 64, "point suppressions: one mask bit per register slot");
     const int step = *b.step_dev;
     __shared__ __attribute__((aligned(16))) float shf[SEL_T / 64];
     __shared__ __attribute__((aligned(16))) ArgMax sha[SEL_T / 64];
@@ -281,15 +294,29 @@
     const int nsamp = step;
     const int tsb = c.timestamp_begin;
 
-    if (c.suppress_blank && nsamp == 0 && tid == 0) { if (c.blank_token >= 0) lg[c.blank_token] = NEG_INF; lg[c.eot] = NEG_INF; }
-    for (int i = tid; i < c.n_suppress; i += SEL_T) { const int t = b.suppress[i]; if ((unsigned)t < (unsigned)V) lg[t] = NEG_INF; }
-    if (c.min_tokens > 0 && nsamp < c.min_tokens && tid == 0) lg[c.eot] = NEG_INF;
-    if (c.apply_timestamp_rules && tid == 0) { sh_last_ts = -1; if (c.no_timestamps >= 0) lg[c.no_timestamps] = NEG_INF; }
+    unsigned long long pm = 0;
+    if constexpr (ROW_STORES) {
+        if (c.suppress_blank && nsamp == 0 && tid == 0) { if (c.blank_token >= 0) lg[c.blank_token] = NEG_INF; lg[c.eot] = NEG_INF; }
+        for (int i = tid; i < c.n_suppress; i += SEL_T) { const int t = b.suppress[i]; if ((unsigned)t < (unsigned)V) lg[t] = NEG_INF; }
+        if (c.min_tokens > 0 && nsamp < c.min_tokens && tid == 0) lg[c.eot] = NEG_INF;
+        if (c.apply_timestamp_rules && tid == 0) { sh_last_ts = -1; if (c.no_timestamps >= 0) lg[c.no_timestamps] = NEG_INF; }
+    } else {
+        if (c.n_suppress > 0) pm = b.sup_mask[tid];
+        auto point = [&](int t) { if ((t & (SEL_T - 1)) == tid && (unsigned)t < (unsigned)V) pm |= 1ull << (t >> 10); };
+        if (c.suppress_blank && nsamp == 0) { if (c.blank_token >= 0) point(c.blank_token); point(c.eot); }
+        if (c.min_tokens > 0 && nsamp < c.min_tokens) point(c.eot);
+        if (c.apply_timestamp_rules) { if (tid == 0) sh_last_ts = -1; if (c.no_timestamps >= 0) point(c.no_timestamps); }
+    }
     __syncthreads();
 
     float v[NV];
 #pragma unroll
     for (int k = 0; k < NV; ++k) { const int i = tid + k * SEL_T; v[k] = i < V ? lg[i] : NEG_INF; }
+    if constexpr (!ROW_STORES) {
+        const unsigned pm_lo = (unsigned)pm, pm_hi = (unsigned)(pm >> 32);
+#pragma unroll
+        for (int k = 0; k < NV; ++k) if ((k < 32 ? pm_lo >> k : pm_hi >> (k - 32)) & 1u) v[k] = NEG_INF;
+    }
 
     if (c.apply_timestamp_rules) {
         int my = -1;
@@ -420,9 +447,8 @@
     }
 }
 
-__global__ __launch_bounds__(256) void decode_beam_update_kernel(DecodeBufs b, int cur)
-{
-    const int step = *b.step_dev;
+__device__ __forceinline__ void beam_update_window(const DecodeBufs &b, int cur, int w, int step)
+{
     constexpr int MAXC = 17 * 16;
     __shared__ float sc[MAXC];
     __shared__ short src[MAXC];
@@ -430,7 +456,7 @@
     __shared__ short order[MAXC];
     __shared__ int sel_src[16], sel_tok[16];
     __shared__ float sel_sc[16];
-    const int w = blockIdx.x, G = b.G, K = G + 1, tid = threadIdx.x;
+    const int G = b.G, K = G + 1, tid = threadIdx.x;
     const swx_decode_cfg &c = b.cfg;
     __shared__ int s_frozen;
     if (tid == 0) s_frozen = b.win_done[w];
@@ -503,6 +529,48 @@
     }
 }
 
+__global__ __launch_bounds__(256) void decode_beam_update_kernel(DecodeBufs b, int cur)
+{
+    beam_update_window(b, cur, blockIdx.x, *b.step_dev);
+}
+
+__device__ __forceinline__ int window_finish(const DecodeBufs &b, int w, int step)
+{
+    int done = b.win_done[w];
+    if (!b.cfg.beam && !done) {
+        int all = 1;
+        for (int g = 0; g < b.G; ++g) all &= b.row_done[w * b.G + g];
+        if (all) { b.win_done[w] = 1; done = 1; }
+    }
+    if (b.begin && !done && b.begin[w] + step + 1 > b.n_ctx) { b.win_done[w] = 1; done = 1; }
+    b.win_done_prev[w] = done;
+    return done;
+}
+
+template <typename T>
+__global__ __launch_bounds__(256) void decode_advance_kernel(DecodeBufs b, int cur)
+{
+    const int step = *b.step_dev;
+    const int w = blockIdx.x, tid = threadIdx.x, G = b.G;
+    if (b.cfg.beam) beam_update_window(b, cur, w, step);
+    __syncthreads();
+    if (tid == 0) {
+        const int done = window_finish(b, w, step);
+        const unsigned old = __hip_atomic_fetch_add((unsigned *)b.adv_ticket, 1u + ((unsigned)done << 16), __ATOMIC_RELAXED,
+                                                    __HIP_MEMORY_SCOPE_AGENT);
+        if ((int)(old & 0xffffu) == b.W - 1) {
+            __hip_atomic_store((unsigned *)b.adv_ticket, 0u, __ATOMIC_RELAXED, __HIP_MEMORY_SCOPE_AGENT);
+            *b.n_done = (int)(old >> 16) + done;
+            *b.step_dev = step + 1;
+        }
+    }
+    const int32_t *tokens = b.tokens[b.cfg.beam ? cur ^ 1 : cur];
+    for (int g = 0; g < G; ++g) {
+        const int r = w * G + g, p = b.pos0[r];
+        embed_row<T>((const T *)b.emb_tok, b.emb_pos, tokens[(size_t)r * b.TS + p], p, b.emb_d, (T *)b.emb_x + (size_t)r * b.emb_d, tid, 256);
+    }
+}
+
 __global__ __launch_bounds__(64) void decode_step_finish_kernel(DecodeBufs b)
 {
     if (blockIdx.x != 0) return;
@@ -510,15 +578,7 @@
     const int step = *b.step_dev;
     int nd = 0;
     for (int w = lane; w < b.W; w += 64) {
-        int done = b.win_done[w];
-        if (!b.cfg.beam && !done) {
-            int all = 1;
-            for (int g = 0; g < b.G; ++g) all &= b.row_done[w * b.G + g];
-            if (all) { b.win_done[w] = 1; done = 1; }
-        }
-        if (b.begin && !done && b.begin[w] + step + 1 > b.n_ctx) { b.win_done[w] = 1; done = 1; }
-        b.win_done_prev[w] = done;
-        nd += done ? 1 : 0;
+        nd += window_finish(b, w, step);
     }
     nd += lane_xor<32>(nd, lane); nd += lane_xor<16>(nd, lane); nd += lane_xor<8>(nd, lane);
     nd += lane_xor<4>(nd, lane); nd += lane_xor<2>(nd, lane); nd += lane_xor<1>(nd, lane);
@@ -594,13 +654,14 @@
 int swx_decode_init(const DecodeBufs &b, const int32_t *init_tokens, hipStream_t s)
 {
     hipLaunchKernelGGL(decode_init_kernel, dim3(b.M), dim3(256), 0, s, b, init_tokens);
+    if (b.sup_mask) hipLaunchKernelGGL(decode_suppress_mask_kernel, dim3(1), dim3(SEL_T), 0, s, b, b.sup_mask);
     SWX_CHECK_LAUNCH();
     return 0;
 }
 int swx_decode_after_prefill(const DecodeBufs &b, const float *lg2, float *nospeech, hipStream_t s)
 {
     hipLaunchKernelGGL(decode_after_prefill_kernel, dim3(b.M), dim3(256), 0, s, b);
-    hipLaunchKernelGGL(decode_prefill_logits_kernel, dim3(b.M), dim3(SEL_T), 0, s, b, lg2, nospeech);
+    if (lg2) hipLaunchKernelGGL(decode_prefill_logits_kernel, dim3(b.M), dim3(SEL_T), 0, s, b, lg2, nospeech);
     SWX_CHECK_LAUNCH();
     return 0;
 }
@@ -608,10 +669,21 @@
 {
     SwxProfScope prof(PC_SELECT, (double)b.M * b.V * 4.0, s);
     const bool mem_kernel = swx_flags() & SWX_FLAG_SELECT_MEM;
-    if (!mem_kernel && b.V <= 51 * SEL_T)
-        hipLaunchKernelGGL(decode_select_reg_kernel<51>, dim3(b.M), dim3(SEL_T), 0, s, b, cur);
+    if (!mem_kernel && b.V <= 51 * SEL_T) {
+        if (!b.sup_mask || (swx_flags() & SWX_FLAG_SELECT_ROW_STORES))
+            hipLaunchKernelGGL((decode_select_reg_kernel<51, true>), dim3(b.M), dim3(SEL_T), 0, s, b, cur);
+        else
+            hipLaunchKernelGGL((decode_select_reg_kernel<51, false>), dim3(b.M), dim3(SEL_T), 0, s, b, cur);
+    }
     else
         hipLaunchKernelGGL(decode_select_kernel, dim3(b.M), dim3(SEL_T), 0, s, b, cur);
+    if (b.emb_x) {
+        if (!b.adv_ticket || !b.emb_tok || !b.emb_pos || b.W > 0x7fff) return -1;
+        if (b.emb_f16) hipLaunchKernelGGL(decode_advance_kernel<f16>, dim3(b.W), dim3(256), 0, s, b, cur);
+        else hipLaunchKernelGGL(decode_advance_kernel<float>, dim3(b.W), dim3(256), 0, s, b, cur);
+        SWX_CHECK_LAUNCH();
+        return 0;
+    }
     if (b.cfg.beam) {
         hipLaunchKernelGGL(decode_beam_update_kernel, dim3(b.W), dim3(256), 0, s, b, cur);
     }
diff --git a/stable_ts_amd/csrc/swx_kernels.h b/stable_ts_amd/csrc/swx_kernels.h
--- a/stable_ts_amd/csrc/swx_kernels.h
+++ b/stable_ts_amd/csrc/swx_kernels.h
@@ -58,10 +58,25 @@
 #define SWX_FLAG_SELFATTN_NO_MQ 256
 #define SWX_FLAG_FLASH_NO_QB1 64
 #define SWX_FLAG_XKV_PACK_SEPARATE 128
-#define SWX_FLAG_DEC_W1_FULL_TILE 256
+#define SWX_FLAG_DEC_W1_FULL_TILE 1024
 #define SWX_FLAG_XQ_FULL_TILE 512
 #define SWX_FLAG_NO_BIG_TILE 131072
+#define SWX_FLAG_TAIL_3LAUNCH 4096
+#define SWX_FLAG_SELECT_ROW_STORES 8
 #define SWX_DEFAULT_FLAGS 0
+namespace swx_flag_check {
+constexpr unsigned all[] = {
+    SWX_FLAG_NO_FAST_STEP, SWX_FLAG_NO_PACKED_XKV, SWX_FLAG_SELECT_MEM, SWX_FLAG_NO_GRAPH, SWX_FLAG_NO_PREFETCH, SWX_FLAG_NO_RING,
+    SWX_FLAG_SCORE_TILED, SWX_FLAG_NO_TALL, SWX_FLAG_NO_FUSED_XQ, SWX_FLAG_TICKET, SWX_FLAG_BIG8_GROUPED, SWX_FLAG_XKV_TWO_LAUNCHES,
+    SWX_FLAG_LOUDNESS_ONE_WG, SWX_FLAG_XATTN_R5, SWX_FLAG_FLASH_PIPELINED, SWX_FLAG_SELFATTN_WG5, SWX_FLAG_QKV_SEPARATE_VT,
+    SWX_FLAG_SELFATTN_NO_DEEP, SWX_FLAG_DEC_NO_W1, SWX_FLAG_TALL_NO_W8, SWX_FLAG_SELFATTN_NO_MQ, SWX_FLAG_FLASH_NO_QB1,
+    SWX_FLAG_XKV_PACK_SEPARATE, SWX_FLAG_DEC_W1_FULL_TILE, SWX_FLAG_XQ_FULL_TILE, SWX_FLAG_NO_BIG_TILE, SWX_FLAG_TAIL_3LAUNCH,
+    SWX_FLAG_SELECT_ROW_STORES};
+constexpr bool single_bits() { for (unsigned f : all) if (f == 0 || (f & (f - 1)) != 0 || f > 0x40000000u) return false; return true; }
+constexpr bool distinct() { unsigned seen = 0; for (unsigned f : all) { if (seen & f) return false; seen |= f; } return true; }
+static_assert(single_bits(), "every SWX_FLAG_* is a single bit of a non-negative int");
+static_assert(distinct(), "two SWX_FLAG_* share a bit");
+}
 int swx_flags();
 
 #define DEC_LN 1
diff --git a/stable_ts_amd/csrc/swx_norm.hip b/stable_ts_amd/csrc/swx_norm.hip
--- a/stable_ts_amd/csrc/swx_norm.hip
+++ b/stable_ts_amd/csrc/swx_norm.hip
@@ -71,10 +71,7 @@
     const int r = blockIdx.y, i = blockIdx.x;
     const int p = pos0[r] + i;
     const int tok = tokens[(size_t)r * ld_tok + p];
-    const T *e = tok_emb + (size_t)tok * d;
-    const float *pe = pos_emb + (size_t)p * d;
-    T *o = x + ((size_t)r * n_new + i) * d;
-    for (int c = threadIdx.x; c < d; c += 256) o[c] = from_f32<T>(to_f32<T>(e[c]) + pe[c]);
+    embed_row<T>(tok_emb, pos_emb, tok, p, d, x + ((size_t)r * n_new + i) * d, threadIdx.x, 256);
 }
 
 template <typename T>
diff --git a/stable_ts_amd/csrc/swx_runtime.hip b/stable_ts_amd/csrc/swx_runtime.hip
--- a/stable_ts_amd/csrc/swx_runtime.hip
+++ b/stable_ts_amd/csrc/swx_runtime.hip
@@ -59,7 +59,7 @@
     int max_windows = 0, max_rows = 0, ws_n_align = 0;
     struct WsLayout {
         size_t melT, h1, x, h, qkv, att, u, gmax, small_i32, zeros_i32, ticket;
-        size_t tokens0, tokens1, anc0, anc1, pos0, win_begin, sum_lp, sum_lp_next, row_done, win_done, win_done_prev, n_done;
+        size_t tokens0, tokens1, anc0, anc1, pos0, win_begin, sum_lp, sum_lp_next, row_done, win_done, win_done_prev, n_done, sup_mask;
         size_t fin_tokens, fin_score, fin_len, fin_count, cand_lp, cand_tok, logits, hid2;
         size_t kcache, vcache, sk, sv, cap, mean, sd, suppress, slabs, heads, win_uid;
         size_t total;
@@ -263,6 +263,7 @@
     L.mean = take((size_t)Bmax * (n_align > 0 ? n_align : 1) * D.n_audio_ctx * 4);
     L.sd = take((size_t)Bmax * (n_align > 0 ? n_align : 1) * D.n_audio_ctx * 4);
     L.suppress = take((size_t)MAX_SUPPRESS * 4);
+    L.sup_mask = take((size_t)1024 * 8);
     {
         int64_t srows = Mmax > 160 ? Mmax : 160;
         if ((int64_t)Bmax * D.n_text_ctx > srows) srows = (int64_t)Bmax * D.n_text_ctx;
@@ -343,6 +344,7 @@
     int step_pos;
     int pos_bound;
     unsigned char *qcap;
+    bool skip_embed;
 };
 
 int decoder_step_dec(swx_model *m, const FwdCfg &f, hipStream_t s)
@@ -353,8 +355,9 @@
     const int rows = f.W * f.rpw;
     f16 *x = m->Wp<f16>(m->L.x), *q = m->Wp<f16>(m->L.qkv), *att = m->Wp<f16>(m->L.att), *u = m->Wp<f16>(m->L.u);
     float *slabs = m->Wp<float>(m->L.slabs);
-    SWX_TRY(swx_embed(m->dtype, f.tokens, f.ld_tok, nullptr, f.pos0, rows, 1, m->arena + m->o_tok_emb,
-                      m->A<float>(m->o_dec_pos), d, x, s));
+    if (!f.skip_embed)
+        SWX_TRY(swx_embed(m->dtype, f.tokens, f.ld_tok, nullptr, f.pos0, rows, 1, m->arena + m->o_tok_emb,
+                          m->A<float>(m->o_dec_pos), d, x, s));
     const int64_t chunk = xkv_chunk_elems(m);
     const bool pf_on = !(g_debug_flags & SWX_FLAG_NO_PREFETCH) && rows >= 32;
     auto pf_of = [&](size_t w_off, int N, int K, int epi) {
@@ -428,8 +431,9 @@
     const int R = f.W * f.rpw, rows = R * f.n_new;
     f16 *x = m->Wp<f16>(m->L.x), *q = m->Wp<f16>(m->L.qkv), *att = m->Wp<f16>(m->L.att), *u = m->Wp<f16>(m->L.u);
     float *slabs = m->Wp<float>(m->L.slabs);
-    SWX_TRY(swx_embed(m->dtype, f.tokens, f.ld_tok, nullptr, f.pos0, R, f.n_new, m->arena + m->o_tok_emb,
-                      m->A<float>(m->o_dec_pos), d, x, s));
+    if (!f.skip_embed)
+        SWX_TRY(swx_embed(m->dtype, f.tokens, f.ld_tok, nullptr, f.pos0, R, f.n_new, m->arena + m->o_tok_emb,
+                          m->A<float>(m->o_dec_pos), d, x, s));
     const int64_t chunk = xkv_chunk_elems(m);
     const bool pf_on = !(g_debug_flags & SWX_FLAG_NO_PREFETCH) && rows >= 32;
     auto pf_of = [&](size_t w_off, int N, int K, int epi) {
@@ -511,8 +515,9 @@
     const int rows = R * f.n_new;
     if (rows > m->L.rows_big) return -8;
     unsigned char *x = m->ws + m->L.x, *h = m->ws + m->L.h, *qkv = m->ws + m->L.qkv, *att = m->ws + m->L.att, *u = m->ws + m->L.u;
-    SWX_TRY(swx_embed(m->dtype, f.tokens, f.ld_tok, nullptr, f.pos0, R, f.n_new, m->arena + m->o_tok_emb,
-                      m->A<float>(m->o_dec_pos), d, x, s));
+    if (!f.skip_embed)
+        SWX_TRY(swx_embed(m->dtype, f.tokens, f.ld_tok, nullptr, f.pos0, R, f.n_new, m->arena + m->o_tok_emb,
+                          m->A<float>(m->o_dec_pos), d, x, s));
     for (int l = 0; l < D.n_text_layer; ++l) {
         const LayerW &w = m->dec[l];
         SWX_TRY(swx_layernorm(m->dtype, x, d, m->A<float>(w.ln1_g), m->A<float>(w.ln1_b), h, d, rows, d, s));
@@ -1161,6 +1166,12 @@
     b.win_done = m->Wp<int32_t>(m->L.win_done); b.win_done_prev = m->Wp<int32_t>(m->L.win_done_prev);
     b.n_done = m->Wp<int32_t>(m->L.n_done);
     b.step_dev = b.n_done + 1;
+    const bool fused_tail = !(g_debug_flags & SWX_FLAG_TAIL_3LAUNCH);
+    if (fused_tail) {
+        b.emb_tok = m->arena + m->o_tok_emb; b.emb_pos = m->A<float>(m->o_dec_pos); b.emb_x = m->ws + m->L.x;
+        b.emb_d = D.n_text_state; b.emb_f16 = m->dtype == SWX_F16 ? 1 : 0;
+    }
+    b.adv_ticket = b.n_done + 2;
     b.fin_tokens = m->Wp<int32_t>(m->L.fin_tokens); b.fin_score = m->Wp<float>(m->L.fin_score);
     b.fin_len = m->Wp<int32_t>(m->L.fin_len); b.fin_count = m->Wp<int32_t>(m->L.fin_count);
     b.cand_lp = m->Wp<float>(m->L.cand_lp); b.cand_tok = m->Wp<int32_t>(m->L.cand_tok);
@@ -1172,6 +1183,7 @@
         if (er != hipSuccess) return -100 - (int)er;
     }
     b.suppress = sup;
+    b.sup_mask = m->Wp<unsigned long long>(m->L.sup_mask);
     for (int t : {cfg->eot, cfg->sot, cfg->timestamp_begin}) if (t < 0 || t >= D.n_vocab) return -2;
     for (int t : {cfg->no_timestamps, cfg->no_speech, cfg->blank_token}) if (t < -1 || t >= D.n_vocab) return -2;
     b.win_uid = nullptr;
@@ -1259,6 +1271,7 @@
         g.tokens = b.tokens[cur_in]; g.ld_tok = b.TS; g.pos0 = b.pos0;
         g.kcache = f.kcache; g.vcache = f.vcache; g.layer_stride = layer_stride; g.cache_rows = m->max_rows;
         g.anc = use_anc ? b.anc[cur_in] : nullptr; g.xkv = (const unsigned char *)d_xkv; g.capture = false;
+        g.skip_embed = fused_tail;
         g.step_pos = capturing ? 0 : n_init + steps;
         g.pos_bound = n_init + cfg->sample_len;
         const int fr = decoder_forward(m, g, st);
@@ -1649,6 +1662,119 @@
     return swx_self_attention(SWX_F16, sa, 1, S(stream));
 }
 
+namespace {
+struct TailLayout { int64_t off[SWX_TAIL_N_FIELDS]; int64_t state_bytes, logits, suppress, begin, sup_mask, work_bytes; };
+int tail_layout(const swx_decode_cfg *c, int V, int n_ctx, int d, int dtype, TailLayout &L)
+{
+    if (!c || c->n_windows <= 0 || c->n_group <= 0 || c->n_group > MAX_GROUP || V <= 0 || n_ctx <= 0 || d <= 0) return -1;
+    if (dtype != SWX_F16 && dtype != SWX_F32) return -1;
+    if (c->n_suppress < 0 || c->n_suppress > MAX_SUPPRESS) return -2;
+    const int64_t W = c->n_windows, M = W * c->n_group, TS = n_ctx + 1, e = dtype == SWX_F16 ? 2 : 4;
+    int64_t cur = 0;
+    auto take = [&](int64_t bytes) { const int64_t o = cur; cur = (cur + bytes + 255) & ~(int64_t)255; return o; };
+    int k = 0;
+    L.off[k++] = take(M * TS * 4); L.off[k++] = take(M * TS * 4);
+    L.off[k++] = take(M * n_ctx * 4); L.off[k++] = take(M * n_ctx * 4);
+    L.off[k++] = take(M * 4); L.off[k++] = take(M * 4); L.off[k++] = take(M * 4);
+    L.off[k++] = take(W * 4); L.off[k++] = take(W * 4);
+    L.off[k++] = take(256);
+    L.off[k++] = take(W * FIN_CAP * TS * 4); L.off[k++] = take(W * FIN_CAP * 4);
+    L.off[k++] = take(W * FIN_CAP * 4); L.off[k++] = take(W * 4);
+    L.off[k++] = take(M * (c->n_group + 1) * 4); L.off[k++] = take(M * (c->n_group + 1) * 4);
+    L.off[k++] = take(M * d * e);
+    static_assert(SWX_TAIL_N_FIELDS == 17, "swx_test_decode_tail: state fields");
+    L.state_bytes = cur;
+    L.logits = take(M * (int64_t)V * 4); L.suppress = take((int64_t)MAX_SUPPRESS * 4); L.begin = take(W * 4); L.sup_mask = take(1024 * 8);
+    L.work_bytes = cur;
+    return 0;
+}
+}
+
+int64_t swx_test_decode_tail_layout(const swx_decode_cfg *cfg, int n_vocab, int n_ctx, int d, int dtype, int64_t *h_offsets)
+{
+    TailLayout L;
+    const int rc = tail_layout(cfg, n_vocab, n_ctx, d, dtype, L);
+    if (rc < 0) return rc;
+    if (h_offsets) { for (int k = 0; k < SWX_TAIL_N_FIELDS; ++k) h_offsets[k] = L.off[k]; h_offsets[SWX_TAIL_N_FIELDS] = L.state_bytes; }
+    return L.work_bytes;
+}
+
+int swx_test_decode_tail(const swx_decode_cfg *cfg, const int32_t *d_init_tokens, const int32_t *d_suppress, const uint8_t *d_ts_mask,
+                         int n_vocab, int n_ctx, int d, int dtype, const float *d_logits, int n_steps, const void *d_tok_emb,
+                         const float *d_pos_emb, void *d_work, void *d_state_out, void *stream)
+{
+    TailLayout L;
+    SWX_TRY(tail_layout(cfg, n_vocab, n_ctx, d, dtype, L));
+    if (!d_init_tokens || !d_logits || !d_tok_emb || !d_pos_emb || !d_work || !d_state_out || n_steps <= 0) return -1;
+    const int W = cfg->n_windows, G = cfg->n_group, M = W * G;
+    int n_init = cfg->sample_begin;
+    std::vector<int32_t> nb;
+    if (cfg->sample_begins) {
+        nb.assign(cfg->sample_begins, cfg->sample_begins + W);
+        for (int v : nb) if (v <= 0 || v > n_ctx) return -1;
+        n_init = *std::max_element(nb.begin(), nb.end());
+    }
+    const int n_min = nb.empty() ? n_init : *std::min_element(nb.begin(), nb.end());
+    const bool ragged = n_min != n_init;
+    if (n_init <= 0 || n_init > n_ctx || n_min + n_steps > n_ctx + 1) return -1;
+    for (int t : {cfg->eot, cfg->timestamp_begin}) if (t < 0 || t >= n_vocab) return -2;
+    for (int t : {cfg->no_timestamps, cfg->blank_token}) if (t < -1 || t >= n_vocab) return -2;
+    hipStream_t s = S(stream);
+    unsigned char *wk = (unsigned char *)d_work;
+    hipError_t er = hipMemsetAsync(wk, 0, (size_t)L.work_bytes, s);
+    if (er != hipSuccess) return -100 - (int)er;
+    DecodeBufs b{};
+    b.cfg = *cfg;
+    b.cfg.sample_begin = n_init; b.cfg.sample_begins = nullptr; b.cfg.sot_indices = nullptr; b.cfg.window_uid = nullptr;
+    if (cfg->beam || cfg->temperature == 0.f) b.cfg.noise = nullptr;
+    b.W = W; b.G = G; b.M = M; b.V = n_vocab; b.TS = n_ctx + 1; b.n_ctx = n_ctx; b.n_init = n_init;
+    const float pat = cfg->patience > 0.f ? cfg->patience : 1.0f;
+    b.max_cand = cfg->beam ? (int)lrintf((float)G * pat) : 0;
+    if (cfg->beam && (b.max_cand <= 0 || b.max_cand > FIN_CAP)) return -2;
+    b.fin_cap = FIN_CAP;
+    auto at = [&](int k) { return wk + L.off[k]; };
+    b.tokens[0] = (int32_t *)at(0); b.tokens[1] = (int32_t *)at(1);
+    b.anc[0] = G > 1 ? (int32_t *)at(2) : nullptr; b.anc[1] = G > 1 ? (int32_t *)at(3) : nullptr;
+    b.pos0 = (int32_t *)at(4); b.sum_lp = (float *)at(5); b.sum_lp_next = nullptr; b.row_done = (int32_t *)at(6);
+    b.win_done = (int32_t *)at(7); b.win_done_prev = (int32_t *)at(8);
+    b.n_done = (int32_t *)at(9); b.step_dev = b.n_done + 1; b.adv_ticket = b.n_done + 2;
+    b.fin_tokens = (int32_t *)at(10); b.fin_score = (float *)at(11); b.fin_len = (int32_t *)at(12); b.fin_count = (int32_t *)at(13);
+    b.cand_lp = (float *)at(14); b.cand_tok = (int32_t *)at(15);
+    void *x = at(16);
+    b.logits = (float *)(wk + L.logits);
+    b.ts_mask = d_ts_mask;
+    if (cfg->n_suppress > 0) {
+        if (!d_suppress) return -1;
+        er = hipMemcpyAsync(wk + L.suppress, d_suppress, (size_t)cfg->n_suppress * 4, hipMemcpyDeviceToDevice, s);
+        if (er != hipSuccess) return -100 - (int)er;
+    }
+    b.suppress = (const int32_t *)(wk + L.suppress);
+    b.sup_mask = (unsigned long long *)(wk + L.sup_mask);
+    if (ragged) {
+        er = hipMemcpyAsync(wk + L.begin, nb.data(), (size_t)W * 4, hipMemcpyHostToDevice, s);
+        if (er == hipSuccess) er = hipStreamSynchronize(s);
+        if (er != hipSuccess) return -100 - (int)er;
+        b.begin = (const int32_t *)(wk + L.begin);
+    }
+    const bool fused_tail = !(g_debug_flags & SWX_FLAG_TAIL_3LAUNCH);
+    if (fused_tail) { b.emb_tok = d_tok_emb; b.emb_pos = d_pos_emb; b.emb_x = x; b.emb_d = d; b.emb_f16 = dtype == SWX_F16 ? 1 : 0; }
+    SWX_TRY(swx_decode_init(b, d_init_tokens, s));
+    SWX_TRY(swx_decode_after_prefill(b, nullptr, nullptr, s));
+    int cur = 0;
+    for (int i = 0; i < n_steps; ++i) {
+        er = hipMemcpyAsync(b.logits, d_logits + (size_t)i * M * n_vocab, (size_t)M * n_vocab * 4, hipMemcpyDeviceToDevice, s);
+        if (er != hipSuccess) return -100 - (int)er;
+        SWX_TRY(swx_decode_select(b, cur, s));
+        if (cfg->beam) cur ^= 1;
+        if (!fused_tail)
+            SWX_TRY(swx_embed(dtype, b.tokens[cur], b.TS, nullptr, b.pos0, M, 1, d_tok_emb, d_pos_emb, d, x, s));
+        er = hipMemcpyAsync((unsigned char *)d_state_out + (size_t)i * L.state_bytes, wk, (size_t)L.state_bytes, hipMemcpyDeviceToDevice, s);
+        if (er != hipSuccess) return -100 - (int)er;
+    }
+    er = hipStreamSynchronize(s);
+    return er == hipSuccess ? 0 : -100 - (int)er;
+}
+
 int swx_test_layernorm(int dtype, const void *d_x, const float *d_g, const float *d_b, void *d_y, int rows, int d, void *stream)
 {
     return swx_layernorm(dtype, d_x, d, d_g, d_b, d_y, d, rows, d, S(stream));
```

Result: slower. 1395 x real time (-1.0%).
